# tie-pilot-qxw/NTT

Measured on AMD Instinct MI355X. Metric: field-elements/sec, 2^24 forward NTT over BN254 Fr; achieved HBM GB/s vs peak, higher is better.
Workload: dtype u256 mod p: 9 x 29-bit limbs, u32 x u32 + u64 MAD (v_mad_u64_u32)

## Files before the change

ntt_amd/csrc/eng29_args.hpp:

```cpp
#pragma once
#include <cmath>
#include <stdint.h>

#include "field29.hpp"

namespace ntt {

template <class E29, int L, int NH, class EA>
inline void eng29_fill_consts(EA& A, const uint32_t* p) {
  uint32_t pw[NH];
  for (int i = 0; i < NH; ++i) pw[i] = p[i];
  pack29<L, NH>(A.M.p, pw);
  for (int i = 0; i < L; ++i) A.kp[0][i] = A.M.p[i];
  for (int j = 1; j < 5; ++j) {
    for (int i = 0; i < L; ++i) A.kp[j][i] = A.kp[j - 1][i] << 1;
    norm_u<L>(A.kp[j]);
  }
  for (int i = 0; i < L; ++i) A.M.p2[i] = A.kp[1][i];
  neg29<L>(A.pbar, A.M.p);
  uint32_t inv = 1;
  for (int i = 0; i < 5; ++i) inv *= 2 - p[0] * inv;
  A.M.pinv = (0u - inv) & kMask29;
  const uint32_t ptop = A.M.p[L - 1];
  A.red_ok = ptop >= (1u << 18) ? 1u : 0u;
  A.red_inv = std::nextafter(1.0f / (float)(ptop + 1u), 0.0f);
  auto padded = [&](uint32_t K, uint32_t pad, uint32_t* c) {
    uint32_t kp[L];
    uint64_t carry = 0;
    for (int i = 0; i < L; ++i) {
      const uint64_t v = (uint64_t)A.M.p[i] * K + carry;
      kp[i] = (uint32_t)v & kMask29;
      carry = v >> 29;
    }
    kp[L - 1] += (uint32_t)(carry << 29);
    const uint32_t b = pad >> 29;
    c[0] = kp[0] + pad;
    for (int i = 1; i + 1 < L; ++i) c[i] = kp[i] + pad - b;
    c[L - 1] = kp[L - 1] - b;
  };
  padded(5, 1u << 29, A.pc[E29::PC_5_29]);
  padded(9, 1u << 30, A.pc[E29::PC_9_30]);
  padded(4, 1u << 29, A.pc[E29::PC_4_29]);
  padded(17, 1u << 29, A.pc[E29::PC_17_29]);
  padded(7, 1u << 30, A.pc[E29::PC_7_30]);
}

}
```

ntt_amd/csrc/engines.hpp:

```cpp
#pragma once
#include "field.hpp"
#include "field29.hpp"
#include "field29_asm9.hpp"
#include "field31.hpp"
#include "field64.hpp"

#ifndef NTT_DEBUG_CHECKS
#define NTT_DEBUG_CHECKS 0
#endif
enum : uint32_t {
  NTT_DBG_BOUNDS = 1u << 8,
  NTT_DBG_INPUT = 1u << 9,
  NTT_DBG_LAZY = 1u << 10,
  NTT_DBG_OUTPUT = 1u << 11
};
__device__ __forceinline__ void ntt_dbg_flag(uint32_t* status, uint32_t bit) {
  if (status) __hip_atomic_fetch_or(status, bit, __ATOMIC_RELAXED, __HIP_MEMORY_SCOPE_AGENT);
}
#ifndef NTT_WAVES_256
#define NTT_WAVES_256 4
#endif
#ifndef NTT_EPT_256
#define NTT_EPT_256 4
#endif
#ifndef NTT_256_PASS1_TABLE
#define NTT_256_PASS1_TABLE 1
#endif
#ifndef NTT_P_SCRATCH32
#define NTT_P_SCRATCH32 1
#endif
#ifndef NTT_P_NARROW_FIRST
#define NTT_P_NARROW_FIRST 1
#endif
#ifndef NTT_P_PASS1_TABLE
#define NTT_P_PASS1_TABLE 1
#endif
#ifndef NTT_P_LDS_TW
#define NTT_P_LDS_TW 1
#endif
#ifndef NTT_EPT_P
#define NTT_EPT_P 8
#endif
#ifndef NTT_TILE_LOG_P
#define NTT_TILE_LOG_P 13
#endif
#ifndef NTT_MIN_COLS_LOG_P
#define NTT_MIN_COLS_LOG_P 4
#endif
#ifndef NTT_TILE_LOG_256
#define NTT_TILE_LOG_256 10
#endif
#ifndef NTT_TILE_LOG_G
#define NTT_TILE_LOG_G 12
#endif
#ifndef NTT_EPT_G
#define NTT_EPT_G 8
#endif
#ifndef NTT_G_PASS1_TABLE
#define NTT_G_PASS1_TABLE 0
#endif
#ifndef NTT_TILE_LOG_31
#define NTT_TILE_LOG_31 13
#endif
#ifndef NTT_EPT_31
#define NTT_EPT_31 8
#endif
#ifndef NTT_MIN_COLS_LOG_31
#define NTT_MIN_COLS_LOG_31 4
#endif
#ifndef NTT_PREF_COLS_LOG_31
#define NTT_PREF_COLS_LOG_31 5
#endif
#ifndef NTT_31_PASS1_TABLE
#define NTT_31_PASS1_TABLE 1
#endif

namespace ntt {

__device__ __forceinline__ void store_wt16(uint4* p, uint32_t a, uint32_t b, uint32_t c, uint32_t d) {
  typedef uint32_t v4u __attribute__((ext_vector_type(4)));
  const v4u v = {a, b, c, d};
  asm volatile("global_store_dwordx4 %0, %1, off sc1\n\ts_nop 1" ::"v"(p), "v"(v) : "memory");
}

template <int L, int W32, int SCR_ = 0, int TL_ = 0>
struct Eng29 {
  static constexpr int W = L;
  static constexpr int MEMW = W32;
  static constexpr int SCRW = SCR_ ? SCR_ : ((L <= 9 && W32 > 8) ? 8 : W32);
  static constexpr int TABW = (L <= 9) ? 8 : W32;
  static constexpr int TW = (2 * L + 3) & ~3;
  static constexpr int LDSW = L;
  static constexpr int IN = 4;
  static constexpr int MUL_OUT = 4;
  static constexpr int EPT = (L <= 9) ? NTT_EPT_256 : 8;
  static constexpr int TILE_LOG = TL_ ? TL_ : ((L <= 9) ? (EPT == 8 ? 11 : NTT_TILE_LOG_256) : 10);
  static constexpr int WAVES_PER_EU = (L <= 9) ? (EPT == 4 ? NTT_WAVES_256 : 2) : 2;
  static constexpr int MIN_COLS_LOG = TL_ == 12 ? 0 : 2;
  static constexpr bool PASS1_FULL_TABLE = NTT_256_PASS1_TABLE;
  static constexpr bool NARROW_FIRST = false;
  static constexpr bool SHOUP_OUTER = (L == 9);
  static constexpr bool LDS_TW = false;
  static constexpr bool SGPR_TW = (L == 9);
  static constexpr bool FASTRED = 29 * L - 18 <= 255;
  struct Tw {
    uint32_t w[L];
    uint32_t ws[L];
  };
  struct Args {
    Mod29<L> M;
    uint32_t kp[5][L];
    uint32_t pbar[L];
    Tw w8[3];
    Tw ninv;
    float red_inv;
    uint32_t red_ok;
    uint32_t pc[5][L];
    uint32_t* dbg;
  };
  __device__ static bool dbg_below(const uint32_t (&x)[W], const uint32_t (&q)[L]) {
    uint32_t y[W];
#pragma unroll
    for (int i = 0; i < W; ++i) y[i] = x[i];
    norm_u<L>(y);
    for (int i = L - 1; i >= 0; --i)
      if (y[i] != q[i]) return y[i] < q[i];
    return false;
  }
  __device__ static bool dbg_canonical(const uint32_t (&x)[W], const Args& A) { return dbg_below(x, A.kp[0]); }
  enum : int { PC_5_29 = 0, PC_9_30 = 1, PC_4_29 = 2, PC_17_29 = 3, PC_7_30 = 4 };

  template <int MW = W32>
  __device__ static __forceinline__ void load(uint32_t (&x)[W], const uint32_t* __restrict__ base, size_t idx) {
    constexpr int MR = (L <= 9 && MW > 8 && !NTT_DEBUG_CHECKS) ? 8 : MW;
    uint32_t w[MW];
    const uint4* p = reinterpret_cast<const uint4*>(base + idx * MW);
#pragma unroll
    for (int q = 0; q < MW / 4; ++q) {
      if (4 * q < MR) {
        const uint4 v = p[q];
        w[4 * q] = v.x; w[4 * q + 1] = v.y; w[4 * q + 2] = v.z; w[4 * q + 3] = v.w;
      } else {
        w[4 * q] = w[4 * q + 1] = w[4 * q + 2] = w[4 * q + 3] = 0u;
      }
    }
    pack29<L, MW>(x, w);
  }
  template <int FROM, int TO>
  __device__ static __forceinline__ void reduce_chain(uint32_t (&x)[W], const Args& A) {
    static_assert(FROM <= 32 && TO >= 1, "lazy bound");
    if constexpr (FROM > TO) {
      constexpr int j = __builtin_ctz(FROM / 2);
      cond_sub<L>(x, A.kp[j]);
      reduce_chain<FROM / 2, TO>(x, A);
    }
  }
  template <bool R32 = true>
  __device__ static __forceinline__ void reduce_top(uint32_t (&x)[W], const Args& A) {
    const float qf = __builtin_fmaf((float)x[L - 1], A.red_inv, -0x1p-15f);
    const uint32_t q = qf > 0.f ? (uint32_t)qf : 0u;
    if constexpr (R32) {
    uint32_t c = 0;
#pragma unroll
    for (int i = 0; i < L; ++i) {
      const uint64_t acc = (uint64_t)q * A.pbar[i] + (uint32_t)(x[i] + c);
      x[i] = (uint32_t)acc & kMask29;
      c = (uint32_t)(acc >> 29);
    }
    } else {
    uint64_t acc = 0;
#pragma unroll
    for (int i = 0; i < L; ++i) {
      acc = (acc >> 29) + x[i] + (uint64_t)q * A.pbar[i];
      x[i] = (uint32_t)acc & kMask29;
    }
    }
  }
  __device__ static __forceinline__ void cond_sub_rare(uint32_t (&x)[W], const uint32_t (&q)[L]) {
    if (__any(x[L - 1] >= q[L - 1])) cond_sub<L>(x, q);
  }
  template <int FROM, int TO, bool FAST = false, bool R32 = true>
  __device__ static __forceinline__ void reduce(uint32_t (&x)[W], const Args& A) {
    if constexpr (FAST && FROM > 4 && TO <= 4) {
      reduce_top<R32>(x, A);
      if constexpr (TO == 1) cond_sub_rare(x, A.kp[0]);
    } else if constexpr (FAST && FROM == 4 && TO == 2) {
      cond_sub_rare(x, A.kp[1]);
    } else {
      reduce_chain<FROM, TO>(x, A);
    }
  }
  template <int BOUND, bool FAST = false, int MW = W32, bool WT = false>
  __device__ static __forceinline__ void store_lazy(uint32_t* __restrict__ base, size_t idx, uint32_t (&x)[W],
                                                    const Args& A) {
    reduce<BOUND, 2, FAST>(x, A);
#if NTT_DEBUG_CHECKS
    if (!dbg_below(x, A.kp[1])) ntt_dbg_flag(A.dbg, NTT_DBG_LAZY);
#endif
    put<MW, WT>(base, idx, x);
  }
  template <int BOUND, bool FAST = false, int MW = W32>
  __device__ static __forceinline__ void store(uint32_t* __restrict__ base, size_t idx, uint32_t (&x)[W],
                                               const Args& A) {
    reduce<BOUND, 1, FAST>(x, A);
#if NTT_DEBUG_CHECKS
    if (!dbg_below(x, A.kp[0])) ntt_dbg_flag(A.dbg, NTT_DBG_OUTPUT);
#endif
    put<MW>(base, idx, x);
  }
  template <int MW = W32, bool WT = false>
  __device__ static __forceinline__ void put(uint32_t* __restrict__ base, size_t idx, const uint32_t (&x)[W]) {
    uint32_t w[MW];
    unpack29<L, MW>(w, x);
    uint4* p = reinterpret_cast<uint4*>(base + idx * MW);
#pragma unroll
    for (int q = 0; q < MW / 4; ++q) {
      if constexpr (WT)
        store_wt16(p + q, w[4 * q], w[4 * q + 1], w[4 * q + 2], w[4 * q + 3]);
      else
        p[q] = make_uint4(w[4 * q], w[4 * q + 1], w[4 * q + 2], w[4 * q + 3]);
    }
  }
  __device__ static __forceinline__ void tload(Tw& t, const uint32_t* __restrict__ tab, size_t idx) {
    const uint4* p = reinterpret_cast<const uint4*>(tab + idx * TW);
#pragma unroll
    for (int q = 0; q < TW / 4; ++q) {
      const uint4 v = p[q];
      const uint32_t vv[4] = {v.x, v.y, v.z, v.w};
#pragma unroll
      for (int r = 0; r < 4; ++r) {
        const int i = 4 * q + r;
        if (i < L) t.w[i] = vv[r];
        else if (i < 2 * L) t.ws[i - L] = vv[r];
      }
    }
  }
  __device__ static __forceinline__ void tload_u(Tw& t, const uint32_t* __restrict__ tab, uint32_t idx) {
    typedef uint32_t V4 __attribute__((ext_vector_type(4)));
    typedef const __attribute__((address_space(4))) V4* CP;
    const CP p = (CP)(tab + (size_t)idx * TW);
#pragma unroll
    for (int q = 0; q < TW / 4; ++q) {
      const V4 v = p[q];
      const uint32_t vv[4] = {v.x, v.y, v.z, v.w};
#pragma unroll
      for (int r = 0; r < 4; ++r) {
        const int i = 4 * q + r;
        if (i < L) t.w[i] = vv[r];
        else if (i < 2 * L) t.ws[i - L] = vv[r];
      }
    }
  }
  __device__ static __forceinline__ void mul(uint32_t (&x)[W], const Tw& t, const Args& A) {
    uint32_t r[W];
    if constexpr (L == 9)
      mulc29_a9(r, x, t.w, t.ws, A.pbar);
    else
      mulc29_blk<L>(r, x, t.w, t.ws, A.pbar);
#pragma unroll
    for (int i = 0; i < W; ++i) x[i] = r[i];
  }
  __device__ static __forceinline__ void mul_u(uint32_t (&x)[W], const Tw& t, const Args& A) {
    uint32_t r[W];
    if constexpr (L == 9)
      mulc29_a9u(r, x, t.w, t.ws, A.pbar);
    else
      mulc29_blk<L>(r, x, t.w, t.ws, A.pbar);
#pragma unroll
    for (int i = 0; i < W; ++i) x[i] = r[i];
  }
  __device__ static __forceinline__ void mulv(uint32_t (&x)[W], const uint32_t (&y)[W], const Args& A) {
    uint32_t r[W];
    if constexpr (L == 9)
      mont29_a9(r, x, y, A.M);
    else
      mont29<L>(r, x, y, A.M);
#pragma unroll
    for (int i = 0; i < W; ++i) x[i] = r[i];
  }
  __device__ static __forceinline__ void bfly_lk(uint32_t (&a)[W], uint32_t (&b)[W], const uint32_t (&q)[L]) {
#pragma unroll
    for (int i = 0; i < L; ++i) {
      const uint32_t x = a[i], y = b[i];
      a[i] = x + y;
      b[i] = x - y + q[i];
    }
    norm_u<L>(a);
    norm_s<L>(b);
  }
  template <int K>
  __device__ static __forceinline__ void bfly_l(uint32_t (&a)[W], uint32_t (&b)[W], const Args& A) {
    static_assert(K == 4 || K == 8 || K == 16, "lazy bound");
    bfly_lk(a, b, A.kp[__builtin_ctz(K)]);
  }
  template <int K>
  __device__ static __forceinline__ void bfly_w_l(uint32_t (&a)[W], uint32_t (&b)[W], const Tw& t,
                                                  const Args& A) {
    bfly_l<K>(a, b, A);
    mul_u(b, t, A);
  }
  template <int CI>
  __device__ static __forceinline__ void bfly_raw(uint32_t (&a)[W], uint32_t (&b)[W], const Args& A) {
#pragma unroll
    for (int i = 0; i < L; ++i) {
      const uint32_t x = a[i], y = b[i];
      a[i] = x + y;
      b[i] = x - y + A.pc[CI][i];
    }
  }
  template <int CI>
  __device__ static __forceinline__ void bfly_raw_w(uint32_t (&a)[W], uint32_t (&b)[W], const Tw& t,
                                                    const Args& A) {
    bfly_raw<CI>(a, b, A);
    mul_u(b, t, A);
  }
  __device__ static __forceinline__ void norm(uint32_t (&x)[W]) {
    norm_u<L>(x);
  }
};

template <int N, int MEMW_, int SCR_ = 0>
struct Eng32 {
  static_assert(N == 1, "the 32-bit engine is the 1-limb path (p < 2^30)");
  static constexpr int W = 1;
  static constexpr int MEMW = MEMW_;
  static constexpr int SCRW = SCR_ ? SCR_ : (NTT_P_SCRATCH32 ? 1 : MEMW_);
  static constexpr int TABW = 1;
  static constexpr int TW = 2;
  static constexpr int LDSW = 1;
  static constexpr int IN = 4;
  static constexpr int MUL_OUT = 4;
  static constexpr int EPT = NTT_EPT_P;
  static constexpr int TILE_LOG = NTT_TILE_LOG_P;
  static constexpr int MIN_COLS_LOG = NTT_MIN_COLS_LOG_P;
  static constexpr bool PASS1_FULL_TABLE = NTT_P_PASS1_TABLE;
  static constexpr bool NARROW_FIRST = NTT_P_NARROW_FIRST;
  static constexpr bool SHOUP_OUTER = false;
  static constexpr bool LDS_TW = NTT_P_LDS_TW;
  static constexpr bool SGPR_TW = false;
  static constexpr int WAVES_PER_EU = 4;
  static constexpr bool FASTRED = false;
  struct Tw {
    uint32_t w[1];
    uint32_t ws;
  };
  struct Args {
    uint32_t p, p2;
    uint32_t pinv;
    Tw w8[3];
    Tw ninv;
    uint32_t* dbg;
  };
  __device__ static __forceinline__ uint32_t red(uint32_t x, uint32_t m) {
    return min(x, x - m);
  }
  __device__ static bool dbg_canonical(const uint32_t (&x)[W], const Args& A) { return x[0] < A.p; }
  __device__ static __forceinline__ uint32_t shoup(uint32_t x, uint32_t w, uint32_t ws, uint32_t p) {
    const uint32_t q = __umulhi(x, ws);
    return x * w - q * p;
  }
  template <int MW = MEMW_>
  __device__ static __forceinline__ void load(uint32_t (&x)[W], const uint32_t* __restrict__ base, size_t idx) {
    static_assert(MW == MEMW_ || MW == SCRW || MW == TABW, "HBM width");
    if constexpr (MW == 1)
      x[0] = base[idx];
    else
      x[0] = reinterpret_cast<const uint2*>(base)[idx].x;
  }
  template <int FROM, int TO, bool FAST = false, bool R32 = true>
  __device__ static __forceinline__ void reduce(uint32_t (&)[W], const Args&) {}
  template <int MW = MEMW_>
  __device__ static __forceinline__ void put(uint32_t* __restrict__ base, size_t idx, uint32_t v) {
    static_assert(MW == MEMW_ || MW == SCRW || MW == TABW, "HBM width");
    if constexpr (MW == 1)
      base[idx] = v;
    else
      reinterpret_cast<uint2*>(base)[idx] = make_uint2(v, 0u);
  }
  template <int BOUND, bool FAST = false, int MW = MEMW_, bool WT = false>
  __device__ static __forceinline__ void store_lazy(uint32_t* __restrict__ base, size_t idx, uint32_t (&x)[W],
                                                    [[maybe_unused]] const Args& A) {
    static_assert(!WT, "write-through scratch stores: Eng29 engines only (fused schedule)");
#if NTT_DEBUG_CHECKS
    if (x[0] >= A.p2) ntt_dbg_flag(A.dbg, NTT_DBG_LAZY);
#endif
    put<MW>(base, idx, x[0]);
  }
  template <int BOUND, bool FAST = false, int MW = MEMW_>
  __device__ static __forceinline__ void store(uint32_t* __restrict__ base, size_t idx, uint32_t (&x)[W],
                                               const Args& A) {
    const uint32_t v = red(x[0], A.p);
#if NTT_DEBUG_CHECKS
    if (v >= A.p) ntt_dbg_flag(A.dbg, NTT_DBG_OUTPUT);
#endif
    put<MW>(base, idx, v);
  }
  __device__ static __forceinline__ void tload(Tw& t, const uint32_t* __restrict__ tab, size_t idx) {
    const uint2 v = reinterpret_cast<const uint2*>(tab)[idx];
    t.w[0] = v.x;
    t.ws = v.y;
  }
  __device__ static __forceinline__ void tload_lds(Tw& t, const uint32_t* lds_tw, uint32_t idx) {
    const uint2 v = reinterpret_cast<const uint2*>(lds_tw)[idx];
    t.w[0] = v.x;
    t.ws = v.y;
  }
  __device__ static __forceinline__ void mul(uint32_t (&x)[W], const Tw& t, const Args& A) {
    x[0] = shoup(x[0], t.w[0], t.ws, A.p);
  }
  __device__ static __forceinline__ void mul_u(uint32_t (&x)[W], const Tw& t, const Args& A) { mul(x, t, A); }
  __device__ static __forceinline__ void mulv(uint32_t (&x)[W], const uint32_t (&y)[W], const Args& A) {
    const uint32_t lo = x[0] * y[0], hi = __umulhi(x[0], y[0]);
    const uint32_t m = lo * A.pinv;
    x[0] = hi - __umulhi(m, A.p) + A.p;
  }
  template <int K>
  __device__ static __forceinline__ void bfly_l(uint32_t (&a)[W], uint32_t (&b)[W], const Args& A) {
    const uint32_t s = a[0] + b[0], d = a[0] - b[0] + A.p2;
    a[0] = red(s, A.p2);
    b[0] = red(d, A.p2);
  }
  template <int K>
  __device__ static __forceinline__ void bfly_w_l(uint32_t (&a)[W], uint32_t (&b)[W], const Tw& t, const Args& A) {
    const uint32_t s = a[0] + b[0], d = a[0] - b[0] + A.p2;
    a[0] = red(s, A.p2);
    b[0] = shoup(d, t.w[0], t.ws, A.p);
  }
};

struct Eng64G {
  static constexpr int W = 2;
  static constexpr int MEMW = 2;
  static constexpr int SCRW = 2;
  static constexpr int TABW = 2;
  static constexpr int TW = 2;
  static constexpr int LDSW = 2;
  static constexpr int IN = 1;
  static constexpr int MUL_OUT = 1;
  static constexpr int EPT = NTT_EPT_G;
  static constexpr int TILE_LOG = NTT_TILE_LOG_G;
  static constexpr int MIN_COLS_LOG = 4;
  static constexpr bool PASS1_FULL_TABLE = NTT_G_PASS1_TABLE;
  static constexpr bool NARROW_FIRST = true;
  static constexpr bool SHOUP_OUTER = false;
  static constexpr bool LDS_TW = false;
  static constexpr bool SGPR_TW = false;
  static constexpr int WAVES_PER_EU = 4;
  static constexpr bool FASTRED = false;
  struct Tw {
    uint32_t w[2];
  };
  struct Args {
    Tw w8[3];
    Tw ninv;
    uint32_t* dbg;
  };
  __device__ static __forceinline__ uint64_t u64(const uint32_t (&x)[W]) { return ((uint64_t)x[1] << 32) | x[0]; }
  __device__ static __forceinline__ void set(uint32_t (&x)[W], uint64_t v) {
    x[0] = (uint32_t)v;
    x[1] = (uint32_t)(v >> 32);
  }
  __device__ static bool dbg_canonical(const uint32_t (&x)[W], const Args&) { return gl64::is_canonical(u64(x)); }
  template <int MW = MEMW>
  __device__ static __forceinline__ void load(uint32_t (&x)[W], const uint32_t* __restrict__ base, size_t idx) {
    static_assert(MW == 2, "HBM width");
    const uint2 v = reinterpret_cast<const uint2*>(base)[idx];
    x[0] = v.x;
    x[1] = v.y;
  }
  template <int FROM, int TO, bool FAST = false, bool R32 = true>
  __device__ static __forceinline__ void reduce(uint32_t (&)[W], const Args&) {}
  template <int MW = MEMW, bool WT = false>
  __device__ static __forceinline__ void put(uint32_t* __restrict__ base, size_t idx, const uint32_t (&x)[W]) {
    static_assert(MW == 2 && !WT, "HBM width; write-through stores: Eng29 engines only");
    reinterpret_cast<uint2*>(base)[idx] = make_uint2(x[0], x[1]);
  }
  template <int BOUND, bool FAST = false, int MW = MEMW, bool WT = false>
  __device__ static __forceinline__ void store_lazy(uint32_t* __restrict__ base, size_t idx, uint32_t (&x)[W],
                                                    [[maybe_unused]] const Args& A) {
#if NTT_DEBUG_CHECKS
    if (!gl64::is_canonical(u64(x))) ntt_dbg_flag(A.dbg, NTT_DBG_LAZY);
#endif
    put<MW, WT>(base, idx, x);
  }
  template <int BOUND, bool FAST = false, int MW = MEMW>
  __device__ static __forceinline__ void store(uint32_t* __restrict__ base, size_t idx, uint32_t (&x)[W],
                                               [[maybe_unused]] const Args& A) {
#if NTT_DEBUG_CHECKS
    if (!gl64::is_canonical(u64(x))) ntt_dbg_flag(A.dbg, NTT_DBG_OUTPUT);
#endif
    put<MW>(base, idx, x);
  }
  __device__ static __forceinline__ void tload(Tw& t, const uint32_t* __restrict__ tab, size_t idx) {
    const uint2 v = reinterpret_cast<const uint2*>(tab)[idx];
    t.w[0] = v.x;
    t.w[1] = v.y;
  }
  __device__ static __forceinline__ void tload_lds(Tw& t, const uint32_t* lds_tw, uint32_t idx) {
    const uint2 v = reinterpret_cast<const uint2*>(lds_tw)[idx];
    t.w[0] = v.x;
    t.w[1] = v.y;
  }
  __device__ static __forceinline__ void mul(uint32_t (&x)[W], const Tw& t, const Args&) {
    set(x, gl64::mul(u64(x), u64(t.w)));
  }
  __device__ static __forceinline__ void mul_u(uint32_t (&x)[W], const Tw& t, const Args& A) { mul(x, t, A); }
  __device__ static __forceinline__ void mulv(uint32_t (&x)[W], const uint32_t (&y)[W], const Args&) {
    set(x, gl64::mul(u64(x), u64(y)));
  }
  template <int K>
  __device__ static __forceinline__ void bfly_l(uint32_t (&a)[W], uint32_t (&b)[W], const Args&) {
    const uint64_t x = u64(a), y = u64(b);
    set(a, gl64::add(x, y));
    set(b, gl64::sub(x, y));
  }
  template <int K>
  __device__ static __forceinline__ void bfly_w_l(uint32_t (&a)[W], uint32_t (&b)[W], const Tw& t, const Args&) {
    const uint64_t x = u64(a), y = u64(b);
    set(a, gl64::add(x, y));
    set(b, gl64::mul(gl64::sub(x, y), u64(t.w)));
  }
};

struct Eng31 {
  static constexpr int W = 1;
  static constexpr int MEMW = 1;
  static constexpr int SCRW = 1;
  static constexpr int TABW = 1;
  static constexpr int TW = 2;
  static constexpr int LDSW = 1;
  static constexpr int IN = 1;
  static constexpr int MUL_OUT = 1;
  static constexpr int EPT = NTT_EPT_31;
  static constexpr int TILE_LOG = NTT_TILE_LOG_31;
  static constexpr int MIN_COLS_LOG = NTT_MIN_COLS_LOG_31;
  static constexpr int PREF_COLS_LOG = NTT_PREF_COLS_LOG_31 > NTT_MIN_COLS_LOG_31 ? NTT_PREF_COLS_LOG_31 : NTT_MIN_COLS_LOG_31;
  static constexpr bool PASS1_FULL_TABLE = NTT_31_PASS1_TABLE;
  static constexpr bool NARROW_FIRST = true;
  static constexpr bool SHOUP_OUTER = false;
  static constexpr bool LDS_TW = true;
  static constexpr bool SGPR_TW = false;
  static constexpr int WAVES_PER_EU = 4;
  static constexpr bool FASTRED = false;
  struct Tw {
    uint32_t w[1];
    uint32_t ws;
  };
  struct Args {
    uint32_t p;
    uint32_t pinv;
    Tw w8[3];
    Tw ninv;
    uint32_t* dbg;
  };
  __device__ static bool dbg_canonical(const uint32_t (&x)[W], const Args& A) { return f31::is_canonical(x[0], A.p); }
  template <int MW = MEMW>
  __device__ static __forceinline__ void load(uint32_t (&x)[W], const uint32_t* __restrict__ base, size_t idx) {
    static_assert(MW == 1, "HBM width");
    x[0] = base[idx];
  }
  template <int FROM, int TO, bool FAST = false, bool R32 = true>
  __device__ static __forceinline__ void reduce(uint32_t (&)[W], const Args&) {}
  template <int BOUND, bool FAST = false, int MW = MEMW, bool WT = false>
  __device__ static __forceinline__ void store_lazy(uint32_t* __restrict__ base, size_t idx, uint32_t (&x)[W],
                                                    [[maybe_unused]] const Args& A) {
    static_assert(MW == 1 && !WT, "HBM width; write-through stores: Eng29 engines only");
#if NTT_DEBUG_CHECKS
    if (!f31::is_canonical(x[0], A.p)) ntt_dbg_flag(A.dbg, NTT_DBG_LAZY);
#endif
    base[idx] = x[0];
  }
  template <int BOUND, bool FAST = false, int MW = MEMW>
  __device__ static __forceinline__ void store(uint32_t* __restrict__ base, size_t idx, uint32_t (&x)[W],
                                               [[maybe_unused]] const Args& A) {
    static_assert(MW == 1, "HBM width");
#if NTT_DEBUG_CHECKS
    if (!f31::is_canonical(x[0], A.p)) ntt_dbg_flag(A.dbg, NTT_DBG_OUTPUT);
#endif
    base[idx] = x[0];
  }
  __device__ static __forceinline__ void tload(Tw& t, const uint32_t* __restrict__ tab, size_t idx) {
    const uint2 v = reinterpret_cast<const uint2*>(tab)[idx];
    t.w[0] = v.x;
    t.ws = v.y;
  }
  __device__ static __forceinline__ void tload_lds(Tw& t, const uint32_t* lds_tw, uint32_t idx) {
    const uint2 v = reinterpret_cast<const uint2*>(lds_tw)[idx];
    t.w[0] = v.x;
    t.ws = v.y;
  }
  __device__ static __forceinline__ void mul(uint32_t (&x)[W], const Tw& t, const Args& A) {
    x[0] = f31::mulc(x[0], t.w[0], t.ws, A.p);
  }
  __device__ static __forceinline__ void mul_u(uint32_t (&x)[W], const Tw& t, const Args& A) { mul(x, t, A); }
  __device__ static __forceinline__ void mulv(uint32_t (&x)[W], const uint32_t (&y)[W], const Args& A) {
    x[0] = f31::mulv(x[0], y[0], A.p, A.pinv);
  }
  template <int K>
  __device__ static __forceinline__ void bfly_l(uint32_t (&a)[W], uint32_t (&b)[W], const Args& A) {
    const uint32_t x = a[0], y = b[0];
    a[0] = f31::add(x, y, A.p);
    b[0] = f31::sub(x, y, A.p);
  }
  template <int K>
  __device__ static __forceinline__ void bfly_w_l(uint32_t (&a)[W], uint32_t (&b)[W], const Tw& t, const Args& A) {
    const uint32_t x = a[0], y = b[0];
    a[0] = f31::add(x, y, A.p);
    b[0] = f31::mulc(f31::sub_lazy(x, y, A.p), t.w[0], t.ws, A.p);
  }
};

template <int LDSW, int E>
__device__ __forceinline__ void lds_put(uint32_t* lds, uint32_t idx, const uint32_t (&x)[LDSW]) {
  constexpr int Q = LDSW / 4;
  uint4* l4 = reinterpret_cast<uint4*>(lds);
#pragma unroll
  for (int q = 0; q < Q; ++q) l4[q * E + idx] = make_uint4(x[4 * q], x[4 * q + 1], x[4 * q + 2], x[4 * q + 3]);
  uint32_t* l1 = lds + 4 * Q * E;
#pragma unroll
  for (int r = 4 * Q; r < LDSW; ++r) l1[(r - 4 * Q) * E + idx] = x[r];
}
template <int LDSW, int E>
__device__ __forceinline__ void lds_get(uint32_t (&x)[LDSW], const uint32_t* lds, uint32_t idx) {
  constexpr int Q = LDSW / 4;
  const uint4* l4 = reinterpret_cast<const uint4*>(lds);
#pragma unroll
  for (int q = 0; q < Q; ++q) {
    const uint4 v = l4[q * E + idx];
    x[4 * q] = v.x; x[4 * q + 1] = v.y; x[4 * q + 2] = v.z; x[4 * q + 3] = v.w;
  }
  const uint32_t* l1 = lds + 4 * Q * E;
#pragma unroll
  for (int r = 4 * Q; r < LDSW; ++r) x[r] = l1[(r - 4 * Q) * E + idx];
}

}
```

ntt_amd/csrc/field29.hpp:

```cpp
#pragma once
#include <stdint.h>

#if defined(__HIPCC__) || defined(__HIP__)
#include <hip/hip_runtime.h>
#define F29_HD __host__ __device__ __forceinline__
#else
#define F29_HD static inline
#endif

namespace ntt {

constexpr uint32_t kMask29 = (1u << 29) - 1;

template <int L>
struct Mod29 {
  uint32_t p[L];
  uint32_t p2[L];
  uint32_t pinv;
};

template <int L>
F29_HD void norm_u(uint32_t (&x)[L]) {
#pragma unroll
  for (int i = 0; i + 1 < L; ++i) {
    x[i + 1] += x[i] >> 29;
    x[i] &= kMask29;
  }
}
template <int L>
F29_HD int32_t norm_s(uint32_t (&x)[L]) {
#pragma unroll
  for (int i = 0; i + 1 < L; ++i) {
    x[i + 1] = (uint32_t)((int32_t)x[i + 1] + ((int32_t)x[i] >> 29));
    x[i] &= kMask29;
  }
  return (int32_t)x[L - 1];
}

template <int L>
F29_HD void cond_sub(uint32_t (&x)[L], const uint32_t (&q)[L]) {
  uint32_t t[L];
#pragma unroll
  for (int i = 0; i < L; ++i) t[i] = x[i] - q[i];
  const bool neg = norm_s<L>(t) < 0;
#pragma unroll
  for (int i = 0; i < L; ++i) x[i] = neg ? x[i] : t[i];
}

template <int L>
F29_HD void add29(uint32_t (&u)[L], const uint32_t (&a)[L], const uint32_t (&b)[L], const Mod29<L>& M) {
#pragma unroll
  for (int i = 0; i < L; ++i) u[i] = a[i] + b[i];
  norm_u<L>(u);
  cond_sub<L>(u, M.p2);
}
template <int L>
F29_HD void sub29_raw(uint32_t (&d)[L], const uint32_t (&a)[L], const uint32_t (&b)[L], const Mod29<L>& M) {
#pragma unroll
  for (int i = 0; i < L; ++i) d[i] = a[i] - b[i] + M.p2[i];
  norm_s<L>(d);
}
template <int L>
F29_HD void sub29(uint32_t (&d)[L], const uint32_t (&a)[L], const uint32_t (&b)[L], const Mod29<L>& M) {
  sub29_raw<L>(d, a, b, M);
  cond_sub<L>(d, M.p2);
}

template <int L>
F29_HD void mont29(uint32_t (&r)[L], const uint32_t (&a)[L], const uint32_t (&b)[L], const Mod29<L>& M) {
  uint32_t m[L];
  uint64_t acc = 0;
#pragma unroll
  for (int i = 0; i < L; ++i) {
#pragma unroll
    for (int j = 0; j < i; ++j) {
      acc += (uint64_t)a[j] * b[i - j];
      acc += (uint64_t)m[j] * M.p[i - j];
    }
    acc += (uint64_t)a[i] * b[0];
    m[i] = ((uint32_t)acc * M.pinv) & kMask29;
    acc += (uint64_t)m[i] * M.p[0];
    acc >>= 29;
  }
#pragma unroll
  for (int i = L; i < 2 * L; ++i) {
#pragma unroll
    for (int j = i - L + 1; j < L; ++j) {
      acc += (uint64_t)a[j] * b[i - j];
      acc += (uint64_t)m[j] * M.p[i - j];
    }
    r[i - L] = (uint32_t)acc & kMask29;
    acc >>= 29;
  }
}

#if defined(__HIP_DEVICE_COMPILE__)
__device__ __forceinline__ uint64_t mad29v(uint32_t a, uint32_t b, uint64_t c) {
  uint64_t r, cc;
  asm("v_mad_u64_u32 %0, %1, %2, %3, %4" : "=v"(r), "=s"(cc) : "v"(a), "v"(b), "v"(c));
  return r;
}
__device__ __forceinline__ uint64_t mad29s(uint32_t a, uint32_t b, uint64_t c) {
  uint64_t r, cc;
  asm("v_mad_u64_u32 %0, %1, %2, %3, %4" : "=v"(r), "=s"(cc) : "v"(a), "s"(b), "v"(c));
  return r;
}
#else
static inline uint64_t mad29v(uint32_t a, uint32_t b, uint64_t c) { return c + (uint64_t)a * b; }
static inline uint64_t mad29s(uint32_t a, uint32_t b, uint64_t c) { return c + (uint64_t)a * b; }
#endif

#if defined(__HIP_DEVICE_COMPILE__)
#define NTT_MAD4(C1, C2)                                                                          \
  asm("v_mad_u64_u32 %0, %1, %2, %3, %0\n\t"                                                   \
      "v_mad_u64_u32 %0, %1, %4, %5, %0\n\t"                                                   \
      "v_mad_u64_u32 %0, %1, %6, %7, %0\n\t"                                                   \
      "v_mad_u64_u32 %0, %1, %8, %9, %0"                                                       \
      : "+v"(acc), "=&s"(cc)                                                                    \
      : "v"(a0), C2(b0), "v"(a1), C2(b1), "v"(a2), C2(b2), "v"(a3), C2(b3))
#define NTT_MAD2(C2)                                                                              \
  asm("v_mad_u64_u32 %0, %1, %2, %3, %0\n\t"                                                   \
      "v_mad_u64_u32 %0, %1, %4, %5, %0"                                                       \
      : "+v"(acc), "=&s"(cc)                                                                    \
      : "v"(a0), C2(b0), "v"(a1), C2(b1))
#define NTT_CV(x) "v"(x)
#define NTT_CS(x) "s"(x)
__device__ __forceinline__ uint64_t mad4vv(uint64_t acc, uint32_t a0, uint32_t b0, uint32_t a1, uint32_t b1,
                                           uint32_t a2, uint32_t b2, uint32_t a3, uint32_t b3) {
  uint64_t cc;
  NTT_MAD4(NTT_CV, NTT_CV);
  return acc;
}
__device__ __forceinline__ uint64_t mad4vs(uint64_t acc, uint32_t a0, uint32_t b0, uint32_t a1, uint32_t b1,
                                           uint32_t a2, uint32_t b2, uint32_t a3, uint32_t b3) {
  uint64_t cc;
  NTT_MAD4(NTT_CV, NTT_CS);
  return acc;
}
__device__ __forceinline__ uint64_t mad2vv(uint64_t acc, uint32_t a0, uint32_t b0, uint32_t a1, uint32_t b1) {
  uint64_t cc;
  NTT_MAD2(NTT_CV);
  return acc;
}
__device__ __forceinline__ uint64_t mad2vs(uint64_t acc, uint32_t a0, uint32_t b0, uint32_t a1, uint32_t b1) {
  uint64_t cc;
  NTT_MAD2(NTT_CS);
  return acc;
}
#undef NTT_MAD4
#undef NTT_MAD2
#undef NTT_CV
#undef NTT_CS
#else
static inline uint64_t mad4vv(uint64_t acc, uint32_t a0, uint32_t b0, uint32_t a1, uint32_t b1, uint32_t a2,
                              uint32_t b2, uint32_t a3, uint32_t b3) {
  return acc + (uint64_t)a0 * b0 + (uint64_t)a1 * b1 + (uint64_t)a2 * b2 + (uint64_t)a3 * b3;
}
static inline uint64_t mad4vs(uint64_t acc, uint32_t a0, uint32_t b0, uint32_t a1, uint32_t b1, uint32_t a2,
                              uint32_t b2, uint32_t a3, uint32_t b3) {
  return mad4vv(acc, a0, b0, a1, b1, a2, b2, a3, b3);
}
static inline uint64_t mad2vv(uint64_t acc, uint32_t a0, uint32_t b0, uint32_t a1, uint32_t b1) {
  return acc + (uint64_t)a0 * b0 + (uint64_t)a1 * b1;
}
static inline uint64_t mad2vs(uint64_t acc, uint32_t a0, uint32_t b0, uint32_t a1, uint32_t b1) {
  return mad2vv(acc, a0, b0, a1, b1);
}
#endif

template <int L, bool US, int lo, int hi>
F29_HD uint64_t mad_span(uint64_t acc, const uint32_t (&a)[L], const uint32_t (&b)[L], int k) {
  if constexpr (hi - lo + 1 >= 4) {
    acc = US ? mad4vs(acc, a[lo], b[k - lo], a[lo + 1], b[k - lo - 1], a[lo + 2], b[k - lo - 2], a[lo + 3],
                      b[k - lo - 3])
             : mad4vv(acc, a[lo], b[k - lo], a[lo + 1], b[k - lo - 1], a[lo + 2], b[k - lo - 2], a[lo + 3],
                      b[k - lo - 3]);
    return mad_span<L, US, lo + 4, hi>(acc, a, b, k);
  } else if constexpr (hi - lo + 1 >= 2) {
    acc = US ? mad2vs(acc, a[lo], b[k - lo], a[lo + 1], b[k - lo - 1])
             : mad2vv(acc, a[lo], b[k - lo], a[lo + 1], b[k - lo - 1]);
    return mad_span<L, US, lo + 2, hi>(acc, a, b, k);
  } else if constexpr (hi - lo + 1 == 1) {
    return US ? mad29s(a[lo], b[k - lo], acc) : mad29v(a[lo], b[k - lo], acc);
  } else {
    return acc;
  }
}

template <int L, int K = L - 2>
F29_HD void mulc29_hi(uint32_t (&q)[L], uint64_t& acc, const uint32_t (&x)[L], const uint32_t (&ws)[L]) {
  if constexpr (K < 2 * L - 1) {
    constexpr int lo = (K - (L - 1) > 0) ? K - (L - 1) : 0, hi = (K < L - 1) ? K : L - 1;
    acc = mad_span<L, false, lo, hi>(acc, x, ws, K);
    if constexpr (K >= L) q[K - L] = (uint32_t)acc & kMask29;
    acc >>= 29;
    mulc29_hi<L, K + 1>(q, acc, x, ws);
  }
}
template <int L, int K = 0>
F29_HD void mulc29_lo(uint32_t (&r)[L], uint64_t& acc, const uint32_t (&x)[L], const uint32_t (&w)[L],
                      const uint32_t (&q)[L], const uint32_t (&pbar)[L]) {
  if constexpr (K < L) {
    acc = mad_span<L, false, 0, K>(acc, x, w, K);
    acc = mad_span<L, true, 0, K>(acc, q, pbar, K);
    r[K] = (uint32_t)acc & kMask29;
    acc >>= 29;
    mulc29_lo<L, K + 1>(r, acc, x, w, q, pbar);
  }
}
template <int L>
F29_HD void mulc29_blk(uint32_t (&r)[L], const uint32_t (&x)[L], const uint32_t (&w)[L], const uint32_t (&ws)[L],
                       const uint32_t (&pbar)[L]) {
  uint32_t q[L];
  uint64_t acc = 0;
  mulc29_hi<L>(q, acc, x, ws);
  q[L - 1] = (uint32_t)acc;
  acc = 0;
  mulc29_lo<L>(r, acc, x, w, q, pbar);
}

template <int L>
F29_HD void mont29_chain(uint32_t (&r)[L], const uint32_t (&a)[L], const uint32_t (&b)[L], const Mod29<L>& M) {
  uint32_t m[L];
  uint64_t acc = 0;
#pragma unroll
  for (int i = 0; i < L; ++i) {
#pragma unroll
    for (int j = 0; j <= i; ++j) acc = mad29v(a[j], b[i - j], acc);
#pragma unroll
    for (int j = 0; j < i; ++j) acc = mad29s(m[j], M.p[i - j], acc);
    m[i] = ((uint32_t)acc * M.pinv) & kMask29;
    acc = mad29s(m[i], M.p[0], acc);
    acc >>= 29;
  }
#pragma unroll
  for (int i = L; i < 2 * L; ++i) {
#pragma unroll
    for (int j = i - L + 1; j < L; ++j) acc = mad29v(a[j], b[i - j], acc);
#pragma unroll
    for (int j = i - L + 1; j < L; ++j) acc = mad29s(m[j], M.p[i - j], acc);
    r[i - L] = (uint32_t)acc & kMask29;
    acc >>= 29;
  }
}

template <int L>
F29_HD void mulc29(uint32_t (&r)[L], const uint32_t (&x)[L], const uint32_t (&w)[L], const uint32_t (&ws)[L],
                   const uint32_t (&pbar)[L]) {
  uint32_t q[L];
  uint64_t acc = 0;
#pragma unroll
  for (int k = L - 2; k < 2 * L - 1; ++k) {
#pragma unroll
    for (int i = (k - (L - 1) > 0 ? k - (L - 1) : 0); i <= (k < L - 1 ? k : L - 1); ++i)
      acc = mad29v(x[i], ws[k - i], acc);
    if (k >= L) q[k - L] = (uint32_t)acc & kMask29;
    acc >>= 29;
  }
  q[L - 1] = (uint32_t)acc;
  acc = 0;
#pragma unroll
  for (int k = 0; k < L; ++k) {
#pragma unroll
    for (int i = 0; i <= k; ++i) acc = mad29v(x[i], w[k - i], acc);
#pragma unroll
    for (int i = 0; i <= k; ++i) acc = mad29s(q[i], pbar[k - i], acc);
    r[k] = (uint32_t)acc & kMask29;
    acc >>= 29;
  }
}

template <int L>
F29_HD void mulc29_cc(uint32_t (&r)[L], const uint32_t (&x)[L], const uint32_t (&w)[L], const uint32_t (&ws)[L],
                   const uint32_t (&pbar)[L]) {
  uint32_t q[L];
  uint64_t acc = 0;
#pragma unroll
  for (int k = L - 2; k < 2 * L - 1; ++k) {
#pragma unroll
    for (int i = (k - (L - 1) > 0 ? k - (L - 1) : 0); i <= (k < L - 1 ? k : L - 1); ++i)
      acc += (uint64_t)x[i] * ws[k - i];
    if (k >= L) q[k - L] = (uint32_t)acc & kMask29;
    acc >>= 29;
  }
  q[L - 1] = (uint32_t)acc;
  acc = 0;
#pragma unroll
  for (int k = 0; k < L; ++k) {
#pragma unroll
    for (int i = 0; i <= k; ++i) acc += (uint64_t)x[i] * w[k - i];
#pragma unroll
    for (int i = 0; i <= k; ++i) acc += (uint64_t)q[i] * pbar[k - i];
    r[k] = (uint32_t)acc & kMask29;
    acc >>= 29;
  }
}

template <int L>
F29_HD void mullo29(uint32_t (&r)[L], const uint32_t (&a)[L], const uint32_t (&b)[L]) {
  uint64_t acc = 0;
#pragma unroll
  for (int k = 0; k < L; ++k) {
#pragma unroll
    for (int i = 0; i <= k; ++i) acc = mad29v(a[i], b[k - i], acc);
    r[k] = (uint32_t)acc & kMask29;
    acc >>= 29;
  }
}
template <int L>
F29_HD void neg29(uint32_t (&r)[L], const uint32_t (&a)[L]) {
  uint32_t c = 1;
#pragma unroll
  for (int i = 0; i < L; ++i) {
    const uint32_t v = (kMask29 - a[i]) + c;
    r[i] = v & kMask29;
    c = v >> 29;
  }
}
template <int L>
F29_HD void shoup_ws29(uint32_t (&ws)[L], const uint32_t (&wR)[L], const uint32_t (&pinvB)[L]) {
  uint32_t t[L];
  neg29<L>(t, wR);
  mullo29<L>(ws, t, pinvB);
}
template <int L>
F29_HD void inv_mod_B29(uint32_t (&inv)[L], const uint32_t (&p)[L]) {
  uint32_t i0 = 1;
  for (int k = 0; k < 5; ++k) i0 *= 2 - p[0] * i0;
#pragma unroll
  for (int i = 0; i < L; ++i) inv[i] = 0;
  inv[0] = i0 & kMask29;
  for (int bits = 29; bits < 29 * L; bits *= 2) {
    uint32_t t[L], u[L];
    mullo29<L>(t, p, inv);
    neg29<L>(u, t);
    uint32_t c = 2;
    for (int i = 0; i < L; ++i) {
      const uint32_t v = u[i] + c;
      u[i] = v & kMask29;
      c = v >> 29;
    }
    mullo29<L>(t, inv, u);
    for (int i = 0; i < L; ++i) inv[i] = t[i];
  }
}

template <int L, int W32>
F29_HD void pack29(uint32_t (&x)[L], const uint32_t (&w)[W32]) {
#pragma unroll
  for (int i = 0; i < L; ++i) {
    const int bit = 29 * i, k = bit / 32, s = bit % 32;
    const uint32_t lo = (k < W32) ? w[k] : 0u;
    const uint32_t hi = (k + 1 < W32) ? w[k + 1] : 0u;
#if defined(__HIP_DEVICE_COMPILE__)
    x[i] = __builtin_amdgcn_alignbit(hi, lo, (uint32_t)s) & kMask29;
#else
    const uint64_t v = ((uint64_t)hi << 32) | lo;
    x[i] = (uint32_t)(v >> s) & kMask29;
#endif
  }
}
template <int L, int W32>
F29_HD void unpack29(uint32_t (&w)[W32], const uint32_t (&x)[L]) {
#pragma unroll
  for (int k = 0; k < W32; ++k) {
    const int bit = 32 * k, i = bit / 29, s = bit % 29;
    uint32_t v = (i < L) ? (x[i] >> s) : 0u;
    if (i + 1 < L) v |= x[i + 1] << (29 - s);
    if (i + 2 < L && 58 - s < 32) v |= x[i + 2] << (58 - s);
    w[k] = v;
  }
}

}
```

ntt_amd/csrc/field29_asm9.hpp:

```cpp
#pragma once
#include "field29.hpp"

namespace ntt {
#if defined(__HIP_DEVICE_COMPILE__)
__device__ __forceinline__ void mulc29_a9(uint32_t (&r)[9], const uint32_t (&x)[9], const uint32_t (&w)[9],
                                          const uint32_t (&ws)[9], const uint32_t (&pbar)[9]) {
  uint32_t q[9];
  uint64_t acc = 0, cc;
  asm("v_mad_u64_u32 %0, %1, %2, %3, %0\n\tv_mad_u64_u32 %0, %1, %4, %5, %0\n\tv_mad_u64_u32 %0, %1, %6, %7, %0\n\tv_mad_u64_u32 %0, %1, %8, %9, %0\n\tv_mad_u64_u32 %0, %1, %10, %11, %0\n\tv_mad_u64_u32 %0, %1, %12, %13, %0\n\tv_mad_u64_u32 %0, %1, %14, %15, %0\n\tv_mad_u64_u32 %0, %1, %16, %17, %0"
      : "+v"(acc), "=&s"(cc)
      : "v"(x[0]), "v"(ws[7]), "v"(x[1]), "v"(ws[6]), "v"(x[2]), "v"(ws[5]),
        "v"(x[3]), "v"(ws[4]), "v"(x[4]), "v"(ws[3]), "v"(x[5]), "v"(ws[2]),
        "v"(x[6]), "v"(ws[1]), "v"(x[7]), "v"(ws[0]));
  acc >>= 29;
  asm("v_mad_u64_u32 %0, %1, %2, %3, %0\n\tv_mad_u64_u32 %0, %1, %4, %5, %0\n\tv_mad_u64_u32 %0, %1, %6, %7, %0\n\tv_mad_u64_u32 %0, %1, %8, %9, %0\n\tv_mad_u64_u32 %0, %1, %10, %11, %0\n\tv_mad_u64_u32 %0, %1, %12, %13, %0\n\tv_mad_u64_u32 %0, %1, %14, %15, %0\n\tv_mad_u64_u32 %0, %1, %16, %17, %0\n\tv_mad_u64_u32 %0, %1, %18, %19, %0"
      : "+v"(acc), "=&s"(cc)
      : "v"(x[0]), "v"(ws[8]), "v"(x[1]), "v"(ws[7]), "v"(x[2]), "v"(ws[6]),
        "v"(x[3]), "v"(ws[5]), "v"(x[4]), "v"(ws[4]), "v"(x[5]), "v"(ws[3]),
        "v"(x[6]), "v"(ws[2]), "v"(x[7]), "v"(ws[1]), "v"(x[8]), "v"(ws[0]));
  acc >>= 29;
  asm("v_mad_u64_u32 %0, %1, %2, %3, %0\n\tv_mad_u64_u32 %0, %1, %4, %5, %0\n\tv_mad_u64_u32 %0, %1, %6, %7, %0\n\tv_mad_u64_u32 %0, %1, %8, %9, %0\n\tv_mad_u64_u32 %0, %1, %10, %11, %0\n\tv_mad_u64_u32 %0, %1, %12, %13, %0\n\tv_mad_u64_u32 %0, %1, %14, %15, %0\n\tv_mad_u64_u32 %0, %1, %16, %17, %0"
      : "+v"(acc), "=&s"(cc)
      : "v"(x[1]), "v"(ws[8]), "v"(x[2]), "v"(ws[7]), "v"(x[3]), "v"(ws[6]),
        "v"(x[4]), "v"(ws[5]), "v"(x[5]), "v"(ws[4]), "v"(x[6]), "v"(ws[3]),
        "v"(x[7]), "v"(ws[2]), "v"(x[8]), "v"(ws[1]));
  q[0] = (uint32_t)acc & kMask29;
  acc >>= 29;
  asm("v_mad_u64_u32 %0, %1, %2, %3, %0\n\tv_mad_u64_u32 %0, %1, %4, %5, %0\n\tv_mad_u64_u32 %0, %1, %6, %7, %0\n\tv_mad_u64_u32 %0, %1, %8, %9, %0\n\tv_mad_u64_u32 %0, %1, %10, %11, %0\n\tv_mad_u64_u32 %0, %1, %12, %13, %0\n\tv_mad_u64_u32 %0, %1, %14, %15, %0"
      : "+v"(acc), "=&s"(cc)
      : "v"(x[2]), "v"(ws[8]), "v"(x[3]), "v"(ws[7]), "v"(x[4]), "v"(ws[6]),
        "v"(x[5]), "v"(ws[5]), "v"(x[6]), "v"(ws[4]), "v"(x[7]), "v"(ws[3]),
        "v"(x[8]), "v"(ws[2]));
  q[1] = (uint32_t)acc & kMask29;
  acc >>= 29;
  asm("v_mad_u64_u32 %0, %1, %2, %3, %0\n\tv_mad_u64_u32 %0, %1, %4, %5, %0\n\tv_mad_u64_u32 %0, %1, %6, %7, %0\n\tv_mad_u64_u32 %0, %1, %8, %9, %0\n\tv_mad_u64_u32 %0, %1, %10, %11, %0\n\tv_mad_u64_u32 %0, %1, %12, %13, %0"
      : "+v"(acc), "=&s"(cc)
      : "v"(x[3]), "v"(ws[8]), "v"(x[4]), "v"(ws[7]), "v"(x[5]), "v"(ws[6]),
        "v"(x[6]), "v"(ws[5]), "v"(x[7]), "v"(ws[4]), "v"(x[8]), "v"(ws[3]));
  q[2] = (uint32_t)acc & kMask29;
  acc >>= 29;
  asm("v_mad_u64_u32 %0, %1, %2, %3, %0\n\tv_mad_u64_u32 %0, %1, %4, %5, %0\n\tv_mad_u64_u32 %0, %1, %6, %7, %0\n\tv_mad_u64_u32 %0, %1, %8, %9, %0\n\tv_mad_u64_u32 %0, %1, %10, %11, %0"
      : "+v"(acc), "=&s"(cc)
      : "v"(x[4]), "v"(ws[8]), "v"(x[5]), "v"(ws[7]), "v"(x[6]), "v"(ws[6]),
        "v"(x[7]), "v"(ws[5]), "v"(x[8]), "v"(ws[4]));
  q[3] = (uint32_t)acc & kMask29;
  acc >>= 29;
  asm("v_mad_u64_u32 %0, %1, %2, %3, %0\n\tv_mad_u64_u32 %0, %1, %4, %5, %0\n\tv_mad_u64_u32 %0, %1, %6, %7, %0\n\tv_mad_u64_u32 %0, %1, %8, %9, %0"
      : "+v"(acc), "=&s"(cc)
      : "v"(x[5]), "v"(ws[8]), "v"(x[6]), "v"(ws[7]), "v"(x[7]), "v"(ws[6]),
        "v"(x[8]), "v"(ws[5]));
  q[4] = (uint32_t)acc & kMask29;
  acc >>= 29;
  asm("v_mad_u64_u32 %0, %1, %2, %3, %0\n\tv_mad_u64_u32 %0, %1, %4, %5, %0\n\tv_mad_u64_u32 %0, %1, %6, %7, %0"
      : "+v"(acc), "=&s"(cc)
      : "v"(x[6]), "v"(ws[8]), "v"(x[7]), "v"(ws[7]), "v"(x[8]), "v"(ws[6]));
  q[5] = (uint32_t)acc & kMask29;
  acc >>= 29;
  asm("v_mad_u64_u32 %0, %1, %2, %3, %0\n\tv_mad_u64_u32 %0, %1, %4, %5, %0"
      : "+v"(acc), "=&s"(cc)
      : "v"(x[7]), "v"(ws[8]), "v"(x[8]), "v"(ws[7]));
  q[6] = (uint32_t)acc & kMask29;
  acc >>= 29;
  asm("v_mad_u64_u32 %0, %1, %2, %3, %0"
      : "+v"(acc), "=&s"(cc)
      : "v"(x[8]), "v"(ws[8]));
  q[7] = (uint32_t)acc & kMask29;
  acc >>= 29;
  q[8] = (uint32_t)acc;
  acc = 0;
  asm("v_mad_u64_u32 %0, %1, %2, %3, %0\n\tv_mad_u64_u32 %0, %1, %4, %5, %0"
      : "+v"(acc), "=&s"(cc)
      : "v"(x[0]), "v"(w[0]), "v"(q[0]), "s"(pbar[0]));
  r[0] = (uint32_t)acc & kMask29;
  acc >>= 29;
  asm("v_mad_u64_u32 %0, %1, %2, %3, %0\n\tv_mad_u64_u32 %0, %1, %4, %5, %0\n\tv_mad_u64_u32 %0, %1, %6, %7, %0\n\tv_mad_u64_u32 %0, %1, %8, %9, %0"
      : "+v"(acc), "=&s"(cc)
      : "v"(x[0]), "v"(w[1]), "v"(x[1]), "v"(w[0]), "v"(q[0]), "s"(pbar[1]),
        "v"(q[1]), "s"(pbar[0]));
  r[1] = (uint32_t)acc & kMask29;
  acc >>= 29;
  asm("v_mad_u64_u32 %0, %1, %2, %3, %0\n\tv_mad_u64_u32 %0, %1, %4, %5, %0\n\tv_mad_u64_u32 %0, %1, %6, %7, %0\n\tv_mad_u64_u32 %0, %1, %8, %9, %0\n\tv_mad_u64_u32 %0, %1, %10, %11, %0\n\tv_mad_u64_u32 %0, %1, %12, %13, %0"
      : "+v"(acc), "=&s"(cc)
      : "v"(x[0]), "v"(w[2]), "v"(x[1]), "v"(w[1]), "v"(x[2]), "v"(w[0]),
        "v"(q[0]), "s"(pbar[2]), "v"(q[1]), "s"(pbar[1]), "v"(q[2]), "s"(pbar[0]));
  r[2] = (uint32_t)acc & kMask29;
  acc >>= 29;
  asm("v_mad_u64_u32 %0, %1, %2, %3, %0\n\tv_mad_u64_u32 %0, %1, %4, %5, %0\n\tv_mad_u64_u32 %0, %1, %6, %7, %0\n\tv_mad_u64_u32 %0, %1, %8, %9, %0\n\tv_mad_u64_u32 %0, %1, %10, %11, %0\n\tv_mad_u64_u32 %0, %1, %12, %13, %0\n\tv_mad_u64_u32 %0, %1, %14, %15, %0\n\tv_mad_u64_u32 %0, %1, %16, %17, %0"
      : "+v"(acc), "=&s"(cc)
      : "v"(x[0]), "v"(w[3]), "v"(x[1]), "v"(w[2]), "v"(x[2]), "v"(w[1]),
        "v"(x[3]), "v"(w[0]), "v"(q[0]), "s"(pbar[3]), "v"(q[1]), "s"(pbar[2]),
        "v"(q[2]), "s"(pbar[1]), "v"(q[3]), "s"(pbar[0]));
  r[3] = (uint32_t)acc & kMask29;
  acc >>= 29;
  asm("v_mad_u64_u32 %0, %1, %2, %3, %0\n\tv_mad_u64_u32 %0, %1, %4, %5, %0\n\tv_mad_u64_u32 %0, %1, %6, %7, %0\n\tv_mad_u64_u32 %0, %1, %8, %9, %0\n\tv_mad_u64_u32 %0, %1, %10, %11, %0\n\tv_mad_u64_u32 %0, %1, %12, %13, %0\n\tv_mad_u64_u32 %0, %1, %14, %15, %0\n\tv_mad_u64_u32 %0, %1, %16, %17, %0\n\tv_mad_u64_u32 %0, %1, %18, %19, %0\n\tv_mad_u64_u32 %0, %1, %20, %21, %0"
      : "+v"(acc), "=&s"(cc)
      : "v"(x[0]), "v"(w[4]), "v"(x[1]), "v"(w[3]), "v"(x[2]), "v"(w[2]),
        "v"(x[3]), "v"(w[1]), "v"(x[4]), "v"(w[0]), "v"(q[0]), "s"(pbar[4]),
        "v"(q[1]), "s"(pbar[3]), "v"(q[2]), "s"(pbar[2]), "v"(q[3]), "s"(pbar[1]),
        "v"(q[4]), "s"(pbar[0]));
  r[4] = (uint32_t)acc & kMask29;
  acc >>= 29;
  asm("v_mad_u64_u32 %0, %1, %2, %3, %0\n\tv_mad_u64_u32 %0, %1, %4, %5, %0\n\tv_mad_u64_u32 %0, %1, %6, %7, %0\n\tv_mad_u64_u32 %0, %1, %8, %9, %0\n\tv_mad_u64_u32 %0, %1, %10, %11, %0\n\tv_mad_u64_u32 %0, %1, %12, %13, %0\n\tv_mad_u64_u32 %0, %1, %14, %15, %0\n\tv_mad_u64_u32 %0, %1, %16, %17, %0\n\tv_mad_u64_u32 %0, %1, %18, %19, %0\n\tv_mad_u64_u32 %0, %1, %20, %21, %0\n\tv_mad_u64_u32 %0, %1, %22, %23, %0\n\tv_mad_u64_u32 %0, %1, %24, %25, %0"
      : "+v"(acc), "=&s"(cc)
      : "v"(x[0]), "v"(w[5]), "v"(x[1]), "v"(w[4]), "v"(x[2]), "v"(w[3]),
        "v"(x[3]), "v"(w[2]), "v"(x[4]), "v"(w[1]), "v"(x[5]), "v"(w[0]),
        "v"(q[0]), "s"(pbar[5]), "v"(q[1]), "s"(pbar[4]), "v"(q[2]), "s"(pbar[3]),
        "v"(q[3]), "s"(pbar[2]), "v"(q[4]), "s"(pbar[1]), "v"(q[5]), "s"(pbar[0]));
  r[5] = (uint32_t)acc & kMask29;
  acc >>= 29;
  asm("v_mad_u64_u32 %0, %1, %2, %3, %0\n\tv_mad_u64_u32 %0, %1, %4, %5, %0\n\tv_mad_u64_u32 %0, %1, %6, %7, %0\n\tv_mad_u64_u32 %0, %1, %8, %9, %0\n\tv_mad_u64_u32 %0, %1, %10, %11, %0\n\tv_mad_u64_u32 %0, %1, %12, %13, %0\n\tv_mad_u64_u32 %0, %1, %14, %15, %0\n\tv_mad_u64_u32 %0, %1, %16, %17, %0\n\tv_mad_u64_u32 %0, %1, %18, %19, %0\n\tv_mad_u64_u32 %0, %1, %20, %21, %0\n\tv_mad_u64_u32 %0, %1, %22, %23, %0\n\tv_mad_u64_u32 %0, %1, %24, %25, %0\n\tv_mad_u64_u32 %0, %1, %26, %27, %0\n\tv_mad_u64_u32 %0, %1, %28, %29, %0"
      : "+v"(acc), "=&s"(cc)
      : "v"(x[0]), "v"(w[6]), "v"(x[1]), "v"(w[5]), "v"(x[2]), "v"(w[4]),
        "v"(x[3]), "v"(w[3]), "v"(x[4]), "v"(w[2]), "v"(x[5]), "v"(w[1]),
        "v"(x[6]), "v"(w[0]), "v"(q[0]), "s"(pbar[6]), "v"(q[1]), "s"(pbar[5]),
        "v"(q[2]), "s"(pbar[4]), "v"(q[3]), "s"(pbar[3]), "v"(q[4]), "s"(pbar[2]),
        "v"(q[5]), "s"(pbar[1]), "v"(q[6]), "s"(pbar[0]));
  r[6] = (uint32_t)acc & kMask29;
  acc >>= 29;
  asm("v_mad_u64_u32 %0, %1, %2, %3, %0\n\tv_mad_u64_u32 %0, %1, %4, %5, %0\n\tv_mad_u64_u32 %0, %1, %6, %7, %0\n\tv_mad_u64_u32 %0, %1, %8, %9, %0\n\tv_mad_u64_u32 %0, %1, %10, %11, %0\n\tv_mad_u64_u32 %0, %1, %12, %13, %0\n\tv_mad_u64_u32 %0, %1, %14, %15, %0\n\tv_mad_u64_u32 %0, %1, %16, %17, %0\n\tv_mad_u64_u32 %0, %1, %18, %19, %0\n\tv_mad_u64_u32 %0, %1, %20, %21, %0\n\tv_mad_u64_u32 %0, %1, %22, %23, %0\n\tv_mad_u64_u32 %0, %1, %24, %25, %0\n\tv_mad_u64_u32 %0, %1, %26, %27, %0\n\tv_mad_u64_u32 %0, %1, %28, %29, %0\n\tv_mad_u64_u32 %0, %1, %30, %31, %0\n\tv_mad_u64_u32 %0, %1, %32, %33, %0"
      : "+v"(acc), "=&s"(cc)
      : "v"(x[0]), "v"(w[7]), "v"(x[1]), "v"(w[6]), "v"(x[2]), "v"(w[5]),
        "v"(x[3]), "v"(w[4]), "v"(x[4]), "v"(w[3]), "v"(x[5]), "v"(w[2]),
        "v"(x[6]), "v"(w[1]), "v"(x[7]), "v"(w[0]), "v"(q[0]), "s"(pbar[7]),
        "v"(q[1]), "s"(pbar[6]), "v"(q[2]), "s"(pbar[5]), "v"(q[3]), "s"(pbar[4]),
        "v"(q[4]), "s"(pbar[3]), "v"(q[5]), "s"(pbar[2]), "v"(q[6]), "s"(pbar[1]),
        "v"(q[7]), "s"(pbar[0]));
  r[7] = (uint32_t)acc & kMask29;
  acc >>= 29;
  asm("v_mad_u64_u32 %0, %1, %2, %3, %0\n\tv_mad_u64_u32 %0, %1, %4, %5, %0\n\tv_mad_u64_u32 %0, %1, %6, %7, %0\n\tv_mad_u64_u32 %0, %1, %8, %9, %0\n\tv_mad_u64_u32 %0, %1, %10, %11, %0\n\tv_mad_u64_u32 %0, %1, %12, %13, %0\n\tv_mad_u64_u32 %0, %1, %14, %15, %0\n\tv_mad_u64_u32 %0, %1, %16, %17, %0\n\tv_mad_u64_u32 %0, %1, %18, %19, %0\n\tv_mad_u64_u32 %0, %1, %20, %21, %0\n\tv_mad_u64_u32 %0, %1, %22, %23, %0\n\tv_mad_u64_u32 %0, %1, %24, %25, %0\n\tv_mad_u64_u32 %0, %1, %26, %27, %0\n\tv_mad_u64_u32 %0, %1, %28, %29, %0\n\tv_mad_u64_u32 %0, %1, %30, %31, %0\n\tv_mad_u64_u32 %0, %1, %32, %33, %0\n\tv_mad_u64_u32 %0, %1, %34, %35, %0\n\tv_mad_u64_u32 %0, %1, %36, %37, %0"
      : "+v"(acc), "=&s"(cc)
      : "v"(x[0]), "v"(w[8]), "v"(x[1]), "v"(w[7]), "v"(x[2]), "v"(w[6]),
        "v"(x[3]), "v"(w[5]), "v"(x[4]), "v"(w[4]), "v"(x[5]), "v"(w[3]),
        "v"(x[6]), "v"(w[2]), "v"(x[7]), "v"(w[1]), "v"(x[8]), "v"(w[0]),
        "v"(q[0]), "s"(pbar[8]), "v"(q[1]), "s"(pbar[7]), "v"(q[2]), "s"(pbar[6]),
        "v"(q[3]), "s"(pbar[5]), "v"(q[4]), "s"(pbar[4]), "v"(q[5]), "s"(pbar[3]),
        "v"(q[6]), "s"(pbar[2]), "v"(q[7]), "s"(pbar[1]), "v"(q[8]), "s"(pbar[0]));
  r[8] = (uint32_t)acc & kMask29;
}

__device__ __forceinline__ void mulc29_a9u(uint32_t (&r)[9], const uint32_t (&x)[9], const uint32_t (&w)[9],
                                          const uint32_t (&ws)[9], const uint32_t (&pbar)[9]) {
  uint32_t q[9];
  uint64_t acc = 0, cc;
  asm("v_mad_u64_u32 %0, %1, %2, %3, %0\n\tv_mad_u64_u32 %0, %1, %4, %5, %0\n\tv_mad_u64_u32 %0, %1, %6, %7, %0\n\tv_mad_u64_u32 %0, %1, %8, %9, %0\n\tv_mad_u64_u32 %0, %1, %10, %11, %0\n\tv_mad_u64_u32 %0, %1, %12, %13, %0\n\tv_mad_u64_u32 %0, %1, %14, %15, %0\n\tv_mad_u64_u32 %0, %1, %16, %17, %0"
      : "+v"(acc), "=&s"(cc)
      : "v"(x[0]), "s"(ws[7]), "v"(x[1]), "s"(ws[6]), "v"(x[2]), "s"(ws[5]),
        "v"(x[3]), "s"(ws[4]), "v"(x[4]), "s"(ws[3]), "v"(x[5]), "s"(ws[2]),
        "v"(x[6]), "s"(ws[1]), "v"(x[7]), "s"(ws[0]));
  acc >>= 29;
  asm("v_mad_u64_u32 %0, %1, %2, %3, %0\n\tv_mad_u64_u32 %0, %1, %4, %5, %0\n\tv_mad_u64_u32 %0, %1, %6, %7, %0\n\tv_mad_u64_u32 %0, %1, %8, %9, %0\n\tv_mad_u64_u32 %0, %1, %10, %11, %0\n\tv_mad_u64_u32 %0, %1, %12, %13, %0\n\tv_mad_u64_u32 %0, %1, %14, %15, %0\n\tv_mad_u64_u32 %0, %1, %16, %17, %0\n\tv_mad_u64_u32 %0, %1, %18, %19, %0"
      : "+v"(acc), "=&s"(cc)
      : "v"(x[0]), "s"(ws[8]), "v"(x[1]), "s"(ws[7]), "v"(x[2]), "s"(ws[6]),
        "v"(x[3]), "s"(ws[5]), "v"(x[4]), "s"(ws[4]), "v"(x[5]), "s"(ws[3]),
        "v"(x[6]), "s"(ws[2]), "v"(x[7]), "s"(ws[1]), "v"(x[8]), "s"(ws[0]));
  acc >>= 29;
  asm("v_mad_u64_u32 %0, %1, %2, %3, %0\n\tv_mad_u64_u32 %0, %1, %4, %5, %0\n\tv_mad_u64_u32 %0, %1, %6, %7, %0\n\tv_mad_u64_u32 %0, %1, %8, %9, %0\n\tv_mad_u64_u32 %0, %1, %10, %11, %0\n\tv_mad_u64_u32 %0, %1, %12, %13, %0\n\tv_mad_u64_u32 %0, %1, %14, %15, %0\n\tv_mad_u64_u32 %0, %1, %16, %17, %0"
      : "+v"(acc), "=&s"(cc)
      : "v"(x[1]), "s"(ws[8]), "v"(x[2]), "s"(ws[7]), "v"(x[3]), "s"(ws[6]),
        "v"(x[4]), "s"(ws[5]), "v"(x[5]), "s"(ws[4]), "v"(x[6]), "s"(ws[3]),
        "v"(x[7]), "s"(ws[2]), "v"(x[8]), "s"(ws[1]));
  q[0] = (uint32_t)acc & kMask29;
  acc >>= 29;
  asm("v_mad_u64_u32 %0, %1, %2, %3, %0\n\tv_mad_u64_u32 %0, %1, %4, %5, %0\n\tv_mad_u64_u32 %0, %1, %6, %7, %0\n\tv_mad_u64_u32 %0, %1, %8, %9, %0\n\tv_mad_u64_u32 %0, %1, %10, %11, %0\n\tv_mad_u64_u32 %0, %1, %12, %13, %0\n\tv_mad_u64_u32 %0, %1, %14, %15, %0"
      : "+v"(acc), "=&s"(cc)
      : "v"(x[2]), "s"(ws[8]), "v"(x[3]), "s"(ws[7]), "v"(x[4]), "s"(ws[6]),
        "v"(x[5]), "s"(ws[5]), "v"(x[6]), "s"(ws[4]), "v"(x[7]), "s"(ws[3]),
        "v"(x[8]), "s"(ws[2]));
  q[1] = (uint32_t)acc & kMask29;
  acc >>= 29;
  asm("v_mad_u64_u32 %0, %1, %2, %3, %0\n\tv_mad_u64_u32 %0, %1, %4, %5, %0\n\tv_mad_u64_u32 %0, %1, %6, %7, %0\n\tv_mad_u64_u32 %0, %1, %8, %9, %0\n\tv_mad_u64_u32 %0, %1, %10, %11, %0\n\tv_mad_u64_u32 %0, %1, %12, %13, %0"
      : "+v"(acc), "=&s"(cc)
      : "v"(x[3]), "s"(ws[8]), "v"(x[4]), "s"(ws[7]), "v"(x[5]), "s"(ws[6]),
        "v"(x[6]), "s"(ws[5]), "v"(x[7]), "s"(ws[4]), "v"(x[8]), "s"(ws[3]));
  q[2] = (uint32_t)acc & kMask29;
  acc >>= 29;
  asm("v_mad_u64_u32 %0, %1, %2, %3, %0\n\tv_mad_u64_u32 %0, %1, %4, %5, %0\n\tv_mad_u64_u32 %0, %1, %6, %7, %0\n\tv_mad_u64_u32 %0, %1, %8, %9, %0\n\tv_mad_u64_u32 %0, %1, %10, %11, %0"
      : "+v"(acc), "=&s"(cc)
      : "v"(x[4]), "s"(ws[8]), "v"(x[5]), "s"(ws[7]), "v"(x[6]), "s"(ws[6]),
        "v"(x[7]), "s"(ws[5]), "v"(x[8]), "s"(ws[4]));
  q[3] = (uint32_t)acc & kMask29;
  acc >>= 29;
  asm("v_mad_u64_u32 %0, %1, %2, %3, %0\n\tv_mad_u64_u32 %0, %1, %4, %5, %0\n\tv_mad_u64_u32 %0, %1, %6, %7, %0\n\tv_mad_u64_u32 %0, %1, %8, %9, %0"
      : "+v"(acc), "=&s"(cc)
      : "v"(x[5]), "s"(ws[8]), "v"(x[6]), "s"(ws[7]), "v"(x[7]), "s"(ws[6]),
        "v"(x[8]), "s"(ws[5]));
  q[4] = (uint32_t)acc & kMask29;
  acc >>= 29;
  asm("v_mad_u64_u32 %0, %1, %2, %3, %0\n\tv_mad_u64_u32 %0, %1, %4, %5, %0\n\tv_mad_u64_u32 %0, %1, %6, %7, %0"
      : "+v"(acc), "=&s"(cc)
      : "v"(x[6]), "s"(ws[8]), "v"(x[7]), "s"(ws[7]), "v"(x[8]), "s"(ws[6]));
  q[5] = (uint32_t)acc & kMask29;
  acc >>= 29;
  asm("v_mad_u64_u32 %0, %1, %2, %3, %0\n\tv_mad_u64_u32 %0, %1, %4, %5, %0"
      : "+v"(acc), "=&s"(cc)
      : "v"(x[7]), "s"(ws[8]), "v"(x[8]), "s"(ws[7]));
  q[6] = (uint32_t)acc & kMask29;
  acc >>= 29;
  asm("v_mad_u64_u32 %0, %1, %2, %3, %0"
      : "+v"(acc), "=&s"(cc)
      : "v"(x[8]), "s"(ws[8]));
  q[7] = (uint32_t)acc & kMask29;
  acc >>= 29;
  q[8] = (uint32_t)acc;
  acc = 0;
  asm("v_mad_u64_u32 %0, %1, %2, %3, %0\n\tv_mad_u64_u32 %0, %1, %4, %5, %0"
      : "+v"(acc), "=&s"(cc)
      : "v"(x[0]), "s"(w[0]), "v"(q[0]), "s"(pbar[0]));
  r[0] = (uint32_t)acc & kMask29;
  acc >>= 29;
  asm("v_mad_u64_u32 %0, %1, %2, %3, %0\n\tv_mad_u64_u32 %0, %1, %4, %5, %0\n\tv_mad_u64_u32 %0, %1, %6, %7, %0\n\tv_mad_u64_u32 %0, %1, %8, %9, %0"
      : "+v"(acc), "=&s"(cc)
      : "v"(x[0]), "s"(w[1]), "v"(x[1]), "s"(w[0]), "v"(q[0]), "s"(pbar[1]),
        "v"(q[1]), "s"(pbar[0]));
  r[1] = (uint32_t)acc & kMask29;
  acc >>= 29;
  asm("v_mad_u64_u32 %0, %1, %2, %3, %0\n\tv_mad_u64_u32 %0, %1, %4, %5, %0\n\tv_mad_u64_u32 %0, %1, %6, %7, %0\n\tv_mad_u64_u32 %0, %1, %8, %9, %0\n\tv_mad_u64_u32 %0, %1, %10, %11, %0\n\tv_mad_u64_u32 %0, %1, %12, %13, %0"
      : "+v"(acc), "=&s"(cc)
      : "v"(x[0]), "s"(w[2]), "v"(x[1]), "s"(w[1]), "v"(x[2]), "s"(w[0]),
        "v"(q[0]), "s"(pbar[2]), "v"(q[1]), "s"(pbar[1]), "v"(q[2]), "s"(pbar[0]));
  r[2] = (uint32_t)acc & kMask29;
  acc >>= 29;
  asm("v_mad_u64_u32 %0, %1, %2, %3, %0\n\tv_mad_u64_u32 %0, %1, %4, %5, %0\n\tv_mad_u64_u32 %0, %1, %6, %7, %0\n\tv_mad_u64_u32 %0, %1, %8, %9, %0\n\tv_mad_u64_u32 %0, %1, %10, %11, %0\n\tv_mad_u64_u32 %0, %1, %12, %13, %0\n\tv_mad_u64_u32 %0, %1, %14, %15, %0\n\tv_mad_u64_u32 %0, %1, %16, %17, %0"
      : "+v"(acc), "=&s"(cc)
      : "v"(x[0]), "s"(w[3]), "v"(x[1]), "s"(w[2]), "v"(x[2]), "s"(w[1]),
        "v"(x[3]), "s"(w[0]), "v"(q[0]), "s"(pbar[3]), "v"(q[1]), "s"(pbar[2]),
        "v"(q[2]), "s"(pbar[1]), "v"(q[3]), "s"(pbar[0]));
  r[3] = (uint32_t)acc & kMask29;
  acc >>= 29;
  asm("v_mad_u64_u32 %0, %1, %2, %3, %0\n\tv_mad_u64_u32 %0, %1, %4, %5, %0\n\tv_mad_u64_u32 %0, %1, %6, %7, %0\n\tv_mad_u64_u32 %0, %1, %8, %9, %0\n\tv_mad_u64_u32 %0, %1, %10, %11, %0\n\tv_mad_u64_u32 %0, %1, %12, %13, %0\n\tv_mad_u64_u32 %0, %1, %14, %15, %0\n\tv_mad_u64_u32 %0, %1, %16, %17, %0\n\tv_mad_u64_u32 %0, %1, %18, %19, %0\n\tv_mad_u64_u32 %0, %1, %20, %21, %0"
      : "+v"(acc), "=&s"(cc)
      : "v"(x[0]), "s"(w[4]), "v"(x[1]), "s"(w[3]), "v"(x[2]), "s"(w[2]),
        "v"(x[3]), "s"(w[1]), "v"(x[4]), "s"(w[0]), "v"(q[0]), "s"(pbar[4]),
        "v"(q[1]), "s"(pbar[3]), "v"(q[2]), "s"(pbar[2]), "v"(q[3]), "s"(pbar[1]),
        "v"(q[4]), "s"(pbar[0]));
  r[4] = (uint32_t)acc & kMask29;
  acc >>= 29;
  asm("v_mad_u64_u32 %0, %1, %2, %3, %0\n\tv_mad_u64_u32 %0, %1, %4, %5, %0\n\tv_mad_u64_u32 %0, %1, %6, %7, %0\n\tv_mad_u64_u32 %0, %1, %8, %9, %0\n\tv_mad_u64_u32 %0, %1, %10, %11, %0\n\tv_mad_u64_u32 %0, %1, %12, %13, %0\n\tv_mad_u64_u32 %0, %1, %14, %15, %0\n\tv_mad_u64_u32 %0, %1, %16, %17, %0\n\tv_mad_u64_u32 %0, %1, %18, %19, %0\n\tv_mad_u64_u32 %0, %1, %20, %21, %0\n\tv_mad_u64_u32 %0, %1, %22, %23, %0\n\tv_mad_u64_u32 %0, %1, %24, %25, %0"
      : "+v"(acc), "=&s"(cc)
      : "v"(x[0]), "s"(w[5]), "v"(x[1]), "s"(w[4]), "v"(x[2]), "s"(w[3]),
        "v"(x[3]), "s"(w[2]), "v"(x[4]), "s"(w[1]), "v"(x[5]), "s"(w[0]),
        "v"(q[0]), "s"(pbar[5]), "v"(q[1]), "s"(pbar[4]), "v"(q[2]), "s"(pbar[3]),
        "v"(q[3]), "s"(pbar[2]), "v"(q[4]), "s"(pbar[1]), "v"(q[5]), "s"(pbar[0]));
  r[5] = (uint32_t)acc & kMask29;
  acc >>= 29;
  asm("v_mad_u64_u32 %0, %1, %2, %3, %0\n\tv_mad_u64_u32 %0, %1, %4, %5, %0\n\tv_mad_u64_u32 %0, %1, %6, %7, %0\n\tv_mad_u64_u32 %0, %1, %8, %9, %0\n\tv_mad_u64_u32 %0, %1, %10, %11, %0\n\tv_mad_u64_u32 %0, %1, %12, %13, %0\n\tv_mad_u64_u32 %0, %1, %14, %15, %0\n\tv_mad_u64_u32 %0, %1, %16, %17, %0\n\tv_mad_u64_u32 %0, %1, %18, %19, %0\n\tv_mad_u64_u32 %0, %1, %20, %21, %0\n\tv_mad_u64_u32 %0, %1, %22, %23, %0\n\tv_mad_u64_u32 %0, %1, %24, %25, %0\n\tv_mad_u64_u32 %0, %1, %26, %27, %0\n\tv_mad_u64_u32 %0, %1, %28, %29, %0"
      : "+v"(acc), "=&s"(cc)
      : "v"(x[0]), "s"(w[6]), "v"(x[1]), "s"(w[5]), "v"(x[2]), "s"(w[4]),
        "v"(x[3]), "s"(w[3]), "v"(x[4]), "s"(w[2]), "v"(x[5]), "s"(w[1]),
        "v"(x[6]), "s"(w[0]), "v"(q[0]), "s"(pbar[6]), "v"(q[1]), "s"(pbar[5]),
        "v"(q[2]), "s"(pbar[4]), "v"(q[3]), "s"(pbar[3]), "v"(q[4]), "s"(pbar[2]),
        "v"(q[5]), "s"(pbar[1]), "v"(q[6]), "s"(pbar[0]));
  r[6] = (uint32_t)acc & kMask29;
  acc >>= 29;
  asm("v_mad_u64_u32 %0, %1, %2, %3, %0\n\tv_mad_u64_u32 %0, %1, %4, %5, %0\n\tv_mad_u64_u32 %0, %1, %6, %7, %0\n\tv_mad_u64_u32 %0, %1, %8, %9, %0\n\tv_mad_u64_u32 %0, %1, %10, %11, %0\n\tv_mad_u64_u32 %0, %1, %12, %13, %0\n\tv_mad_u64_u32 %0, %1, %14, %15, %0\n\tv_mad_u64_u32 %0, %1, %16, %17, %0\n\tv_mad_u64_u32 %0, %1, %18, %19, %0\n\tv_mad_u64_u32 %0, %1, %20, %21, %0\n\tv_mad_u64_u32 %0, %1, %22, %23, %0\n\tv_mad_u64_u32 %0, %1, %24, %25, %0\n\tv_mad_u64_u32 %0, %1, %26, %27, %0\n\tv_mad_u64_u32 %0, %1, %28, %29, %0\n\tv_mad_u64_u32 %0, %1, %30, %31, %0\n\tv_mad_u64_u32 %0, %1, %32, %33, %0"
      : "+v"(acc), "=&s"(cc)
      : "v"(x[0]), "s"(w[7]), "v"(x[1]), "s"(w[6]), "v"(x[2]), "s"(w[5]),
        "v"(x[3]), "s"(w[4]), "v"(x[4]), "s"(w[3]), "v"(x[5]), "s"(w[2]),
        "v"(x[6]), "s"(w[1]), "v"(x[7]), "s"(w[0]), "v"(q[0]), "s"(pbar[7]),
        "v"(q[1]), "s"(pbar[6]), "v"(q[2]), "s"(pbar[5]), "v"(q[3]), "s"(pbar[4]),
        "v"(q[4]), "s"(pbar[3]), "v"(q[5]), "s"(pbar[2]), "v"(q[6]), "s"(pbar[1]),
        "v"(q[7]), "s"(pbar[0]));
  r[7] = (uint32_t)acc & kMask29;
  acc >>= 29;
  asm("v_mad_u64_u32 %0, %1, %2, %3, %0\n\tv_mad_u64_u32 %0, %1, %4, %5, %0\n\tv_mad_u64_u32 %0, %1, %6, %7, %0\n\tv_mad_u64_u32 %0, %1, %8, %9, %0\n\tv_mad_u64_u32 %0, %1, %10, %11, %0\n\tv_mad_u64_u32 %0, %1, %12, %13, %0\n\tv_mad_u64_u32 %0, %1, %14, %15, %0\n\tv_mad_u64_u32 %0, %1, %16, %17, %0\n\tv_mad_u64_u32 %0, %1, %18, %19, %0\n\tv_mad_u64_u32 %0, %1, %20, %21, %0\n\tv_mad_u64_u32 %0, %1, %22, %23, %0\n\tv_mad_u64_u32 %0, %1, %24, %25, %0\n\tv_mad_u64_u32 %0, %1, %26, %27, %0\n\tv_mad_u64_u32 %0, %1, %28, %29, %0\n\tv_mad_u64_u32 %0, %1, %30, %31, %0\n\tv_mad_u64_u32 %0, %1, %32, %33, %0\n\tv_mad_u64_u32 %0, %1, %34, %35, %0\n\tv_mad_u64_u32 %0, %1, %36, %37, %0"
      : "+v"(acc), "=&s"(cc)
      : "v"(x[0]), "s"(w[8]), "v"(x[1]), "s"(w[7]), "v"(x[2]), "s"(w[6]),
        "v"(x[3]), "s"(w[5]), "v"(x[4]), "s"(w[4]), "v"(x[5]), "s"(w[3]),
        "v"(x[6]), "s"(w[2]), "v"(x[7]), "s"(w[1]), "v"(x[8]), "s"(w[0]),
        "v"(q[0]), "s"(pbar[8]), "v"(q[1]), "s"(pbar[7]), "v"(q[2]), "s"(pbar[6]),
        "v"(q[3]), "s"(pbar[5]), "v"(q[4]), "s"(pbar[4]), "v"(q[5]), "s"(pbar[3]),
        "v"(q[6]), "s"(pbar[2]), "v"(q[7]), "s"(pbar[1]), "v"(q[8]), "s"(pbar[0]));
  r[8] = (uint32_t)acc & kMask29;
}

__device__ __forceinline__ void mont29_a9(uint32_t (&r)[9], const uint32_t (&a)[9], const uint32_t (&b)[9],
                                          const Mod29<9>& M) {
  uint32_t m[9];
  uint64_t acc = 0, cc;
  asm("v_mad_u64_u32 %0, %1, %2, %3, %0"
      : "+v"(acc), "=&s"(cc)
      : "v"(a[0]), "v"(b[0]));
  m[0] = ((uint32_t)acc * M.pinv) & kMask29;
  asm("v_mad_u64_u32 %0, %1, %2, %3, %0"
      : "+v"(acc), "=&s"(cc)
      : "v"(m[0]), "s"(M.p[0]));
  acc >>= 29;
  asm("v_mad_u64_u32 %0, %1, %2, %3, %0\n\tv_mad_u64_u32 %0, %1, %4, %5, %0\n\tv_mad_u64_u32 %0, %1, %6, %7, %0"
      : "+v"(acc), "=&s"(cc)
      : "v"(a[0]), "v"(b[1]), "v"(a[1]), "v"(b[0]), "v"(m[0]), "s"(M.p[1]));
  m[1] = ((uint32_t)acc * M.pinv) & kMask29;
  asm("v_mad_u64_u32 %0, %1, %2, %3, %0"
      : "+v"(acc), "=&s"(cc)
      : "v"(m[1]), "s"(M.p[0]));
  acc >>= 29;
  asm("v_mad_u64_u32 %0, %1, %2, %3, %0\n\tv_mad_u64_u32 %0, %1, %4, %5, %0\n\tv_mad_u64_u32 %0, %1, %6, %7, %0\n\tv_mad_u64_u32 %0, %1, %8, %9, %0\n\tv_mad_u64_u32 %0, %1, %10, %11, %0"
      : "+v"(acc), "=&s"(cc)
      : "v"(a[0]), "v"(b[2]), "v"(a[1]), "v"(b[1]), "v"(a[2]), "v"(b[0]),
        "v"(m[0]), "s"(M.p[2]), "v"(m[1]), "s"(M.p[1]));
  m[2] = ((uint32_t)acc * M.pinv) & kMask29;
  asm("v_mad_u64_u32 %0, %1, %2, %3, %0"
      : "+v"(acc), "=&s"(cc)
      : "v"(m[2]), "s"(M.p[0]));
  acc >>= 29;
  asm("v_mad_u64_u32 %0, %1, %2, %3, %0\n\tv_mad_u64_u32 %0, %1, %4, %5, %0\n\tv_mad_u64_u32 %0, %1, %6, %7, %0\n\tv_mad_u64_u32 %0, %1, %8, %9, %0\n\tv_mad_u64_u32 %0, %1, %10, %11, %0\n\tv_mad_u64_u32 %0, %1, %12, %13, %0\n\tv_mad_u64_u32 %0, %1, %14, %15, %0"
      : "+v"(acc), "=&s"(cc)
      : "v"(a[0]), "v"(b[3]), "v"(a[1]), "v"(b[2]), "v"(a[2]), "v"(b[1]),
        "v"(a[3]), "v"(b[0]), "v"(m[0]), "s"(M.p[3]), "v"(m[1]), "s"(M.p[2]),
        "v"(m[2]), "s"(M.p[1]));
  m[3] = ((uint32_t)acc * M.pinv) & kMask29;
  asm("v_mad_u64_u32 %0, %1, %2, %3, %0"
      : "+v"(acc), "=&s"(cc)
      : "v"(m[3]), "s"(M.p[0]));
  acc >>= 29;
  asm("v_mad_u64_u32 %0, %1, %2, %3, %0\n\tv_mad_u64_u32 %0, %1, %4, %5, %0\n\tv_mad_u64_u32 %0, %1, %6, %7, %0\n\tv_mad_u64_u32 %0, %1, %8, %9, %0\n\tv_mad_u64_u32 %0, %1, %10, %11, %0\n\tv_mad_u64_u32 %0, %1, %12, %13, %0\n\tv_mad_u64_u32 %0, %1, %14, %15, %0\n\tv_mad_u64_u32 %0, %1, %16, %17, %0\n\tv_mad_u64_u32 %0, %1, %18, %19, %0"
      : "+v"(acc), "=&s"(cc)
      : "v"(a[0]), "v"(b[4]), "v"(a[1]), "v"(b[3]), "v"(a[2]), "v"(b[2]),
        "v"(a[3]), "v"(b[1]), "v"(a[4]), "v"(b[0]), "v"(m[0]), "s"(M.p[4]),
        "v"(m[1]), "s"(M.p[3]), "v"(m[2]), "s"(M.p[2]), "v"(m[3]), "s"(M.p[1]));
  m[4] = ((uint32_t)acc * M.pinv) & kMask29;
  asm("v_mad_u64_u32 %0, %1, %2, %3, %0"
      : "+v"(acc), "=&s"(cc)
      : "v"(m[4]), "s"(M.p[0]));
  acc >>= 29;
  asm("v_mad_u64_u32 %0, %1, %2, %3, %0\n\tv_mad_u64_u32 %0, %1, %4, %5, %0\n\tv_mad_u64_u32 %0, %1, %6, %7, %0\n\tv_mad_u64_u32 %0, %1, %8, %9, %0\n\tv_mad_u64_u32 %0, %1, %10, %11, %0\n\tv_mad_u64_u32 %0, %1, %12, %13, %0\n\tv_mad_u64_u32 %0, %1, %14, %15, %0\n\tv_mad_u64_u32 %0, %1, %16, %17, %0\n\tv_mad_u64_u32 %0, %1, %18, %19, %0\n\tv_mad_u64_u32 %0, %1, %20, %21, %0\n\tv_mad_u64_u32 %0, %1, %22, %23, %0"
      : "+v"(acc), "=&s"(cc)
      : "v"(a[0]), "v"(b[5]), "v"(a[1]), "v"(b[4]), "v"(a[2]), "v"(b[3]),
        "v"(a[3]), "v"(b[2]), "v"(a[4]), "v"(b[1]), "v"(a[5]), "v"(b[0]),
        "v"(m[0]), "s"(M.p[5]), "v"(m[1]), "s"(M.p[4]), "v"(m[2]), "s"(M.p[3]),
        "v"(m[3]), "s"(M.p[2]), "v"(m[4]), "s"(M.p[1]));
  m[5] = ((uint32_t)acc * M.pinv) & kMask29;
  asm("v_mad_u64_u32 %0, %1, %2, %3, %0"
      : "+v"(acc), "=&s"(cc)
      : "v"(m[5]), "s"(M.p[0]));
  acc >>= 29;
  asm("v_mad_u64_u32 %0, %1, %2, %3, %0\n\tv_mad_u64_u32 %0, %1, %4, %5, %0\n\tv_mad_u64_u32 %0, %1, %6, %7, %0\n\tv_mad_u64_u32 %0, %1, %8, %9, %0\n\tv_mad_u64_u32 %0, %1, %10, %11, %0\n\tv_mad_u64_u32 %0, %1, %12, %13, %0\n\tv_mad_u64_u32 %0, %1, %14, %15, %0\n\tv_mad_u64_u32 %0, %1, %16, %17, %0\n\tv_mad_u64_u32 %0, %1, %18, %19, %0\n\tv_mad_u64_u32 %0, %1, %20, %21, %0\n\tv_mad_u64_u32 %0, %1, %22, %23, %0\n\tv_mad_u64_u32 %0, %1, %24, %25, %0\n\tv_mad_u64_u32 %0, %1, %26, %27, %0"
      : "+v"(acc), "=&s"(cc)
      : "v"(a[0]), "v"(b[6]), "v"(a[1]), "v"(b[5]), "v"(a[2]), "v"(b[4]),
        "v"(a[3]), "v"(b[3]), "v"(a[4]), "v"(b[2]), "v"(a[5]), "v"(b[1]),
        "v"(a[6]), "v"(b[0]), "v"(m[0]), "s"(M.p[6]), "v"(m[1]), "s"(M.p[5]),
        "v"(m[2]), "s"(M.p[4]), "v"(m[3]), "s"(M.p[3]), "v"(m[4]), "s"(M.p[2]),
        "v"(m[5]), "s"(M.p[1]));
  m[6] = ((uint32_t)acc * M.pinv) & kMask29;
  asm("v_mad_u64_u32 %0, %1, %2, %3, %0"
      : "+v"(acc), "=&s"(cc)
      : "v"(m[6]), "s"(M.p[0]));
  acc >>= 29;
  asm("v_mad_u64_u32 %0, %1, %2, %3, %0\n\tv_mad_u64_u32 %0, %1, %4, %5, %0\n\tv_mad_u64_u32 %0, %1, %6, %7, %0\n\tv_mad_u64_u32 %0, %1, %8, %9, %0\n\tv_mad_u64_u32 %0, %1, %10, %11, %0\n\tv_mad_u64_u32 %0, %1, %12, %13, %0\n\tv_mad_u64_u32 %0, %1, %14, %15, %0\n\tv_mad_u64_u32 %0, %1, %16, %17, %0\n\tv_mad_u64_u32 %0, %1, %18, %19, %0\n\tv_mad_u64_u32 %0, %1, %20, %21, %0\n\tv_mad_u64_u32 %0, %1, %22, %23, %0\n\tv_mad_u64_u32 %0, %1, %24, %25, %0\n\tv_mad_u64_u32 %0, %1, %26, %27, %0\n\tv_mad_u64_u32 %0, %1, %28, %29, %0\n\tv_mad_u64_u32 %0, %1, %30, %31, %0"
      : "+v"(acc), "=&s"(cc)
      : "v"(a[0]), "v"(b[7]), "v"(a[1]), "v"(b[6]), "v"(a[2]), "v"(b[5]),
        "v"(a[3]), "v"(b[4]), "v"(a[4]), "v"(b[3]), "v"(a[5]), "v"(b[2]),
        "v"(a[6]), "v"(b[1]), "v"(a[7]), "v"(b[0]), "v"(m[0]), "s"(M.p[7]),
        "v"(m[1]), "s"(M.p[6]), "v"(m[2]), "s"(M.p[5]), "v"(m[3]), "s"(M.p[4]),
        "v"(m[4]), "s"(M.p[3]), "v"(m[5]), "s"(M.p[2]), "v"(m[6]), "s"(M.p[1]));
  m[7] = ((uint32_t)acc * M.pinv) & kMask29;
  asm("v_mad_u64_u32 %0, %1, %2, %3, %0"
      : "+v"(acc), "=&s"(cc)
      : "v"(m[7]), "s"(M.p[0]));
  acc >>= 29;
  asm("v_mad_u64_u32 %0, %1, %2, %3, %0\n\tv_mad_u64_u32 %0, %1, %4, %5, %0\n\tv_mad_u64_u32 %0, %1, %6, %7, %0\n\tv_mad_u64_u32 %0, %1, %8, %9, %0\n\tv_mad_u64_u32 %0, %1, %10, %11, %0\n\tv_mad_u64_u32 %0, %1, %12, %13, %0\n\tv_mad_u64_u32 %0, %1, %14, %15, %0\n\tv_mad_u64_u32 %0, %1, %16, %17, %0\n\tv_mad_u64_u32 %0, %1, %18, %19, %0\n\tv_mad_u64_u32 %0, %1, %20, %21, %0\n\tv_mad_u64_u32 %0, %1, %22, %23, %0\n\tv_mad_u64_u32 %0, %1, %24, %25, %0\n\tv_mad_u64_u32 %0, %1, %26, %27, %0\n\tv_mad_u64_u32 %0, %1, %28, %29, %0\n\tv_mad_u64_u32 %0, %1, %30, %31, %0\n\tv_mad_u64_u32 %0, %1, %32, %33, %0\n\tv_mad_u64_u32 %0, %1, %34, %35, %0"
      : "+v"(acc), "=&s"(cc)
      : "v"(a[0]), "v"(b[8]), "v"(a[1]), "v"(b[7]), "v"(a[2]), "v"(b[6]),
        "v"(a[3]), "v"(b[5]), "v"(a[4]), "v"(b[4]), "v"(a[5]), "v"(b[3]),
        "v"(a[6]), "v"(b[2]), "v"(a[7]), "v"(b[1]), "v"(a[8]), "v"(b[0]),
        "v"(m[0]), "s"(M.p[8]), "v"(m[1]), "s"(M.p[7]), "v"(m[2]), "s"(M.p[6]),
        "v"(m[3]), "s"(M.p[5]), "v"(m[4]), "s"(M.p[4]), "v"(m[5]), "s"(M.p[3]),
        "v"(m[6]), "s"(M.p[2]), "v"(m[7]), "s"(M.p[1]));
  m[8] = ((uint32_t)acc * M.pinv) & kMask29;
  asm("v_mad_u64_u32 %0, %1, %2, %3, %0"
      : "+v"(acc), "=&s"(cc)
      : "v"(m[8]), "s"(M.p[0]));
  acc >>= 29;
  asm("v_mad_u64_u32 %0, %1, %2, %3, %0\n\tv_mad_u64_u32 %0, %1, %4, %5, %0\n\tv_mad_u64_u32 %0, %1, %6, %7, %0\n\tv_mad_u64_u32 %0, %1, %8, %9, %0\n\tv_mad_u64_u32 %0, %1, %10, %11, %0\n\tv_mad_u64_u32 %0, %1, %12, %13, %0\n\tv_mad_u64_u32 %0, %1, %14, %15, %0\n\tv_mad_u64_u32 %0, %1, %16, %17, %0\n\tv_mad_u64_u32 %0, %1, %18, %19, %0\n\tv_mad_u64_u32 %0, %1, %20, %21, %0\n\tv_mad_u64_u32 %0, %1, %22, %23, %0\n\tv_mad_u64_u32 %0, %1, %24, %25, %0\n\tv_mad_u64_u32 %0, %1, %26, %27, %0\n\tv_mad_u64_u32 %0, %1, %28, %29, %0\n\tv_mad_u64_u32 %0, %1, %30, %31, %0\n\tv_mad_u64_u32 %0, %1, %32, %33, %0"
      : "+v"(acc), "=&s"(cc)
      : "v"(a[1]), "v"(b[8]), "v"(a[2]), "v"(b[7]), "v"(a[3]), "v"(b[6]),
        "v"(a[4]), "v"(b[5]), "v"(a[5]), "v"(b[4]), "v"(a[6]), "v"(b[3]),
        "v"(a[7]), "v"(b[2]), "v"(a[8]), "v"(b[1]), "v"(m[1]), "s"(M.p[8]),
        "v"(m[2]), "s"(M.p[7]), "v"(m[3]), "s"(M.p[6]), "v"(m[4]), "s"(M.p[5]),
        "v"(m[5]), "s"(M.p[4]), "v"(m[6]), "s"(M.p[3]), "v"(m[7]), "s"(M.p[2]),
        "v"(m[8]), "s"(M.p[1]));
  r[0] = (uint32_t)acc & kMask29;
  acc >>= 29;
  asm("v_mad_u64_u32 %0, %1, %2, %3, %0\n\tv_mad_u64_u32 %0, %1, %4, %5, %0\n\tv_mad_u64_u32 %0, %1, %6, %7, %0\n\tv_mad_u64_u32 %0, %1, %8, %9, %0\n\tv_mad_u64_u32 %0, %1, %10, %11, %0\n\tv_mad_u64_u32 %0, %1, %12, %13, %0\n\tv_mad_u64_u32 %0, %1, %14, %15, %0\n\tv_mad_u64_u32 %0, %1, %16, %17, %0\n\tv_mad_u64_u32 %0, %1, %18, %19, %0\n\tv_mad_u64_u32 %0, %1, %20, %21, %0\n\tv_mad_u64_u32 %0, %1, %22, %23, %0\n\tv_mad_u64_u32 %0, %1, %24, %25, %0\n\tv_mad_u64_u32 %0, %1, %26, %27, %0\n\tv_mad_u64_u32 %0, %1, %28, %29, %0"
      : "+v"(acc), "=&s"(cc)
      : "v"(a[2]), "v"(b[8]), "v"(a[3]), "v"(b[7]), "v"(a[4]), "v"(b[6]),
        "v"(a[5]), "v"(b[5]), "v"(a[6]), "v"(b[4]), "v"(a[7]), "v"(b[3]),
        "v"(a[8]), "v"(b[2]), "v"(m[2]), "s"(M.p[8]), "v"(m[3]), "s"(M.p[7]),
        "v"(m[4]), "s"(M.p[6]), "v"(m[5]), "s"(M.p[5]), "v"(m[6]), "s"(M.p[4]),
        "v"(m[7]), "s"(M.p[3]), "v"(m[8]), "s"(M.p[2]));
  r[1] = (uint32_t)acc & kMask29;
  acc >>= 29;
  asm("v_mad_u64_u32 %0, %1, %2, %3, %0\n\tv_mad_u64_u32 %0, %1, %4, %5, %0\n\tv_mad_u64_u32 %0, %1, %6, %7, %0\n\tv_mad_u64_u32 %0, %1, %8, %9, %0\n\tv_mad_u64_u32 %0, %1, %10, %11, %0\n\tv_mad_u64_u32 %0, %1, %12, %13, %0\n\tv_mad_u64_u32 %0, %1, %14, %15, %0\n\tv_mad_u64_u32 %0, %1, %16, %17, %0\n\tv_mad_u64_u32 %0, %1, %18, %19, %0\n\tv_mad_u64_u32 %0, %1, %20, %21, %0\n\tv_mad_u64_u32 %0, %1, %22, %23, %0\n\tv_mad_u64_u32 %0, %1, %24, %25, %0"
      : "+v"(acc), "=&s"(cc)
      : "v"(a[3]), "v"(b[8]), "v"(a[4]), "v"(b[7]), "v"(a[5]), "v"(b[6]),
        "v"(a[6]), "v"(b[5]), "v"(a[7]), "v"(b[4]), "v"(a[8]), "v"(b[3]),
        "v"(m[3]), "s"(M.p[8]), "v"(m[4]), "s"(M.p[7]), "v"(m[5]), "s"(M.p[6]),
        "v"(m[6]), "s"(M.p[5]), "v"(m[7]), "s"(M.p[4]), "v"(m[8]), "s"(M.p[3]));
  r[2] = (uint32_t)acc & kMask29;
  acc >>= 29;
  asm("v_mad_u64_u32 %0, %1, %2, %3, %0\n\tv_mad_u64_u32 %0, %1, %4, %5, %0\n\tv_mad_u64_u32 %0, %1, %6, %7, %0\n\tv_mad_u64_u32 %0, %1, %8, %9, %0\n\tv_mad_u64_u32 %0, %1, %10, %11, %0\n\tv_mad_u64_u32 %0, %1, %12, %13, %0\n\tv_mad_u64_u32 %0, %1, %14, %15, %0\n\tv_mad_u64_u32 %0, %1, %16, %17, %0\n\tv_mad_u64_u32 %0, %1, %18, %19, %0\n\tv_mad_u64_u32 %0, %1, %20, %21, %0"
      : "+v"(acc), "=&s"(cc)
      : "v"(a[4]), "v"(b[8]), "v"(a[5]), "v"(b[7]), "v"(a[6]), "v"(b[6]),
        "v"(a[7]), "v"(b[5]), "v"(a[8]), "v"(b[4]), "v"(m[4]), "s"(M.p[8]),
        "v"(m[5]), "s"(M.p[7]), "v"(m[6]), "s"(M.p[6]), "v"(m[7]), "s"(M.p[5]),
        "v"(m[8]), "s"(M.p[4]));
  r[3] = (uint32_t)acc & kMask29;
  acc >>= 29;
  asm("v_mad_u64_u32 %0, %1, %2, %3, %0\n\tv_mad_u64_u32 %0, %1, %4, %5, %0\n\tv_mad_u64_u32 %0, %1, %6, %7, %0\n\tv_mad_u64_u32 %0, %1, %8, %9, %0\n\tv_mad_u64_u32 %0, %1, %10, %11, %0\n\tv_mad_u64_u32 %0, %1, %12, %13, %0\n\tv_mad_u64_u32 %0, %1, %14, %15, %0\n\tv_mad_u64_u32 %0, %1, %16, %17, %0"
      : "+v"(acc), "=&s"(cc)
      : "v"(a[5]), "v"(b[8]), "v"(a[6]), "v"(b[7]), "v"(a[7]), "v"(b[6]),
        "v"(a[8]), "v"(b[5]), "v"(m[5]), "s"(M.p[8]), "v"(m[6]), "s"(M.p[7]),
        "v"(m[7]), "s"(M.p[6]), "v"(m[8]), "s"(M.p[5]));
  r[4] = (uint32_t)acc & kMask29;
  acc >>= 29;
  asm("v_mad_u64_u32 %0, %1, %2, %3, %0\n\tv_mad_u64_u32 %0, %1, %4, %5, %0\n\tv_mad_u64_u32 %0, %1, %6, %7, %0\n\tv_mad_u64_u32 %0, %1, %8, %9, %0\n\tv_mad_u64_u32 %0, %1, %10, %11, %0\n\tv_mad_u64_u32 %0, %1, %12, %13, %0"
      : "+v"(acc), "=&s"(cc)
      : "v"(a[6]), "v"(b[8]), "v"(a[7]), "v"(b[7]), "v"(a[8]), "v"(b[6]),
        "v"(m[6]), "s"(M.p[8]), "v"(m[7]), "s"(M.p[7]), "v"(m[8]), "s"(M.p[6]));
  r[5] = (uint32_t)acc & kMask29;
  acc >>= 29;
  asm("v_mad_u64_u32 %0, %1, %2, %3, %0\n\tv_mad_u64_u32 %0, %1, %4, %5, %0\n\tv_mad_u64_u32 %0, %1, %6, %7, %0\n\tv_mad_u64_u32 %0, %1, %8, %9, %0"
      : "+v"(acc), "=&s"(cc)
      : "v"(a[7]), "v"(b[8]), "v"(a[8]), "v"(b[7]), "v"(m[7]), "s"(M.p[8]),
        "v"(m[8]), "s"(M.p[7]));
  r[6] = (uint32_t)acc & kMask29;
  acc >>= 29;
  asm("v_mad_u64_u32 %0, %1, %2, %3, %0\n\tv_mad_u64_u32 %0, %1, %4, %5, %0"
      : "+v"(acc), "=&s"(cc)
      : "v"(a[8]), "v"(b[8]), "v"(m[8]), "s"(M.p[8]));
  r[7] = (uint32_t)acc & kMask29;
  acc >>= 29;
  r[8] = (uint32_t)acc & kMask29;
}
#else
F29_HD void mulc29_a9(uint32_t (&r)[9], const uint32_t (&x)[9], const uint32_t (&w)[9], const uint32_t (&ws)[9],
                       const uint32_t (&pbar)[9]) {
  mulc29<9>(r, x, w, ws, pbar);
}
F29_HD void mulc29_a9u(uint32_t (&r)[9], const uint32_t (&x)[9], const uint32_t (&w)[9], const uint32_t (&ws)[9],
                        const uint32_t (&pbar)[9]) {
  mulc29<9>(r, x, w, ws, pbar);
}
F29_HD void mont29_a9(uint32_t (&r)[9], const uint32_t (&a)[9], const uint32_t (&b)[9], const Mod29<9>& M) {
  mont29<9>(r, a, b, M);
}
#endif
}
```

ntt_amd/csrc/ntt_kernels_impl.hpp:

```cpp
#pragma once
#include <cstdlib>
#include <utility>

#include "ntt_kernels.hpp"

namespace ntt {


template <class F, int... I>
__device__ __forceinline__ void static_for_impl(F&& f, std::integer_sequence<int, I...>) {
  (f(std::integral_constant<int, I>{}), ...);
}
template <int N, class F>
__device__ __forceinline__ void static_for(F&& f) {
  static_for_impl(f, std::make_integer_sequence<int, N>{});
}

template <int LO, class F, int... I>
hipError_t with_radix_impl(int logr, F&& f, std::integer_sequence<int, I...>) {
  hipError_t e = hipErrorInvalidValue;
  (void)((logr == LO + I ? (e = f(std::integral_constant<int, LO + I>{}), true) : false) || ...);
  return e;
}
template <int LO, int HI, class F>
hipError_t with_radix(int logr, F&& f) {
  return with_radix_impl<LO>(logr, f, std::make_integer_sequence<int, HI - LO + 1>{});
}

__host__ __device__ constexpr int brev_bits(int v, int bits) {
  int r = 0;
  for (int i = 0; i < bits; ++i) r |= ((v >> i) & 1) << (bits - 1 - i);
  return r;
}

template <int LOGR, int QB>
struct Sched {
  static constexpr int nsub = (LOGR + QB - 1) / QB;
  static constexpr int qb(int s) { return (LOGR - QB * s) >= QB ? QB : (LOGR - QB * s); }
  static constexpr int logN(int s) { return LOGR - QB * s; }
  static constexpr int logsig(int s) { return logN(s) - qb(s); }
};
template <class E>
constexpr int ept_log() { return E::EPT >= 8 ? 3 : (E::EPT == 4 ? 2 : 1); }

template <int LOGR, int QB>
__device__ __forceinline__ uint32_t natural_index(uint32_t pi) {
  using S = Sched<LOGR, QB>;
  uint32_t k = 0;
#pragma unroll
  for (int s = 0; s < S::nsub; ++s) {
    const uint32_t ks = (pi >> S::logsig(s)) & ((1u << S::qb(s)) - 1);
    k |= ks << (QB * s);
  }
  return k;
}

template <class E, int Q, int base, int N>
__device__ __forceinline__ void dft_q(uint32_t (&x)[N][E::W], const typename E::Args& F) {
  constexpr int K1 = E::IN, K2 = 2 * E::IN, K3 = 4 * E::IN;
  if constexpr (Q == 2) {
    E::template bfly_l<K1>(x[base], x[base + 1], F);
  } else if constexpr (Q == 4) {
    E::template bfly_l<K1>(x[base], x[base + 2], F);
    E::template bfly_w_l<K1>(x[base + 1], x[base + 3], F.w8[1], F);
    E::template bfly_l<K2>(x[base], x[base + 1], F);
    E::template bfly_l<K2>(x[base + 2], x[base + 3], F);
  } else {
    static_assert(Q == 8, "radix");
    E::template bfly_l<K1>(x[base], x[base + 4], F);
    E::template bfly_w_l<K1>(x[base + 1], x[base + 5], F.w8[0], F);
    E::template bfly_w_l<K1>(x[base + 2], x[base + 6], F.w8[1], F);
    E::template bfly_w_l<K1>(x[base + 3], x[base + 7], F.w8[2], F);
    E::template bfly_l<K2>(x[base], x[base + 2], F);
    E::template bfly_w_l<K2>(x[base + 1], x[base + 3], F.w8[1], F);
    E::template bfly_l<K2>(x[base + 4], x[base + 6], F);
    E::template bfly_w_l<K2>(x[base + 5], x[base + 7], F.w8[1], F);
    E::template bfly_l<K3>(x[base], x[base + 1], F);
    E::template bfly_l<K3>(x[base + 2], x[base + 3], F);
    E::template bfly_l<K3>(x[base + 4], x[base + 5], F);
    E::template bfly_l<K3>(x[base + 6], x[base + 7], F);
  }
}

template <class E, int Q, int base, int N>
__device__ __forceinline__ void dft_q_fast(uint32_t (&x)[N][E::W], const typename E::Args& F) {
  if constexpr (Q == 2) {
    E::template bfly_raw<E::PC_5_29>(x[base], x[base + 1], F);
  } else if constexpr (Q == 4) {
    E::template bfly_raw<E::PC_5_29>(x[base], x[base + 2], F);
    E::template bfly_raw_w<E::PC_5_29>(x[base + 1], x[base + 3], F.w8[1], F);
    E::template bfly_raw<E::PC_9_30>(x[base], x[base + 1], F);
    E::template bfly_raw<E::PC_4_29>(x[base + 2], x[base + 3], F);
  } else {
    static_assert(Q == 8, "radix");
    E::template bfly_raw<E::PC_5_29>(x[base], x[base + 4], F);
    E::template bfly_raw_w<E::PC_5_29>(x[base + 1], x[base + 5], F.w8[0], F);
    E::template bfly_raw_w<E::PC_5_29>(x[base + 2], x[base + 6], F.w8[1], F);
    E::template bfly_raw_w<E::PC_5_29>(x[base + 3], x[base + 7], F.w8[2], F);
    E::template bfly_raw<E::PC_9_30>(x[base], x[base + 2], F);
    E::template bfly_raw_w<E::PC_9_30>(x[base + 1], x[base + 3], F.w8[1], F);
    E::template bfly_raw<E::PC_4_29>(x[base + 4], x[base + 6], F);
    E::template bfly_raw_w<E::PC_4_29>(x[base + 5], x[base + 7], F.w8[1], F);
    E::norm(x[base]);
    E::norm(x[base + 1]);
    E::norm(x[base + 2]);
    E::norm(x[base + 4]);
    E::norm(x[base + 6]);
    E::template bfly_raw<E::PC_17_29>(x[base], x[base + 1], F);
    E::template bfly_raw<E::PC_4_29>(x[base + 2], x[base + 3], F);
    E::template bfly_raw<E::PC_7_30>(x[base + 4], x[base + 5], F);
    E::template bfly_raw<E::PC_4_29>(x[base + 6], x[base + 7], F);
  }
}
template <class E, int Q, int base, bool FAST, int N>
__device__ __forceinline__ void dft(uint32_t (&x)[N][E::W], const typename E::Args& F) {
  if constexpr (FAST)
    dft_q_fast<E, Q, base>(x, F);
  else
    dft_q<E, Q, base>(x, F);
}

template <class E>
__device__ __forceinline__ void twiddle_mul(uint32_t (&x)[E::W], const uint32_t* tab, uint32_t e,
                                            const typename E::Args& F) {
  typename E::Tw w;
  E::tload(w, tab, e);
  E::mul(x, w, F);
}
template <class E>
__device__ __forceinline__ void twiddle_mul_lds(uint32_t (&x)[E::W], const uint32_t* lds_tw, uint32_t e,
                                                const typename E::Args& F) {
  typename E::Tw w;
  E::tload_lds(w, lds_tw, e);
  E::mul(x, w, F);
}

template <int T>
__device__ __forceinline__ uint32_t lds_slot(uint32_t c, uint32_t pi) {
  if constexpr (T == 1)
    return pi ^ (((pi >> 4) ^ (pi >> 8)) & 15u);
  else
    return (c ^ (pi & (T - 1))) + T * pi;
}

#ifndef NTT_UNIFORM_CP
#define NTT_UNIFORM_CP 1
#endif
template <int LOGR, int QB, int NT, int s>
struct Uniform {
  using S = Sched<LOGR, QB>;
  static constexpr int sb = S::logsig(s);
  static constexpr bool on = NTT_UNIFORM_CP && s > 0 && s + 1 < S::nsub && sb >= 1 && (1 << sb) <= NT / 64;
};
template <int LOGR, int QB, int T, int NT, int EPT, int s>
__device__ __forceinline__ void sub_map(uint32_t t, int j, uint32_t rot, uint32_t& c, uint32_t& g) {
  using U = Uniform<LOGR, QB, NT, s>;
  if constexpr (U::on) {
    constexpr int sb = U::sb, G = EPT >> Sched<LOGR, QB>::qb(s);
    const uint32_t wave = t >> 6, lane = t & 63;
    const uint32_t cp = (wave + rot) & ((1u << sb) - 1);
    const uint32_t u = ((((wave >> sb) << 6) | lane)) + (uint32_t)(NT >> sb) * (uint32_t)j;
    (void)G;
    c = u % T;
    g = ((u / T) << sb) | cp;
  } else {
    const uint32_t lam = t + NT * j;
    c = lam % T;
    g = lam / T;
  }
}

template <class E, int LOGR, int T, int TE, int NT, int s, bool FAST, bool R32, bool LTW>
__device__ __forceinline__ void substage(uint32_t (&x)[E::EPT][E::W], uint32_t (&cl)[E::EPT / 2],
                                         uint32_t (&pil)[E::EPT / 2], uint32_t* lds, const PassArgs<E>& A, int t,
                                         const uint32_t* lds_tw, uint32_t rot) {
  using S = Sched<LOGR, ept_log<E>()>;
  constexpr int EPT = E::EPT;
  constexpr int pqb = S::qb(s - 1), PQ = 1 << pqb, PG = EPT / PQ, psb = S::logsig(s - 1), plN = S::logN(s - 1);
  constexpr int qb = S::qb(s), Q = 1 << qb, G = EPT / Q, sb = S::logsig(s), lN = S::logN(s);
  static_for<1>([&](auto) {
    if constexpr (s > 1) __syncthreads();
    static_for<PG>([&](auto J) {
      constexpr int j = J;
      const uint32_t g = pil[j];
      const uint32_t rho = g >> psb, cp = g & ((1u << psb) - 1);
      static_for<PQ>([&](auto K) {
        constexpr int k = K;
        const uint32_t pi = (rho << plN) + cp + (k << psb);
        lds_put<E::LDSW, TE>(lds, lds_slot<T>(cl[j], pi), x[j * PQ + brev_bits(k, pqb)]);
      });
    });
    __syncthreads();
    static_for<G>([&](auto J) {
      constexpr int j = J;
      uint32_t c, g;
      sub_map<LOGR, ept_log<E>(), T, NT, EPT, s>(t, j, rot, c, g);
      const uint32_t rho = g >> sb, cp = g & ((1u << sb) - 1);
      static_for<Q>([&](auto D) {
        constexpr int d = D;
        const uint32_t pi = (rho << lN) + cp + (d << sb);
        lds_get<E::LDSW, TE>(x[j * Q + d], lds, lds_slot<T>(c, pi));
      });
    });
  });
  static_for<G>([&](auto J) {
    constexpr int j = J;
    uint32_t c, g;
    sub_map<LOGR, ept_log<E>(), T, NT, EPT, s>(t, j, rot, c, g);
    cl[j] = c;
    pil[j] = g;
  });
  static_for<G>([&](auto J) {
    constexpr int j = J;
    dft<E, Q, j * Q, FAST>(x, A.F);
    if constexpr (s + 1 < S::nsub) {
      E::template reduce<E::IN * Q, E::IN, FAST, R32>(x[j * Q], A.F);
      const uint32_t cp = pil[j] & ((1u << sb) - 1);
      auto twiddles = [&]() {
        static_for<Q - 1>([&](auto K1) {
          constexpr int k = K1 + 1;
          if constexpr (LTW)
            twiddle_mul_lds<E>(x[j * Q + brev_bits(k, qb)], lds_tw, (cp * k) << (LOGR - lN), A.F);
          else
            twiddle_mul<E>(x[j * Q + brev_bits(k, qb)], A.tw_int, (cp * k) << (LOGR - lN), A.F);
        });
      };
      if constexpr (Uniform<LOGR, ept_log<E>(), NT, s>::on) {
        const uint32_t cps = __builtin_amdgcn_readfirstlane(cp);
        if (cps == 0) {
          static_for<Q - 1>([&](auto K1) {
            E::template reduce<E::IN * Q, E::IN, FAST, R32>(x[j * Q + brev_bits(K1 + 1, qb)], A.F);
          });
        } else if constexpr (E::SGPR_TW && !LTW) {
          static_for<Q - 1>([&](auto K1) {
            constexpr int k = K1 + 1;
            typename E::Tw w;
            E::tload_u(w, A.tw_int, (cps * k) << (LOGR - lN));
            E::mul_u(x[j * Q + brev_bits(k, qb)], w, A.F);
          });
        } else {
          twiddles();
        }
      } else {
        twiddles();
      }
    }
  });
}

enum : int { PRO_NONE = 0, PRO_PW = 1, PRO_COSET = 2, PRO_LDE = 3 };
#ifndef NTT_COL_R32_BELOW
#define NTT_COL_R32_BELOW 9
#endif
template <class E>
__device__ __forceinline__ void ipn_signal_read(const PassArgs<E>& A, uint32_t mid) {
  asm volatile("s_waitcnt vmcnt(0)" ::: "memory");
  __syncthreads();
  uint32_t* line = A.ipn_sync + 32 * (1 + mid);
  if (threadIdx.x == 0 && __hip_atomic_fetch_add(line, 1u, __ATOMIC_RELAXED, __HIP_MEMORY_SCOPE_AGENT) == A.ipn_strips - 1)
    __hip_atomic_store(line + 1, 1u, __ATOMIC_RELAXED, __HIP_MEMORY_SCOPE_AGENT);
}
__device__ __forceinline__ void watchdog_trip(const Watchdog& wd) {
  if (wd.abort) __hip_atomic_store(wd.abort, 1u, __ATOMIC_RELAXED, __HIP_MEMORY_SCOPE_AGENT);
  if (wd.report) __hip_atomic_store(wd.report, 1u, __ATOMIC_RELAXED, __HIP_MEMORY_SCOPE_SYSTEM);
}
template <int S0, uint32_t N0, int S1, uint32_t N1, int S2>
__device__ __forceinline__ bool poll_bounded(uint32_t* word, const Watchdog& wd) {
  typedef __attribute__((address_space(1))) uint32_t gu32;
  gu32* const g = (gu32*)word;
  gu32* const ab = (gu32*)wd.abort;
  for (uint32_t spins = 0;; ++spins) {
    if (__hip_atomic_load(g, __ATOMIC_RELAXED, __HIP_MEMORY_SCOPE_AGENT)) return true;
    if (spins >= wd.spins) {
      watchdog_trip(wd);
      return false;
    }
    if ((spins & 255u) == 255u && ab && __hip_atomic_load(ab, __ATOMIC_RELAXED, __HIP_MEMORY_SCOPE_AGENT)) return false;
    if (spins < N0) __builtin_amdgcn_s_sleep(S0);
    else if (spins < N1) __builtin_amdgcn_s_sleep(S1);
    else __builtin_amdgcn_s_sleep(S2);
  }
}
template <class E>
__device__ __forceinline__ bool ipn_wait_mirror(const PassArgs<E>& A, uint32_t midrev) {
  __shared__ uint32_t s_ok;
  if (threadIdx.x == 0)
    s_ok = poll_bounded<4, 8, 32, 8, 32>(A.ipn_sync + 32 * (1 + midrev) + 1, A.wd) ? 1u : 0u;
  __syncthreads();
  return __builtin_amdgcn_readfirstlane(s_ok) != 0u;
}

__device__ __forceinline__ bool grid_barrier_words(uint32_t* top, uint32_t* shards, uint32_t* go, uint32_t k,
                                                   const Watchdog& wd) {
  asm volatile("s_waitcnt vmcnt(0)" ::: "memory");
  __syncthreads();
  __shared__ uint32_t s_ok;
  if (threadIdx.x == 0) {
    const uint32_t G = gridDim.x, sh = blockIdx.x & 7u;
    const uint32_t ns = (G + 7u - sh) >> 3, nsh = G < 8u ? G : 8u;
    if (__hip_atomic_fetch_add(shards + 32 * sh, 1u, __ATOMIC_RELAXED, __HIP_MEMORY_SCOPE_AGENT) == k * ns - 1 &&
        __hip_atomic_fetch_add(top, 1u, __ATOMIC_RELAXED, __HIP_MEMORY_SCOPE_AGENT) == k * nsh - 1)
      __hip_atomic_store(go, 1u, __ATOMIC_RELAXED, __HIP_MEMORY_SCOPE_AGENT);
    s_ok = poll_bounded<4, 16, 32, 16, 32>(go, wd) ? 1u : 0u;
    __builtin_amdgcn_fence(__ATOMIC_ACQUIRE, "agent");
    asm volatile("s_waitcnt vmcnt(0)" ::: "memory");
  }
  __syncthreads();
  return __builtin_amdgcn_readfirstlane(s_ok) != 0u;
}
template <uint32_t K, class E>
__device__ __forceinline__ bool ipn_grid_barrier(const PassArgs<E>& A) {
  return grid_barrier_words(A.ipn_sync, A.ipn_shards, A.ipn_go, K, A.wd);
}

__device__ __forceinline__ void residency_arrive(uint32_t* top, uint32_t* shards, uint32_t* go) {
  if (threadIdx.x == 0) {
    const uint32_t G = gridDim.x, sh = blockIdx.x & 7u;
    const uint32_t ns = (G + 7u - sh) >> 3, nsh = G < 8u ? G : 8u;
    if (__hip_atomic_fetch_add(shards + 32 * sh, 1u, __ATOMIC_RELAXED, __HIP_MEMORY_SCOPE_AGENT) == ns - 1 &&
        __hip_atomic_fetch_add(top, 1u, __ATOMIC_RELAXED, __HIP_MEMORY_SCOPE_AGENT) == nsh - 1) {
      uint32_t zero = 0u;
      __hip_atomic_compare_exchange_strong(go, &zero, 1u, __ATOMIC_RELAXED, __ATOMIC_RELAXED, __HIP_MEMORY_SCOPE_AGENT);
    }
  }
}
__device__ __forceinline__ bool residency_wait(uint32_t* go, const Watchdog& wd) {
  __shared__ uint32_t s_go;
  if (threadIdx.x == 0) {
    typedef __attribute__((address_space(1))) uint32_t gu32;
    uint32_t v = 0;
    for (uint32_t spins = 0;; ++spins) {
      v = __hip_atomic_load((gu32*)go, __ATOMIC_RELAXED, __HIP_MEMORY_SCOPE_AGENT);
      if (v) break;
      if (spins >= wd.spins) {
        uint32_t cur = 0u;
        if (__hip_atomic_compare_exchange_strong(go, &cur, 2u, __ATOMIC_RELAXED, __ATOMIC_RELAXED,
                                                 __HIP_MEMORY_SCOPE_AGENT)) {
          watchdog_trip(wd);
          v = 2u;
        } else {
          v = cur;
        }
        break;
      }
      if (spins < 16) __builtin_amdgcn_s_sleep(4);
      else __builtin_amdgcn_s_sleep(32);
    }
    s_go = v;
  }
  __syncthreads();
  return __builtin_amdgcn_readfirstlane(s_go) == 1u;
}
__device__ __forceinline__ bool residency_went(uint32_t* go) {
  __shared__ uint32_t s_go;
  if (threadIdx.x == 0) s_go = __hip_atomic_load(go, __ATOMIC_RELAXED, __HIP_MEMORY_SCOPE_AGENT);
  __syncthreads();
  return __builtin_amdgcn_readfirstlane(s_go) == 1u;
}

template <class E, int LOGR, int KIND>
__host__ __device__ constexpr int pass_tile_te() {
  return (KIND == KIND_SINGLE) ? (1 << LOGR) : (1 << tile_log_of<E>());
}
template <class E, int LOGR, int KIND>
__host__ __device__ constexpr int pass_lds_words() {
  return pass_tile_te<E, LOGR, KIND>() * E::LDSW;
}
template <class E, int KIND, bool FULLTW>
__host__ __device__ constexpr bool pass_ltw() {
  return E::LDS_TW && !(KIND == KIND_COLUMN && !FULLTW);
}

enum : int { IPN_NONE = 0, IPN_SLAB = 1, IPN_FUSED3 = 2, IPN_FUSED2 = 3, IPN_RESIDENCY = 4 };
constexpr bool TW_FULL = true, TW_TWO_LEVEL = false;
constexpr bool RED_FAST = true, RED_GENERIC = false;
constexpr bool SRC_CALLER = true, SRC_SCRATCH = false;
enum : int { FSM_NONE = 0, FSM_MAPS = 1, FSM_EPILOGUE = 2 };
constexpr bool OUTER_SHOUP = true, OUTER_MONT = false;
constexpr bool STORE_WT = true, STORE_PLAIN = false;
constexpr bool TILE_LOOPED = true, TILE_ONCE = false;
constexpr bool STRIP_FORM = true;
template <class E, int LOGR, int KIND, bool FULLTW, bool FAST, int PRO = PRO_NONE, bool SRC_USER = true,
          int FSM = 0, bool SHTW = false, bool WT = false, bool LOOPED = false, int IPN = 0, bool MAT = false>
__device__ __forceinline__ void pass_tile(const uint32_t* __restrict__ src, uint32_t* __restrict__ dst,
                                          const PassArgs<E>& A, const uint32_t w, const uint32_t bq,
                                          uint32_t* __restrict__ lds, uint32_t* __restrict__ lds_tw) {
  static_assert(!SHTW || (FULLTW && KIND == KIND_COLUMN), "Shoup pairs: a column pass's full table");
  static_assert(!WT || KIND == KIND_COLUMN, "write-through stores: scratch");
  static_assert(IPN == IPN_NONE || (IPN == IPN_RESIDENCY ? KIND == KIND_COLUMN && WT : KIND == KIND_FINAL), "IPN forms");
  constexpr int QB = ept_log<E>(), EPT = E::EPT;
  using S = Sched<LOGR, QB>;
  constexpr bool COLLIKE = KIND == KIND_COLUMN || KIND == KIND_STOCKHAM || KIND == KIND_DIT;
  constexpr bool ROWS = KIND == KIND_ROWS;
  constexpr int TE = pass_tile_te<E, LOGR, KIND>();
  constexpr int T = TE >> LOGR;
  constexpr bool R32 = KIND != KIND_COLUMN || LOGR < NTT_COL_R32_BELOW;
  constexpr int NT = TE / EPT;
  static_assert(LOGR >= QB && T >= 1, "radix");
  constexpr bool LTW = pass_ltw<E, KIND, FULLTW>();

  constexpr int SW = (KIND == KIND_COLUMN) ? (SRC_USER ? E::MEMW : E::SCRW) : (KIND == KIND_FINAL ? E::SCRW : E::MEMW);
  constexpr int DW = (KIND == KIND_COLUMN) ? E::SCRW : E::MEMW;

  int t = threadIdx.x;
  if constexpr (LOOPED) asm volatile("" : "+v"(t));
  if (t >= NT) return;
  constexpr bool IN_USER = (KIND == KIND_COLUMN && SRC_USER) || KIND == KIND_SINGLE || ROWS;
  constexpr bool EPI = FSM == 2 && KIND != KIND_COLUMN;
  static_assert(!MAT || ((KIND == KIND_COLUMN || KIND == KIND_FINAL) && FSM == 1 && !FULLTW && IPN == 0), "strip form");
  const bool fs_il = MAT || (FSM > 0 && (A.fs & FS_IL) != 0);
  const bool map_in = !MAT && FSM > 0 && IN_USER && (A.fs & FS_MAP_IN);
  const bool map_out = !MAT && FSM > 0 && KIND != KIND_COLUMN && (A.fs & FS_MAP_OUT);
  const bool single_il = (KIND == KIND_SINGLE || ROWS) && fs_il;
  const size_t tstride = A.batch_stride / E::MEMW;
  const size_t bidx = MAT ? 0 : (size_t)bq * tstride;
  if constexpr (MAT) {}
  else if constexpr (PRO == PRO_LDE) src += (size_t)bq * A.src_stride;
  else if (!map_in && !single_il) src += bidx * SW;
  if (!map_out && !single_il) dst += bidx * DW;
  const size_t boff = bidx * E::MEMW;
  auto in_pos = [&](size_t pos, size_t b) -> size_t {
    if (single_il) pos = (pos << A.il) + b;
    else if (ROWS && !map_in) pos += b * tstride;
    if (!map_in) return pos;
    return A.min(pos, fs_il ? 0 : b);
  };
  auto out_pos = [&](size_t pos, size_t b) -> size_t {
    if (single_il) pos = (pos << A.il) + b;
    else if (ROWS && !map_out) pos += b * tstride;
    if (!map_out) return pos;
    return A.mout(pos, fs_il ? 0 : b);
  };
  auto epi_idx = [&](size_t pos, size_t b) -> size_t {
    if (!fs_il) return (b << A.log_n) + pos;
    if (single_il) pos = (pos << A.il) + b;
    return (A.fs & FS_MAP_EPI) ? A.mepi(pos, 0) : pos;
  };
  auto mat_at = [&](size_t P, size_t& at, bool rev = false) -> bool {
    const uint32_t col = (bq << A.il) + (uint32_t)(P & ((1u << A.il) - 1));
    uint32_t row = (uint32_t)(P >> A.il);
    if (rev) row = __builtin_bitreverse32(row) >> (32 - A.log_n);
    at = (size_t)row * A.mat_w + col;
    return col < A.mat_w;
  };
  auto mat_mul_out = [&]([[maybe_unused]] uint32_t (&v)[E::W], [[maybe_unused]] uint32_t row) {
    if constexpr (MAT) {
      typename E::Tw tl, th;
      E::tload(tl, A.tw_in, row & ((1u << A.lo_bits) - 1));
      E::tload(th, A.tw_in_hi, row >> A.lo_bits);
      E::mul(tl.w, th, A.F);
      E::mulv(v, tl.w, A.F);
    }
  };
  auto ck = [&](size_t i, [[maybe_unused]] size_t lim) -> size_t {
#if NTT_DEBUG_CHECKS
    if (i >= lim) {
      ntt_dbg_flag(A.F.dbg, NTT_DBG_BOUNDS);
      return 0;
    }
#endif
    return i;
  };

  size_t colbase = 0;
  uint32_t col0 = 0;
  uint32_t mid = 0, k10 = 0, midrev = 0;
  uint32_t b0 = 0, tb_log = 0;
  if constexpr (COLLIKE) {
    const uint32_t log_s = A.log_blk - LOGR;
    const uint32_t groups_log = log_s - __builtin_ctz(T);
    const size_t blk = w >> groups_log;
    col0 = (w & ((1u << groups_log) - 1)) * T;
    colbase = (blk << A.log_blk) + col0;
  } else if constexpr (KIND == KIND_FINAL) {
    const uint32_t w1_log = A.log_n - A.r1 - LOGR;
    mid = w & ((1u << w1_log) - 1);
    if (fs_il) {
      constexpr uint32_t tl = __builtin_ctz(T);
      tb_log = tl < A.il ? tl : A.il;
      const uint32_t tk_log = tl - tb_log;
      const uint32_t rest = w >> w1_log;
      k10 = (rest & ((1u << (A.r1 - tk_log)) - 1)) << tk_log;
      b0 = (rest >> (A.r1 - tk_log)) << tb_log;
    } else {
      k10 = (w >> w1_log) * T;
    }
    uint32_t m = mid;
    for (uint32_t i = 0; i < A.nmid; ++i) {
      const uint32_t d = m & ((1u << A.mid_bits[i]) - 1);
      m >>= A.mid_bits[i];
      midrev |= d << A.mid_off[i];
    }
  }
  const uint32_t log_s = COLLIKE ? (A.log_blk - LOGR) : 0u;

  uint32_t x[EPT][E::W];
  uint32_t cl[EPT / 2];
  uint32_t pil[EPT / 2];

  constexpr int TWWORDS = LTW ? (1 << LOGR) * E::TW : 1;
  uint32_t stw[LTW ? (TWWORDS + NT - 1) / NT : 1];
  if constexpr (LTW && S::nsub > 1) {
    static_for<(TWWORDS + NT - 1) / NT>([&](auto I) {
      constexpr int i = I;
      stw[i] = (t + NT * i < TWWORDS) ? A.tw_int[t + NT * i] : 0u;
    });
  }
  {
    constexpr int qb = S::qb(0), Q = 1 << qb, G = EPT / Q, sb = S::logsig(0);
    static_for<G>([&](auto J) {
      constexpr int j = J;
      const uint32_t lam = t + NT * j;
      uint32_t c, g;
      if constexpr (COLLIKE) {
        c = lam % T;
        g = lam / T;
      } else {
        g = lam & ((1u << sb) - 1);
        c = lam >> sb;
      }
      cl[j] = c;
      pil[j] = g;
      static_for<Q>([&](auto D) {
        constexpr int d = D;
        const uint32_t pi = g + (d << sb);
        size_t pos;
        if constexpr (COLLIKE) {
          pos = colbase + c + ((size_t)pi << log_s);
        } else if constexpr (KIND == KIND_FINAL) {
          if (fs_il) {
            const uint32_t k1 = k10 + (c >> tb_log), b = b0 + (c & ((1u << tb_log) - 1));
            const size_t beta = ((size_t)k1 << (A.log_n - A.r1 - LOGR)) + mid;
            pos = (((beta << LOGR) + pi) << A.il) + b;
          } else {
            const size_t beta = ((size_t)(k10 + c) << (A.log_n - A.r1 - LOGR)) + mid;
            pos = (beta << LOGR) + pi;
          }
        } else {
          pos = pi;
        }
        const size_t b = ROWS ? (size_t)w * T + c : (size_t)bq;
        if constexpr (PRO == PRO_LDE) {
          static_assert((FSM == 0 || MAT) && SRC_USER && (KIND == KIND_SINGLE || KIND == KIND_COLUMN), "PRO_LDE passes");
          size_t at = pos;
          bool have = true;
          if constexpr (MAT) {
            have = mat_at(pos, at);
            pos >>= A.il;
          }
          if (have && pos < A.src_stride / E::MEMW) {
            E::template load<SW>(x[j * Q + d], src, ck(at, A.dbg_src_n));
#if NTT_DEBUG_CHECKS
            if (!E::dbg_canonical(x[j * Q + d], A.F)) ntt_dbg_flag(A.F.dbg, NTT_DBG_INPUT);
#endif
            if constexpr (KIND == KIND_COLUMN && FULLTW) {
              if (A.tw_in) {
                typename E::Tw u;
                E::tload(u, A.tw_in, pi);
                E::mul(x[j * Q + d], u, A.F);
              }
            } else if constexpr (lde_mul_at_load<E, KIND>()) {
              if (A.tw_in) {
                typename E::Tw tl, th;
                E::tload(tl, A.tw_in, (uint32_t)(pos & ((1u << A.lo_bits) - 1)));
                E::tload(th, A.tw_in_hi, (uint32_t)(pos >> A.lo_bits));
                E::mul(tl.w, th, A.F);
                E::mulv(x[j * Q + d], tl.w, A.F);
              }
            }
          } else {
#pragma unroll
            for (int l = 0; l < E::W; ++l) x[j * Q + d][l] = 0u;
          }
        } else if constexpr (MAT) {
          size_t at;
          if (mat_at(pos, at, KIND == KIND_COLUMN && (A.mat_ops & MAT_REV_IN))) {
            E::template load<SW>(x[j * Q + d], src, ck(at, A.dbg_src_n));
#if NTT_DEBUG_CHECKS
            if (KIND == KIND_COLUMN && A.src_user) {
              if (!E::dbg_canonical(x[j * Q + d], A.F)) ntt_dbg_flag(A.F.dbg, NTT_DBG_INPUT);
            }
#endif
          } else {
#pragma unroll
            for (int l = 0; l < E::W; ++l) x[j * Q + d][l] = 0u;
          }
        } else {
          E::template load<SW>(x[j * Q + d], src, ck(IN_USER ? in_pos(pos, b) : pos, A.dbg_src_n));
#if NTT_DEBUG_CHECKS
          if (KIND == KIND_SINGLE || ROWS || (KIND == KIND_COLUMN && A.src_user)) {
            if (!E::dbg_canonical(x[j * Q + d], A.F)) ntt_dbg_flag(A.F.dbg, NTT_DBG_INPUT);
          }
#endif
        }
        if constexpr ((KIND == KIND_STOCKHAM || KIND == KIND_DIT) && FULLTW) {
          uint32_t tw[E::W];
          const uint32_t k0 = col0 & ((1u << A.lgp) - 1);
          E::template load<E::TABW>(tw, A.tw_full, ((size_t)k0 << LOGR) + pi * T + c);
          E::mulv(x[j * Q + d], tw, A.F);
        }
        if constexpr (PRO == PRO_PW) {
          uint32_t y[E::W];
          E::load(y, A.src2 + boff, in_pos(pos, b));
          E::mulv(x[j * Q + d], y, A.F);
        } else if constexpr (PRO == PRO_COSET) {
          typename E::Tw u;
          E::tload(u, A.tw_in, pi);
          E::mul(x[j * Q + d], u, A.F);
        }
      });
    });
    static_for<G>([&](auto J) {
      constexpr int j = J;
      dft<E, Q, j * Q, FAST>(x, A.F);
      if constexpr (S::nsub > 1) {
        E::template reduce<E::IN * Q, E::IN, FAST, R32>(x[j * Q], A.F);
        static_for<Q - 1>([&](auto K1) {
          constexpr int k = K1 + 1;
          twiddle_mul<E>(x[j * Q + brev_bits(k, qb)], A.tw_int, pil[j] * k, A.F);
        });
      }
    });
    if constexpr (LTW && S::nsub > 1) {
      static_for<(TWWORDS + NT - 1) / NT>([&](auto I) {
        constexpr int i = I;
        if (t + NT * i < TWWORDS) lds_tw[t + NT * i] = stw[i];
      });
    }
  }

  if constexpr (IPN == IPN_SLAB) ipn_signal_read(A, mid);

  if constexpr (S::nsub > 1) substage<E, LOGR, T, TE, NT, 1, FAST, R32, LTW>(x, cl, pil, lds, A, t, lds_tw, w);
  if constexpr (S::nsub > 2) substage<E, LOGR, T, TE, NT, 2, FAST, R32, LTW>(x, cl, pil, lds, A, t, lds_tw, w);
  if constexpr (S::nsub > 3) substage<E, LOGR, T, TE, NT, 3, FAST, R32, LTW>(x, cl, pil, lds, A, t, lds_tw, w);
  if constexpr (S::nsub > 4) substage<E, LOGR, T, TE, NT, 4, FAST, R32, LTW>(x, cl, pil, lds, A, t, lds_tw, w);
  if constexpr (S::nsub > 5) substage<E, LOGR, T, TE, NT, 5, FAST, R32, LTW>(x, cl, pil, lds, A, t, lds_tw, w);
  static_assert(S::nsub <= 6, "sub-stages");

  if constexpr (IPN == IPN_SLAB) {
    if (!ipn_wait_mirror(A, midrev)) return;
  } else if constexpr (IPN == IPN_FUSED3 || IPN == IPN_FUSED2) {
    if (!ipn_grid_barrier<IPN == IPN_FUSED3 ? FUSED3BI_BARRIERS : FUSED2BI_BARRIERS>(A)) return;
  } else if constexpr (IPN == IPN_RESIDENCY) {
    if (!residency_wait(A.ipn_go, A.wd)) return;
  }
  {
    constexpr int ls = S::nsub - 1;
    constexpr int qb = S::qb(ls), Q = 1 << qb, G = EPT / Q, sb = S::logsig(ls), lN = S::logN(ls);
    static_for<G>([&](auto J) {
      constexpr int j = J;
      const uint32_t g = pil[j];
      const uint32_t rho = g >> sb, cp = g & ((1u << sb) - 1);
      const uint32_t c = cl[j];
      static_for<Q>([&](auto K) {
        constexpr int k = K;
        uint32_t(&v)[E::W] = x[j * Q + brev_bits(k, qb)];
        const uint32_t pi = (rho << lN) + cp + (k << sb);
        const uint32_t kn = natural_index<LOGR, QB>(pi);
        size_t pos;
        if constexpr (KIND == KIND_DIT) {
          pos = colbase + c + ((size_t)kn << log_s);
          E::template store<E::IN * Q, FAST, DW>(dst, ck(pos, A.dbg_dst_n), v, A.F);
        } else if constexpr (KIND == KIND_STOCKHAM) {
          const uint32_t idx = col0 + c, kk = idx & ((1u << A.lgp) - 1);
          pos = ((size_t)(idx - kk) << LOGR) + kk + ((size_t)kn << A.lgp);
          E::template store<E::IN * Q, FAST, DW>(dst, ck(pos, A.dbg_dst_n), v, A.F);
        } else if constexpr (KIND == KIND_COLUMN) {
          if constexpr (FULLTW) {
            uint32_t tw[E::W];
            size_t ti = ((size_t)col0 << LOGR) + (kn * T + c);
            if (fs_il) {
              const uint32_t tc = (col0 + c) >> A.il;
              ti = ((size_t)(tc & ~(uint32_t)(T - 1)) << LOGR) + kn * T + (tc & (T - 1));
            }
            if constexpr (SHTW) {
              typename E::Tw tws;
              E::tload(tws, A.tw_full, ti);
              E::mul(v, tws, A.F);
            } else {
              E::template load<E::TABW>(tw, A.tw_full, ti);
              E::mulv(v, tw, A.F);
            }
          } else {
            const size_t e = ((size_t)((col0 + c) >> A.il) * kn) << A.log_m;
            typename E::Tw tl, th;
            E::tload(tl, A.tw_lo, (uint32_t)(e & ((1u << A.lo_bits) - 1)));
            E::tload(th, A.tw_hi, (uint32_t)(e >> A.lo_bits));
            E::mul(tl.w, th, A.F);
            E::mulv(v, tl.w, A.F);
          }
          pos = colbase + c + ((size_t)kn << log_s);
          if constexpr (MAT) {
            size_t at;
            if (mat_at(pos, at, (A.mat_ops & MAT_REV_OUT) != 0)) {
              if constexpr (PRO == PRO_NONE) {
                if (A.mat_ops & MAT_MUL_OUT) mat_mul_out(v, (uint32_t)(pos >> A.il));
              }
              E::template store_lazy<E::MUL_OUT, FAST, DW, WT>(dst, ck(at, A.dbg_dst_n), v, A.F);
            }
          } else {
            E::template store_lazy<E::MUL_OUT, FAST, DW, WT>(dst, ck(pos, A.dbg_dst_n), v, A.F);
          }
        } else if constexpr (KIND == KIND_FINAL) {
          if (fs_il) {
            const uint32_t k1 = k10 + (c >> tb_log), b = b0 + (c & ((1u << tb_log) - 1));
            pos = (((size_t)k1 + ((size_t)midrev << A.r1) + ((size_t)kn << (A.log_n - LOGR))) << A.il) + b;
          } else if (!IPN && (A.flags & 2u)) {
            pos = ((size_t)(k10 + c) << (A.log_n - A.r1)) + ((size_t)mid << LOGR) + kn;
          } else {
            pos = (size_t)(k10 + c) + ((size_t)midrev << A.r1) + ((size_t)kn << (A.log_n - LOGR));
          }
          if constexpr (EPI) {
            uint32_t tw[E::W];
            E::template load<E::TABW>(tw, A.tw_epi, epi_idx(pos, bq));
            E::mulv(v, tw, A.F);
            E::template store<E::MUL_OUT, FAST, DW>(dst, ck(out_pos(pos, bq), A.dbg_dst_n), v, A.F);
          } else if constexpr (MAT) {
            size_t at;
            if (mat_at(pos, at, (A.mat_ops & MAT_REV_OUT) != 0)) {
              if (A.mat_ops & MAT_MUL_OUT) {
                mat_mul_out(v, (uint32_t)(pos >> A.il));
                E::template store<E::MUL_OUT, FAST, DW>(dst, ck(at, A.dbg_dst_n), v, A.F);
              } else {
                E::template store<E::IN * Q, FAST, DW>(dst, ck(at, A.dbg_dst_n), v, A.F);
              }
            }
          } else {
            E::template store<E::IN * Q, FAST, DW>(dst, ck(out_pos(pos, bq), A.dbg_dst_n), v, A.F);
          }
        } else {
          pos = kn;
          const size_t b = ROWS ? (size_t)w * T + c : (size_t)bq;
          if constexpr (EPI) {
            if (A.flags & 1u) E::mul(v, A.F.ninv, A.F);
            uint32_t tw[E::W];
            E::template load<E::TABW>(tw, A.tw_epi, epi_idx(pos, b));
            E::mulv(v, tw, A.F);
            E::template store<E::MUL_OUT, FAST>(dst, ck(out_pos(pos, b), A.dbg_dst_n), v, A.F);
          } else if (A.flags & 1u) {
            E::mul(v, A.F.ninv, A.F);
            E::template store<E::MUL_OUT, FAST>(dst, ck(out_pos(pos, b), A.dbg_dst_n), v, A.F);
          } else {
            E::template store<E::IN * Q, FAST>(dst, ck(out_pos(pos, b), A.dbg_dst_n), v, A.F);
          }
        }
      });
    });
  }
}

template <class E, int LOGR, int KIND, bool FULLTW, bool FAST, int PRO = PRO_NONE, bool SRC_USER = true,
          int FSM = 0, bool SHTW = false>
__global__ __launch_bounds__((1 << E::TILE_LOG) / E::EPT) __attribute__((amdgpu_waves_per_eu(E::WAVES_PER_EU)))
void k_pass(const uint32_t* __restrict__ src, uint32_t* __restrict__ dst, const PassArgs<E> A) {
  __shared__ __attribute__((aligned(16))) uint32_t lds[pass_lds_words<E, LOGR, KIND>()];
  __shared__ __attribute__((aligned(16))) uint32_t lds_tw[pass_ltw<E, KIND, FULLTW>() ? (1 << LOGR) * E::TW : 1];
  uint32_t w = blockIdx.x;
  if (A.flags & 4u) {
    const uint32_t G = gridDim.x;
    if ((G & 7u) == 0) w = (w & 7u) * (G >> 3) + (w >> 3);
  }
  pass_tile<E, LOGR, KIND, FULLTW, FAST, PRO, SRC_USER, FSM, SHTW>(src, dst, A, w, blockIdx.y, lds, lds_tw);
}

template <class E, int LOGR, int KIND, bool FULLTW, bool FAST, int FSM>
static hipError_t launch_plain(const uint32_t* src, uint32_t* dst, const PassArgs<E>& A, dim3 g, dim3 b,
                               hipStream_t st) {
  if constexpr (KIND == KIND_COLUMN && FULLTW && FAST && E::SHOUP_OUTER) {
    if (A.tw_sh) {
      constexpr bool SU = E::SCRW == E::MEMW;
      if (A.src_user && !SU) return hipErrorInvalidValue;
      hipLaunchKernelGGL((k_pass<E, LOGR, KIND, true, true, PRO_NONE, SU, FSM, true>), g, b, 0, st, src, dst, A);
      return hipGetLastError();
    }
  }
  if (A.tw_sh) return hipErrorInvalidValue;
  if constexpr (KIND == KIND_COLUMN && E::SCRW != E::MEMW) {
    if (!A.src_user) {
      hipLaunchKernelGGL((k_pass<E, LOGR, KIND, FULLTW, FAST, PRO_NONE, false, FSM>), g, b, 0, st, src, dst, A);
      return hipGetLastError();
    }
  }
  hipLaunchKernelGGL((k_pass<E, LOGR, KIND, FULLTW, FAST, PRO_NONE, true, FSM>), g, b, 0, st, src, dst, A);
  return hipGetLastError();
}

template <class E, int KIND, int LOGR, bool FULLTW, bool FAST>
static hipError_t launch_fsm(const uint32_t* src, uint32_t* dst, const PassArgs<E>& A, dim3 g, dim3 b,
                             hipStream_t st) {
  if constexpr (KIND == KIND_STOCKHAM || KIND == KIND_DIT) {
    if (A.fs || A.tw_epi) return hipErrorInvalidValue;
    return launch_plain<E, LOGR, KIND, FULLTW, FAST, 0>(src, dst, A, g, b, st);
  }
  if (A.fs == 0 && !A.tw_epi) return launch_plain<E, LOGR, KIND, FULLTW, FAST, 0>(src, dst, A, g, b, st);
  if constexpr (KIND != KIND_COLUMN) {
    if (A.tw_epi) return launch_plain<E, LOGR, KIND, FULLTW, FAST, 2>(src, dst, A, g, b, st);
  }
  return launch_plain<E, LOGR, KIND, FULLTW, FAST, 1>(src, dst, A, g, b, st);
}

template <class E, int KIND, int LOGR>
static hipError_t launch_pass_r(const uint32_t* src, uint32_t* dst, const PassArgs<E>& A, uint32_t grid,
                                uint32_t batch, hipStream_t st) {
  constexpr int TL = tile_log_of<E>();
  constexpr int MAXR = (KIND == KIND_SINGLE || KIND == KIND_ROWS) ? TL : TL - E::MIN_COLS_LOG;
  constexpr bool ROWS_OFF = KIND == KIND_ROWS && (!HasRows<E>::value || LOGR < kRowsMinLog ||
                                                  LOGR > rows_max_log<E>() || LOGR >= TL);
  if constexpr (LOGR > MAXR || ROWS_OFF || ((KIND == KIND_STOCKHAM || KIND == KIND_DIT) && !HasStockham<E>::value)) {
    return hipErrorInvalidValue;
  } else {
    constexpr int TE = (KIND == KIND_SINGLE) ? (1 << LOGR) : (1 << TL);
    constexpr int NT = TE / E::EPT;
    const dim3 g(grid, batch), b(NT < 64 ? 64 : NT);
    if constexpr (E::FASTRED) {
      if (A.F.red_ok) {
        if constexpr (KIND == KIND_STOCKHAM || KIND == KIND_DIT) {
          return A.tw_full ? launch_fsm<E, KIND, LOGR, true, true>(src, dst, A, g, b, st)
                           : launch_fsm<E, KIND, LOGR, false, true>(src, dst, A, g, b, st);
        }
        if constexpr (KIND == KIND_COLUMN) {
          if (A.tw_full && A.src2) {
            if (A.fs)
              hipLaunchKernelGGL((k_pass<E, LOGR, KIND, true, true, PRO_PW, true, 1>), g, b, 0, st, src, dst, A);
            else
              hipLaunchKernelGGL((k_pass<E, LOGR, KIND, true, true, PRO_PW>), g, b, 0, st, src, dst, A);
            return hipGetLastError();
          }
          if (A.tw_full && A.tw_in) {
            if (A.fs) return hipErrorInvalidValue;
            hipLaunchKernelGGL((k_pass<E, LOGR, KIND, true, true, PRO_COSET>), g, b, 0, st, src, dst, A);
            return hipGetLastError();
          }
          if (A.tw_full) return launch_fsm<E, KIND, LOGR, true, true>(src, dst, A, g, b, st);
        }
        if (A.src2 || A.tw_in) return hipErrorInvalidValue;
        return launch_fsm<E, KIND, LOGR, false, true>(src, dst, A, g, b, st);
      }
    }
    if (A.src2 || A.tw_in) return hipErrorInvalidValue;
    if constexpr (KIND == KIND_ROWS && E::FASTRED) {
      return hipErrorInvalidValue;
    } else {
      if constexpr (KIND == KIND_COLUMN || KIND == KIND_STOCKHAM || KIND == KIND_DIT) {
        if (A.tw_full) return launch_fsm<E, KIND, LOGR, true, false>(src, dst, A, g, b, st);
      }
      return launch_fsm<E, KIND, LOGR, false, false>(src, dst, A, g, b, st);
    }
  }
}

template <class E, int KIND>
hipError_t launch_pass_kind(int logr, const uint32_t* src, uint32_t* dst, const PassArgs<E>& A, uint32_t grid,
                                uint32_t batch, hipStream_t st) {
  return with_radix<3, 13>(logr, [&](auto R) { return launch_pass_r<E, KIND, R>(src, dst, A, grid, batch, st); });
}

template <class E>
hipError_t launch_pass(int kind, int logr, const uint32_t* src, uint32_t* dst, const PassArgs<E>& A, uint32_t grid,
                       uint32_t batch, hipStream_t st) {
  if (kind == KIND_COLUMN) return launch_pass_kind<E, KIND_COLUMN>(logr, src, dst, A, grid, batch, st);
  if (kind == KIND_FINAL) return launch_pass_kind<E, KIND_FINAL>(logr, src, dst, A, grid, batch, st);
  if (kind == KIND_STOCKHAM || kind == KIND_DIT) {
    if constexpr (HasStockham<E>::value) {
      if (kind == KIND_DIT) return launch_pass_kind<E, KIND_DIT>(logr, src, dst, A, grid, batch, st);
      return launch_pass_kind<E, KIND_STOCKHAM>(logr, src, dst, A, grid, batch, st);
    }
    return hipErrorInvalidValue;
  }
  if (kind == KIND_ROWS) {
    if constexpr (HasRows<E>::value) return launch_pass_kind<E, KIND_ROWS>(logr, src, dst, A, grid, batch, st);
    return hipErrorInvalidValue;
  }
  return launch_pass_kind<E, KIND_SINGLE>(logr, src, dst, A, grid, batch, st);
}

#define NTT_INSTANTIATE_KIND(E, KIND)                                                                          \
  template hipError_t launch_pass_kind<E, KIND>(int, const uint32_t*, uint32_t*, const PassArgs<E>&, uint32_t, \
                                                uint32_t, hipStream_t);

#define NTT_EXTERN_KIND(E, KIND)                                                                                     \
  extern template hipError_t launch_pass_kind<E, KIND>(int, const uint32_t*, uint32_t*, const PassArgs<E>&, uint32_t, \
                                                       uint32_t, hipStream_t);

#define NTT_INSTANTIATE(E)                                                                                         \
  NTT_EXTERN_KIND(E, KIND_COLUMN)                                                                                  \
  NTT_EXTERN_KIND(E, KIND_FINAL)                                                                                   \
  NTT_EXTERN_KIND(E, KIND_SINGLE)                                                                                  \
  NTT_EXTERN_KIND(E, KIND_STOCKHAM)                                                                                \
  NTT_EXTERN_KIND(E, KIND_DIT)                                                                                     \
  template hipError_t launch_pass<E>(int, int, const uint32_t*, uint32_t*, const PassArgs<E>&, uint32_t, uint32_t, \
                                     hipStream_t);

}
```

Measured before the change: 11.05 billion.

## Use signed lazy butterflies with signed Shoup twiddle products for 256-bit radix-4

Adds a signed-limb lazy representation for the 9-limb BN254 engine. Radix-2/4 butterflies drop the padded-modulus correction on the difference and let limbs go negative. A new signed Shoup multiply built on v_mad_i64_i32 consumes these signed values directly, and non-multiplied slots are re-biased with a padded constant before reduce or store. The aim is to cut per-limb add instructions in the FFT core at the cost of a new multiply routine with different bound assumptions, plus a risk of correctness edge cases in the signed bounds.

```diff
diff --git a/ntt_amd/csrc/eng29_args.hpp b/ntt_amd/csrc/eng29_args.hpp
--- a/ntt_amd/csrc/eng29_args.hpp
+++ b/ntt_amd/csrc/eng29_args.hpp
@@ -18,6 +18,7 @@
   }
   for (int i = 0; i < L; ++i) A.M.p2[i] = A.kp[1][i];
   neg29<L>(A.pbar, A.M.p);
+  for (int i = 0; i < L; ++i) A.np[i] = 0u - A.M.p[i];
   uint32_t inv = 1;
   for (int i = 0; i < 5; ++i) inv *= 2 - p[0] * inv;
   A.M.pinv = (0u - inv) & kMask29;
diff --git a/ntt_amd/csrc/engines.hpp b/ntt_amd/csrc/engines.hpp
--- a/ntt_amd/csrc/engines.hpp
+++ b/ntt_amd/csrc/engines.hpp
@@ -25,6 +25,9 @@
 #endif
 #ifndef NTT_256_PASS1_TABLE
 #define NTT_256_PASS1_TABLE 1
+#endif
+#ifndef NTT_SIGNED_LAZY
+#define NTT_SIGNED_LAZY 1
 #endif
 #ifndef NTT_P_SCRATCH32
 #define NTT_P_SCRATCH32 1
@@ -103,6 +106,7 @@
   static constexpr bool LDS_TW = false;
   static constexpr bool SGPR_TW = (L == 9);
   static constexpr bool FASTRED = 29 * L - 18 <= 255;
+  static constexpr bool SIGNED_LAZY = NTT_SIGNED_LAZY && L == 9 && EPT == 4;
   struct Tw {
     uint32_t w[L];
     uint32_t ws[L];
@@ -116,6 +120,7 @@
     float red_inv;
     uint32_t red_ok;
     uint32_t pc[5][L];
+    uint32_t np[L];
     uint32_t* dbg;
   };
   __device__ static bool dbg_below(const uint32_t (&x)[W], const uint32_t (&q)[L]) {
@@ -260,6 +265,25 @@
 #pragma unroll
     for (int i = 0; i < W; ++i) x[i] = r[i];
   }
+  __device__ static __forceinline__ void mul_s(uint32_t (&x)[W], const Tw& t, const Args& A) {
+    static_assert(L == 9, "signed product: 256-bit class");
+    uint32_t r[W];
+    mulc29_s9(r, x, t.w, t.ws, A.np);
+#pragma unroll
+    for (int i = 0; i < W; ++i) x[i] = r[i];
+  }
+  __device__ static __forceinline__ void mul_us(uint32_t (&x)[W], const Tw& t, const Args& A) {
+    static_assert(L == 9, "signed product: 256-bit class");
+    uint32_t r[W];
+    mulc29_s9u(r, x, t.w, t.ws, A.np);
+#pragma unroll
+    for (int i = 0; i < W; ++i) x[i] = r[i];
+  }
+  static constexpr int UNSIGNED_BOUND = 32;
+  __device__ static __forceinline__ void unsign(uint32_t (&x)[W], const Args& A) {
+#pragma unroll
+    for (int i = 0; i < L; ++i) x[i] += A.pc[PC_9_30][i];
+  }
   __device__ static __forceinline__ void mul_u(uint32_t (&x)[W], const Tw& t, const Args& A) {
     uint32_t r[W];
     if constexpr (L == 9)
@@ -313,6 +337,19 @@
                                                     const Args& A) {
     bfly_raw<CI>(a, b, A);
     mul_u(b, t, A);
+  }
+  __device__ static __forceinline__ void bfly_sgn(uint32_t (&a)[W], uint32_t (&b)[W]) {
+#pragma unroll
+    for (int i = 0; i < L; ++i) {
+      const uint32_t x = a[i], y = b[i];
+      a[i] = x + y;
+      b[i] = x - y;
+    }
+  }
+  __device__ static __forceinline__ void bfly_sgn_w(uint32_t (&a)[W], uint32_t (&b)[W], const Tw& t,
+                                                    const Args& A) {
+    bfly_sgn(a, b);
+    mul_us(b, t, A);
   }
   __device__ static __forceinline__ void norm(uint32_t (&x)[W]) {
     norm_u<L>(x);
diff --git a/ntt_amd/csrc/field29.hpp b/ntt_amd/csrc/field29.hpp
--- a/ntt_amd/csrc/field29.hpp
+++ b/ntt_amd/csrc/field29.hpp
@@ -270,6 +270,33 @@
   }
 }
 
+constexpr int64_t kShoupBiasS = ((int64_t)1 << 55) + ((int64_t)1 << 33);
+template <int L>
+F29_HD void mulc29_s(uint32_t (&r)[L], const uint32_t (&x)[L], const uint32_t (&w)[L], const uint32_t (&ws)[L],
+                     const uint32_t (&np)[L]) {
+  uint32_t q[L];
+  int64_t acc = -kShoupBiasS;
+#pragma unroll
+  for (int k = L - 2; k < 2 * L - 1; ++k) {
+#pragma unroll
+    for (int i = (k - (L - 1) > 0 ? k - (L - 1) : 0); i <= (k < L - 1 ? k : L - 1); ++i)
+      acc += (int64_t)(int32_t)x[i] * (int32_t)ws[k - i];
+    if (k >= L) q[k - L] = (uint32_t)acc & kMask29;
+    acc >>= 29;
+  }
+  q[L - 1] = (uint32_t)acc;
+  acc = 0;
+#pragma unroll
+  for (int k = 0; k < L; ++k) {
+#pragma unroll
+    for (int i = 0; i <= k; ++i) acc += (int64_t)(int32_t)x[i] * (int32_t)w[k - i];
+#pragma unroll
+    for (int i = 0; i <= k; ++i) acc += (int64_t)(int32_t)q[i] * (int32_t)np[k - i];
+    r[k] = (uint32_t)acc & kMask29;
+    acc >>= 29;
+  }
+}
+
 template <int L>
 F29_HD void mulc29_cc(uint32_t (&r)[L], const uint32_t (&x)[L], const uint32_t (&w)[L], const uint32_t (&ws)[L],
                    const uint32_t (&pbar)[L]) {
diff --git a/ntt_amd/csrc/field29_asm9.hpp b/ntt_amd/csrc/field29_asm9.hpp
--- a/ntt_amd/csrc/field29_asm9.hpp
+++ b/ntt_amd/csrc/field29_asm9.hpp
@@ -431,6 +431,278 @@
   acc >>= 29;
   r[8] = (uint32_t)acc & kMask29;
 }
+
+__device__ __forceinline__ void mulc29_s9(uint32_t (&r)[9], const uint32_t (&x)[9], const uint32_t (&w)[9],
+                                          const uint32_t (&ws)[9], const uint32_t (&np)[9]) {
+  uint32_t q[9];
+  int64_t acc = -kShoupBiasS;
+  uint64_t cc;
+  asm("v_mad_i64_i32 %0, %1, %2, %3, %0\n\tv_mad_i64_i32 %0, %1, %4, %5, %0\n\tv_mad_i64_i32 %0, %1, %6, %7, %0\n\tv_mad_i64_i32 %0, %1, %8, %9, %0\n\tv_mad_i64_i32 %0, %1, %10, %11, %0\n\tv_mad_i64_i32 %0, %1, %12, %13, %0\n\tv_mad_i64_i32 %0, %1, %14, %15, %0\n\tv_mad_i64_i32 %0, %1, %16, %17, %0"
+      : "+v"(acc), "=&s"(cc)
+      : "v"(x[0]), "v"(ws[7]), "v"(x[1]), "v"(ws[6]), "v"(x[2]), "v"(ws[5]),
+        "v"(x[3]), "v"(ws[4]), "v"(x[4]), "v"(ws[3]), "v"(x[5]), "v"(ws[2]),
+        "v"(x[6]), "v"(ws[1]), "v"(x[7]), "v"(ws[0]));
+  acc >>= 29;
+  asm("v_mad_i64_i32 %0, %1, %2, %3, %0\n\tv_mad_i64_i32 %0, %1, %4, %5, %0\n\tv_mad_i64_i32 %0, %1, %6, %7, %0\n\tv_mad_i64_i32 %0, %1, %8, %9, %0\n\tv_mad_i64_i32 %0, %1, %10, %11, %0\n\tv_mad_i64_i32 %0, %1, %12, %13, %0\n\tv_mad_i64_i32 %0, %1, %14, %15, %0\n\tv_mad_i64_i32 %0, %1, %16, %17, %0\n\tv_mad_i64_i32 %0, %1, %18, %19, %0"
+      : "+v"(acc), "=&s"(cc)
+      : "v"(x[0]), "v"(ws[8]), "v"(x[1]), "v"(ws[7]), "v"(x[2]), "v"(ws[6]),
+        "v"(x[3]), "v"(ws[5]), "v"(x[4]), "v"(ws[4]), "v"(x[5]), "v"(ws[3]),
+        "v"(x[6]), "v"(ws[2]), "v"(x[7]), "v"(ws[1]), "v"(x[8]), "v"(ws[0]));
+  acc >>= 29;
+  asm("v_mad_i64_i32 %0, %1, %2, %3, %0\n\tv_mad_i64_i32 %0, %1, %4, %5, %0\n\tv_mad_i64_i32 %0, %1, %6, %7, %0\n\tv_mad_i64_i32 %0, %1, %8, %9, %0\n\tv_mad_i64_i32 %0, %1, %10, %11, %0\n\tv_mad_i64_i32 %0, %1, %12, %13, %0\n\tv_mad_i64_i32 %0, %1, %14, %15, %0\n\tv_mad_i64_i32 %0, %1, %16, %17, %0"
+      : "+v"(acc), "=&s"(cc)
+      : "v"(x[1]), "v"(ws[8]), "v"(x[2]), "v"(ws[7]), "v"(x[3]), "v"(ws[6]),
+        "v"(x[4]), "v"(ws[5]), "v"(x[5]), "v"(ws[4]), "v"(x[6]), "v"(ws[3]),
+        "v"(x[7]), "v"(ws[2]), "v"(x[8]), "v"(ws[1]));
+  q[0] = (uint32_t)acc & kMask29;
+  acc >>= 29;
+  asm("v_mad_i64_i32 %0, %1, %2, %3, %0\n\tv_mad_i64_i32 %0, %1, %4, %5, %0\n\tv_mad_i64_i32 %0, %1, %6, %7, %0\n\tv_mad_i64_i32 %0, %1, %8, %9, %0\n\tv_mad_i64_i32 %0, %1, %10, %11, %0\n\tv_mad_i64_i32 %0, %1, %12, %13, %0\n\tv_mad_i64_i32 %0, %1, %14, %15, %0"
+      : "+v"(acc), "=&s"(cc)
+      : "v"(x[2]), "v"(ws[8]), "v"(x[3]), "v"(ws[7]), "v"(x[4]), "v"(ws[6]),
+        "v"(x[5]), "v"(ws[5]), "v"(x[6]), "v"(ws[4]), "v"(x[7]), "v"(ws[3]),
+        "v"(x[8]), "v"(ws[2]));
+  q[1] = (uint32_t)acc & kMask29;
+  acc >>= 29;
+  asm("v_mad_i64_i32 %0, %1, %2, %3, %0\n\tv_mad_i64_i32 %0, %1, %4, %5, %0\n\tv_mad_i64_i32 %0, %1, %6, %7, %0\n\tv_mad_i64_i32 %0, %1, %8, %9, %0\n\tv_mad_i64_i32 %0, %1, %10, %11, %0\n\tv_mad_i64_i32 %0, %1, %12, %13, %0"
+      : "+v"(acc), "=&s"(cc)
+      : "v"(x[3]), "v"(ws[8]), "v"(x[4]), "v"(ws[7]), "v"(x[5]), "v"(ws[6]),
+        "v"(x[6]), "v"(ws[5]), "v"(x[7]), "v"(ws[4]), "v"(x[8]), "v"(ws[3]));
+  q[2] = (uint32_t)acc & kMask29;
+  acc >>= 29;
+  asm("v_mad_i64_i32 %0, %1, %2, %3, %0\n\tv_mad_i64_i32 %0, %1, %4, %5, %0\n\tv_mad_i64_i32 %0, %1, %6, %7, %0\n\tv_mad_i64_i32 %0, %1, %8, %9, %0\n\tv_mad_i64_i32 %0, %1, %10, %11, %0"
+      : "+v"(acc), "=&s"(cc)
+      : "v"(x[4]), "v"(ws[8]), "v"(x[5]), "v"(ws[7]), "v"(x[6]), "v"(ws[6]),
+        "v"(x[7]), "v"(ws[5]), "v"(x[8]), "v"(ws[4]));
+  q[3] = (uint32_t)acc & kMask29;
+  acc >>= 29;
+  asm("v_mad_i64_i32 %0, %1, %2, %3, %0\n\tv_mad_i64_i32 %0, %1, %4, %5, %0\n\tv_mad_i64_i32 %0, %1, %6, %7, %0\n\tv_mad_i64_i32 %0, %1, %8, %9, %0"
+      : "+v"(acc), "=&s"(cc)
+      : "v"(x[5]), "v"(ws[8]), "v"(x[6]), "v"(ws[7]), "v"(x[7]), "v"(ws[6]),
+        "v"(x[8]), "v"(ws[5]));
+  q[4] = (uint32_t)acc & kMask29;
+  acc >>= 29;
+  asm("v_mad_i64_i32 %0, %1, %2, %3, %0\n\tv_mad_i64_i32 %0, %1, %4, %5, %0\n\tv_mad_i64_i32 %0, %1, %6, %7, %0"
+      : "+v"(acc), "=&s"(cc)
+      : "v"(x[6]), "v"(ws[8]), "v"(x[7]), "v"(ws[7]), "v"(x[8]), "v"(ws[6]));
+  q[5] = (uint32_t)acc & kMask29;
+  acc >>= 29;
+  asm("v_mad_i64_i32 %0, %1, %2, %3, %0\n\tv_mad_i64_i32 %0, %1, %4, %5, %0"
+      : "+v"(acc), "=&s"(cc)
+      : "v"(x[7]), "v"(ws[8]), "v"(x[8]), "v"(ws[7]));
+  q[6] = (uint32_t)acc & kMask29;
+  acc >>= 29;
+  asm("v_mad_i64_i32 %0, %1, %2, %3, %0"
+      : "+v"(acc), "=&s"(cc)
+      : "v"(x[8]), "v"(ws[8]));
+  q[7] = (uint32_t)acc & kMask29;
+  acc >>= 29;
+  q[8] = (uint32_t)acc;
+  acc = 0;
+  asm("v_mad_i64_i32 %0, %1, %2, %3, %0\n\tv_mad_i64_i32 %0, %1, %4, %5, %0"
+      : "+v"(acc), "=&s"(cc)
+      : "v"(x[0]), "v"(w[0]), "v"(q[0]), "s"(np[0]));
+  r[0] = (uint32_t)acc & kMask29;
+  acc >>= 29;
+  asm("v_mad_i64_i32 %0, %1, %2, %3, %0\n\tv_mad_i64_i32 %0, %1, %4, %5, %0\n\tv_mad_i64_i32 %0, %1, %6, %7, %0\n\tv_mad_i64_i32 %0, %1, %8, %9, %0"
+      : "+v"(acc), "=&s"(cc)
+      : "v"(x[0]), "v"(w[1]), "v"(x[1]), "v"(w[0]), "v"(q[0]), "s"(np[1]),
+        "v"(q[1]), "s"(np[0]));
+  r[1] = (uint32_t)acc & kMask29;
+  acc >>= 29;
+  asm("v_mad_i64_i32 %0, %1, %2, %3, %0\n\tv_mad_i64_i32 %0, %1, %4, %5, %0\n\tv_mad_i64_i32 %0, %1, %6, %7, %0\n\tv_mad_i64_i32 %0, %1, %8, %9, %0\n\tv_mad_i64_i32 %0, %1, %10, %11, %0\n\tv_mad_i64_i32 %0, %1, %12, %13, %0"
+      : "+v"(acc), "=&s"(cc)
+      : "v"(x[0]), "v"(w[2]), "v"(x[1]), "v"(w[1]), "v"(x[2]), "v"(w[0]),
+        "v"(q[0]), "s"(np[2]), "v"(q[1]), "s"(np[1]), "v"(q[2]), "s"(np[0]));
+  r[2] = (uint32_t)acc & kMask29;
+  acc >>= 29;
+  asm("v_mad_i64_i32 %0, %1, %2, %3, %0\n\tv_mad_i64_i32 %0, %1, %4, %5, %0\n\tv_mad_i64_i32 %0, %1, %6, %7, %0\n\tv_mad_i64_i32 %0, %1, %8, %9, %0\n\tv_mad_i64_i32 %0, %1, %10, %11, %0\n\tv_mad_i64_i32 %0, %1, %12, %13, %0\n\tv_mad_i64_i32 %0, %1, %14, %15, %0\n\tv_mad_i64_i32 %0, %1, %16, %17, %0"
+      : "+v"(acc), "=&s"(cc)
+      : "v"(x[0]), "v"(w[3]), "v"(x[1]), "v"(w[2]), "v"(x[2]), "v"(w[1]),
+        "v"(x[3]), "v"(w[0]), "v"(q[0]), "s"(np[3]), "v"(q[1]), "s"(np[2]),
+        "v"(q[2]), "s"(np[1]), "v"(q[3]), "s"(np[0]));
+  r[3] = (uint32_t)acc & kMask29;
+  acc >>= 29;
+  asm("v_mad_i64_i32 %0, %1, %2, %3, %0\n\tv_mad_i64_i32 %0, %1, %4, %5, %0\n\tv_mad_i64_i32 %0, %1, %6, %7, %0\n\tv_mad_i64_i32 %0, %1, %8, %9, %0\n\tv_mad_i64_i32 %0, %1, %10, %11, %0\n\tv_mad_i64_i32 %0, %1, %12, %13, %0\n\tv_mad_i64_i32 %0, %1, %14, %15, %0\n\tv_mad_i64_i32 %0, %1, %16, %17, %0\n\tv_mad_i64_i32 %0, %1, %18, %19, %0\n\tv_mad_i64_i32 %0, %1, %20, %21, %0"
+      : "+v"(acc), "=&s"(cc)
+      : "v"(x[0]), "v"(w[4]), "v"(x[1]), "v"(w[3]), "v"(x[2]), "v"(w[2]),
+        "v"(x[3]), "v"(w[1]), "v"(x[4]), "v"(w[0]), "v"(q[0]), "s"(np[4]),
+        "v"(q[1]), "s"(np[3]), "v"(q[2]), "s"(np[2]), "v"(q[3]), "s"(np[1]),
+        "v"(q[4]), "s"(np[0]));
+  r[4] = (uint32_t)acc & kMask29;
+  acc >>= 29;
+  asm("v_mad_i64_i32 %0, %1, %2, %3, %0\n\tv_mad_i64_i32 %0, %1, %4, %5, %0\n\tv_mad_i64_i32 %0, %1, %6, %7, %0\n\tv_mad_i64_i32 %0, %1, %8, %9, %0\n\tv_mad_i64_i32 %0, %1, %10, %11, %0\n\tv_mad_i64_i32 %0, %1, %12, %13, %0\n\tv_mad_i64_i32 %0, %1, %14, %15, %0\n\tv_mad_i64_i32 %0, %1, %16, %17, %0\n\tv_mad_i64_i32 %0, %1, %18, %19, %0\n\tv_mad_i64_i32 %0, %1, %20, %21, %0\n\tv_mad_i64_i32 %0, %1, %22, %23, %0\n\tv_mad_i64_i32 %0, %1, %24, %25, %0"
+      : "+v"(acc), "=&s"(cc)
+      : "v"(x[0]), "v"(w[5]), "v"(x[1]), "v"(w[4]), "v"(x[2]), "v"(w[3]),
+        "v"(x[3]), "v"(w[2]), "v"(x[4]), "v"(w[1]), "v"(x[5]), "v"(w[0]),
+        "v"(q[0]), "s"(np[5]), "v"(q[1]), "s"(np[4]), "v"(q[2]), "s"(np[3]),
+        "v"(q[3]), "s"(np[2]), "v"(q[4]), "s"(np[1]), "v"(q[5]), "s"(np[0]));
+  r[5] = (uint32_t)acc & kMask29;
+  acc >>= 29;
+  asm("v_mad_i64_i32 %0, %1, %2, %3, %0\n\tv_mad_i64_i32 %0, %1, %4, %5, %0\n\tv_mad_i64_i32 %0, %1, %6, %7, %0\n\tv_mad_i64_i32 %0, %1, %8, %9, %0\n\tv_mad_i64_i32 %0, %1, %10, %11, %0\n\tv_mad_i64_i32 %0, %1, %12, %13, %0\n\tv_mad_i64_i32 %0, %1, %14, %15, %0\n\tv_mad_i64_i32 %0, %1, %16, %17, %0\n\tv_mad_i64_i32 %0, %1, %18, %19, %0\n\tv_mad_i64_i32 %0, %1, %20, %21, %0\n\tv_mad_i64_i32 %0, %1, %22, %23, %0\n\tv_mad_i64_i32 %0, %1, %24, %25, %0\n\tv_mad_i64_i32 %0, %1, %26, %27, %0\n\tv_mad_i64_i32 %0, %1, %28, %29, %0"
+      : "+v"(acc), "=&s"(cc)
+      : "v"(x[0]), "v"(w[6]), "v"(x[1]), "v"(w[5]), "v"(x[2]), "v"(w[4]),
+        "v"(x[3]), "v"(w[3]), "v"(x[4]), "v"(w[2]), "v"(x[5]), "v"(w[1]),
+        "v"(x[6]), "v"(w[0]), "v"(q[0]), "s"(np[6]), "v"(q[1]), "s"(np[5]),
+        "v"(q[2]), "s"(np[4]), "v"(q[3]), "s"(np[3]), "v"(q[4]), "s"(np[2]),
+        "v"(q[5]), "s"(np[1]), "v"(q[6]), "s"(np[0]));
+  r[6] = (uint32_t)acc & kMask29;
+  acc >>= 29;
+  asm("v_mad_i64_i32 %0, %1, %2, %3, %0\n\tv_mad_i64_i32 %0, %1, %4, %5, %0\n\tv_mad_i64_i32 %0, %1, %6, %7, %0\n\tv_mad_i64_i32 %0, %1, %8, %9, %0\n\tv_mad_i64_i32 %0, %1, %10, %11, %0\n\tv_mad_i64_i32 %0, %1, %12, %13, %0\n\tv_mad_i64_i32 %0, %1, %14, %15, %0\n\tv_mad_i64_i32 %0, %1, %16, %17, %0\n\tv_mad_i64_i32 %0, %1, %18, %19, %0\n\tv_mad_i64_i32 %0, %1, %20, %21, %0\n\tv_mad_i64_i32 %0, %1, %22, %23, %0\n\tv_mad_i64_i32 %0, %1, %24, %25, %0\n\tv_mad_i64_i32 %0, %1, %26, %27, %0\n\tv_mad_i64_i32 %0, %1, %28, %29, %0\n\tv_mad_i64_i32 %0, %1, %30, %31, %0\n\tv_mad_i64_i32 %0, %1, %32, %33, %0"
+      : "+v"(acc), "=&s"(cc)
+      : "v"(x[0]), "v"(w[7]), "v"(x[1]), "v"(w[6]), "v"(x[2]), "v"(w[5]),
+        "v"(x[3]), "v"(w[4]), "v"(x[4]), "v"(w[3]), "v"(x[5]), "v"(w[2]),
+        "v"(x[6]), "v"(w[1]), "v"(x[7]), "v"(w[0]), "v"(q[0]), "s"(np[7]),
+        "v"(q[1]), "s"(np[6]), "v"(q[2]), "s"(np[5]), "v"(q[3]), "s"(np[4]),
+        "v"(q[4]), "s"(np[3]), "v"(q[5]), "s"(np[2]), "v"(q[6]), "s"(np[1]),
+        "v"(q[7]), "s"(np[0]));
+  r[7] = (uint32_t)acc & kMask29;
+  acc >>= 29;
+  asm("v_mad_i64_i32 %0, %1, %2, %3, %0\n\tv_mad_i64_i32 %0, %1, %4, %5, %0\n\tv_mad_i64_i32 %0, %1, %6, %7, %0\n\tv_mad_i64_i32 %0, %1, %8, %9, %0\n\tv_mad_i64_i32 %0, %1, %10, %11, %0\n\tv_mad_i64_i32 %0, %1, %12, %13, %0\n\tv_mad_i64_i32 %0, %1, %14, %15, %0\n\tv_mad_i64_i32 %0, %1, %16, %17, %0\n\tv_mad_i64_i32 %0, %1, %18, %19, %0\n\tv_mad_i64_i32 %0, %1, %20, %21, %0\n\tv_mad_i64_i32 %0, %1, %22, %23, %0\n\tv_mad_i64_i32 %0, %1, %24, %25, %0\n\tv_mad_i64_i32 %0, %1, %26, %27, %0\n\tv_mad_i64_i32 %0, %1, %28, %29, %0\n\tv_mad_i64_i32 %0, %1, %30, %31, %0\n\tv_mad_i64_i32 %0, %1, %32, %33, %0\n\tv_mad_i64_i32 %0, %1, %34, %35, %0\n\tv_mad_i64_i32 %0, %1, %36, %37, %0"
+      : "+v"(acc), "=&s"(cc)
+      : "v"(x[0]), "v"(w[8]), "v"(x[1]), "v"(w[7]), "v"(x[2]), "v"(w[6]),
+        "v"(x[3]), "v"(w[5]), "v"(x[4]), "v"(w[4]), "v"(x[5]), "v"(w[3]),
+        "v"(x[6]), "v"(w[2]), "v"(x[7]), "v"(w[1]), "v"(x[8]), "v"(w[0]),
+        "v"(q[0]), "s"(np[8]), "v"(q[1]), "s"(np[7]), "v"(q[2]), "s"(np[6]),
+        "v"(q[3]), "s"(np[5]), "v"(q[4]), "s"(np[4]), "v"(q[5]), "s"(np[3]),
+        "v"(q[6]), "s"(np[2]), "v"(q[7]), "s"(np[1]), "v"(q[8]), "s"(np[0]));
+  r[8] = (uint32_t)acc & kMask29;
+}
+
+__device__ __forceinline__ void mulc29_s9u(uint32_t (&r)[9], const uint32_t (&x)[9], const uint32_t (&w)[9],
+                                          const uint32_t (&ws)[9], const uint32_t (&np)[9]) {
+  uint32_t q[9];
+  int64_t acc = -kShoupBiasS;
+  uint64_t cc;
+  asm("v_mad_i64_i32 %0, %1, %2, %3, %0\n\tv_mad_i64_i32 %0, %1, %4, %5, %0\n\tv_mad_i64_i32 %0, %1, %6, %7, %0\n\tv_mad_i64_i32 %0, %1, %8, %9, %0\n\tv_mad_i64_i32 %0, %1, %10, %11, %0\n\tv_mad_i64_i32 %0, %1, %12, %13, %0\n\tv_mad_i64_i32 %0, %1, %14, %15, %0\n\tv_mad_i64_i32 %0, %1, %16, %17, %0"
+      : "+v"(acc), "=&s"(cc)
+      : "v"(x[0]), "s"(ws[7]), "v"(x[1]), "s"(ws[6]), "v"(x[2]), "s"(ws[5]),
+        "v"(x[3]), "s"(ws[4]), "v"(x[4]), "s"(ws[3]), "v"(x[5]), "s"(ws[2]),
+        "v"(x[6]), "s"(ws[1]), "v"(x[7]), "s"(ws[0]));
+  acc >>= 29;
+  asm("v_mad_i64_i32 %0, %1, %2, %3, %0\n\tv_mad_i64_i32 %0, %1, %4, %5, %0\n\tv_mad_i64_i32 %0, %1, %6, %7, %0\n\tv_mad_i64_i32 %0, %1, %8, %9, %0\n\tv_mad_i64_i32 %0, %1, %10, %11, %0\n\tv_mad_i64_i32 %0, %1, %12, %13, %0\n\tv_mad_i64_i32 %0, %1, %14, %15, %0\n\tv_mad_i64_i32 %0, %1, %16, %17, %0\n\tv_mad_i64_i32 %0, %1, %18, %19, %0"
+      : "+v"(acc), "=&s"(cc)
+      : "v"(x[0]), "s"(ws[8]), "v"(x[1]), "s"(ws[7]), "v"(x[2]), "s"(ws[6]),
+        "v"(x[3]), "s"(ws[5]), "v"(x[4]), "s"(ws[4]), "v"(x[5]), "s"(ws[3]),
+        "v"(x[6]), "s"(ws[2]), "v"(x[7]), "s"(ws[1]), "v"(x[8]), "s"(ws[0]));
+  acc >>= 29;
+  asm("v_mad_i64_i32 %0, %1, %2, %3, %0\n\tv_mad_i64_i32 %0, %1, %4, %5, %0\n\tv_mad_i64_i32 %0, %1, %6, %7, %0\n\tv_mad_i64_i32 %0, %1, %8, %9, %0\n\tv_mad_i64_i32 %0, %1, %10, %11, %0\n\tv_mad_i64_i32 %0, %1, %12, %13, %0\n\tv_mad_i64_i32 %0, %1, %14, %15, %0\n\tv_mad_i64_i32 %0, %1, %16, %17, %0"
+      : "+v"(acc), "=&s"(cc)
+      : "v"(x[1]), "s"(ws[8]), "v"(x[2]), "s"(ws[7]), "v"(x[3]), "s"(ws[6]),
+        "v"(x[4]), "s"(ws[5]), "v"(x[5]), "s"(ws[4]), "v"(x[6]), "s"(ws[3]),
+        "v"(x[7]), "s"(ws[2]), "v"(x[8]), "s"(ws[1]));
+  q[0] = (uint32_t)acc & kMask29;
+  acc >>= 29;
+  asm("v_mad_i64_i32 %0, %1, %2, %3, %0\n\tv_mad_i64_i32 %0, %1, %4, %5, %0\n\tv_mad_i64_i32 %0, %1, %6, %7, %0\n\tv_mad_i64_i32 %0, %1, %8, %9, %0\n\tv_mad_i64_i32 %0, %1, %10, %11, %0\n\tv_mad_i64_i32 %0, %1, %12, %13, %0\n\tv_mad_i64_i32 %0, %1, %14, %15, %0"
+      : "+v"(acc), "=&s"(cc)
+      : "v"(x[2]), "s"(ws[8]), "v"(x[3]), "s"(ws[7]), "v"(x[4]), "s"(ws[6]),
+        "v"(x[5]), "s"(ws[5]), "v"(x[6]), "s"(ws[4]), "v"(x[7]), "s"(ws[3]),
+        "v"(x[8]), "s"(ws[2]));
+  q[1] = (uint32_t)acc & kMask29;
+  acc >>= 29;
+  asm("v_mad_i64_i32 %0, %1, %2, %3, %0\n\tv_mad_i64_i32 %0, %1, %4, %5, %0\n\tv_mad_i64_i32 %0, %1, %6, %7, %0\n\tv_mad_i64_i32 %0, %1, %8, %9, %0\n\tv_mad_i64_i32 %0, %1, %10, %11, %0\n\tv_mad_i64_i32 %0, %1, %12, %13, %0"
+      : "+v"(acc), "=&s"(cc)
+      : "v"(x[3]), "s"(ws[8]), "v"(x[4]), "s"(ws[7]), "v"(x[5]), "s"(ws[6]),
+        "v"(x[6]), "s"(ws[5]), "v"(x[7]), "s"(ws[4]), "v"(x[8]), "s"(ws[3]));
+  q[2] = (uint32_t)acc & kMask29;
+  acc >>= 29;
+  asm("v_mad_i64_i32 %0, %1, %2, %3, %0\n\tv_mad_i64_i32 %0, %1, %4, %5, %0\n\tv_mad_i64_i32 %0, %1, %6, %7, %0\n\tv_mad_i64_i32 %0, %1, %8, %9, %0\n\tv_mad_i64_i32 %0, %1, %10, %11, %0"
+      : "+v"(acc), "=&s"(cc)
+      : "v"(x[4]), "s"(ws[8]), "v"(x[5]), "s"(ws[7]), "v"(x[6]), "s"(ws[6]),
+        "v"(x[7]), "s"(ws[5]), "v"(x[8]), "s"(ws[4]));
+  q[3] = (uint32_t)acc & kMask29;
+  acc >>= 29;
+  asm("v_mad_i64_i32 %0, %1, %2, %3, %0\n\tv_mad_i64_i32 %0, %1, %4, %5, %0\n\tv_mad_i64_i32 %0, %1, %6, %7, %0\n\tv_mad_i64_i32 %0, %1, %8, %9, %0"
+      : "+v"(acc), "=&s"(cc)
+      : "v"(x[5]), "s"(ws[8]), "v"(x[6]), "s"(ws[7]), "v"(x[7]), "s"(ws[6]),
+        "v"(x[8]), "s"(ws[5]));
+  q[4] = (uint32_t)acc & kMask29;
+  acc >>= 29;
+  asm("v_mad_i64_i32 %0, %1, %2, %3, %0\n\tv_mad_i64_i32 %0, %1, %4, %5, %0\n\tv_mad_i64_i32 %0, %1, %6, %7, %0"
+      : "+v"(acc), "=&s"(cc)
+      : "v"(x[6]), "s"(ws[8]), "v"(x[7]), "s"(ws[7]), "v"(x[8]), "s"(ws[6]));
+  q[5] = (uint32_t)acc & kMask29;
+  acc >>= 29;
+  asm("v_mad_i64_i32 %0, %1, %2, %3, %0\n\tv_mad_i64_i32 %0, %1, %4, %5, %0"
+      : "+v"(acc), "=&s"(cc)
+      : "v"(x[7]), "s"(ws[8]), "v"(x[8]), "s"(ws[7]));
+  q[6] = (uint32_t)acc & kMask29;
+  acc >>= 29;
+  asm("v_mad_i64_i32 %0, %1, %2, %3, %0"
+      : "+v"(acc), "=&s"(cc)
+      : "v"(x[8]), "s"(ws[8]));
+  q[7] = (uint32_t)acc & kMask29;
+  acc >>= 29;
+  q[8] = (uint32_t)acc;
+  acc = 0;
+  asm("v_mad_i64_i32 %0, %1, %2, %3, %0\n\tv_mad_i64_i32 %0, %1, %4, %5, %0"
+      : "+v"(acc), "=&s"(cc)
+      : "v"(x[0]), "s"(w[0]), "v"(q[0]), "s"(np[0]));
+  r[0] = (uint32_t)acc & kMask29;
+  acc >>= 29;
+  asm("v_mad_i64_i32 %0, %1, %2, %3, %0\n\tv_mad_i64_i32 %0, %1, %4, %5, %0\n\tv_mad_i64_i32 %0, %1, %6, %7, %0\n\tv_mad_i64_i32 %0, %1, %8, %9, %0"
+      : "+v"(acc), "=&s"(cc)
+      : "v"(x[0]), "s"(w[1]), "v"(x[1]), "s"(w[0]), "v"(q[0]), "s"(np[1]),
+        "v"(q[1]), "s"(np[0]));
+  r[1] = (uint32_t)acc & kMask29;
+  acc >>= 29;
+  asm("v_mad_i64_i32 %0, %1, %2, %3, %0\n\tv_mad_i64_i32 %0, %1, %4, %5, %0\n\tv_mad_i64_i32 %0, %1, %6, %7, %0\n\tv_mad_i64_i32 %0, %1, %8, %9, %0\n\tv_mad_i64_i32 %0, %1, %10, %11, %0\n\tv_mad_i64_i32 %0, %1, %12, %13, %0"
+      : "+v"(acc), "=&s"(cc)
+      : "v"(x[0]), "s"(w[2]), "v"(x[1]), "s"(w[1]), "v"(x[2]), "s"(w[0]),
+        "v"(q[0]), "s"(np[2]), "v"(q[1]), "s"(np[1]), "v"(q[2]), "s"(np[0]));
+  r[2] = (uint32_t)acc & kMask29;
+  acc >>= 29;
+  asm("v_mad_i64_i32 %0, %1, %2, %3, %0\n\tv_mad_i64_i32 %0, %1, %4, %5, %0\n\tv_mad_i64_i32 %0, %1, %6, %7, %0\n\tv_mad_i64_i32 %0, %1, %8, %9, %0\n\tv_mad_i64_i32 %0, %1, %10, %11, %0\n\tv_mad_i64_i32 %0, %1, %12, %13, %0\n\tv_mad_i64_i32 %0, %1, %14, %15, %0\n\tv_mad_i64_i32 %0, %1, %16, %17, %0"
+      : "+v"(acc), "=&s"(cc)
+      : "v"(x[0]), "s"(w[3]), "v"(x[1]), "s"(w[2]), "v"(x[2]), "s"(w[1]),
+        "v"(x[3]), "s"(w[0]), "v"(q[0]), "s"(np[3]), "v"(q[1]), "s"(np[2]),
+        "v"(q[2]), "s"(np[1]), "v"(q[3]), "s"(np[0]));
+  r[3] = (uint32_t)acc & kMask29;
+  acc >>= 29;
+  asm("v_mad_i64_i32 %0, %1, %2, %3, %0\n\tv_mad_i64_i32 %0, %1, %4, %5, %0\n\tv_mad_i64_i32 %0, %1, %6, %7, %0\n\tv_mad_i64_i32 %0, %1, %8, %9, %0\n\tv_mad_i64_i32 %0, %1, %10, %11, %0\n\tv_mad_i64_i32 %0, %1, %12, %13, %0\n\tv_mad_i64_i32 %0, %1, %14, %15, %0\n\tv_mad_i64_i32 %0, %1, %16, %17, %0\n\tv_mad_i64_i32 %0, %1, %18, %19, %0\n\tv_mad_i64_i32 %0, %1, %20, %21, %0"
+      : "+v"(acc), "=&s"(cc)
+      : "v"(x[0]), "s"(w[4]), "v"(x[1]), "s"(w[3]), "v"(x[2]), "s"(w[2]),
+        "v"(x[3]), "s"(w[1]), "v"(x[4]), "s"(w[0]), "v"(q[0]), "s"(np[4]),
+        "v"(q[1]), "s"(np[3]), "v"(q[2]), "s"(np[2]), "v"(q[3]), "s"(np[1]),
+        "v"(q[4]), "s"(np[0]));
+  r[4] = (uint32_t)acc & kMask29;
+  acc >>= 29;
+  asm("v_mad_i64_i32 %0, %1, %2, %3, %0\n\tv_mad_i64_i32 %0, %1, %4, %5, %0\n\tv_mad_i64_i32 %0, %1, %6, %7, %0\n\tv_mad_i64_i32 %0, %1, %8, %9, %0\n\tv_mad_i64_i32 %0, %1, %10, %11, %0\n\tv_mad_i64_i32 %0, %1, %12, %13, %0\n\tv_mad_i64_i32 %0, %1, %14, %15, %0\n\tv_mad_i64_i32 %0, %1, %16, %17, %0\n\tv_mad_i64_i32 %0, %1, %18, %19, %0\n\tv_mad_i64_i32 %0, %1, %20, %21, %0\n\tv_mad_i64_i32 %0, %1, %22, %23, %0\n\tv_mad_i64_i32 %0, %1, %24, %25, %0"
+      : "+v"(acc), "=&s"(cc)
+      : "v"(x[0]), "s"(w[5]), "v"(x[1]), "s"(w[4]), "v"(x[2]), "s"(w[3]),
+        "v"(x[3]), "s"(w[2]), "v"(x[4]), "s"(w[1]), "v"(x[5]), "s"(w[0]),
+        "v"(q[0]), "s"(np[5]), "v"(q[1]), "s"(np[4]), "v"(q[2]), "s"(np[3]),
+        "v"(q[3]), "s"(np[2]), "v"(q[4]), "s"(np[1]), "v"(q[5]), "s"(np[0]));
+  r[5] = (uint32_t)acc & kMask29;
+  acc >>= 29;
+  asm("v_mad_i64_i32 %0, %1, %2, %3, %0\n\tv_mad_i64_i32 %0, %1, %4, %5, %0\n\tv_mad_i64_i32 %0, %1, %6, %7, %0\n\tv_mad_i64_i32 %0, %1, %8, %9, %0\n\tv_mad_i64_i32 %0, %1, %10, %11, %0\n\tv_mad_i64_i32 %0, %1, %12, %13, %0\n\tv_mad_i64_i32 %0, %1, %14, %15, %0\n\tv_mad_i64_i32 %0, %1, %16, %17, %0\n\tv_mad_i64_i32 %0, %1, %18, %19, %0\n\tv_mad_i64_i32 %0, %1, %20, %21, %0\n\tv_mad_i64_i32 %0, %1, %22, %23, %0\n\tv_mad_i64_i32 %0, %1, %24, %25, %0\n\tv_mad_i64_i32 %0, %1, %26, %27, %0\n\tv_mad_i64_i32 %0, %1, %28, %29, %0"
+      : "+v"(acc), "=&s"(cc)
+      : "v"(x[0]), "s"(w[6]), "v"(x[1]), "s"(w[5]), "v"(x[2]), "s"(w[4]),
+        "v"(x[3]), "s"(w[3]), "v"(x[4]), "s"(w[2]), "v"(x[5]), "s"(w[1]),
+        "v"(x[6]), "s"(w[0]), "v"(q[0]), "s"(np[6]), "v"(q[1]), "s"(np[5]),
+        "v"(q[2]), "s"(np[4]), "v"(q[3]), "s"(np[3]), "v"(q[4]), "s"(np[2]),
+        "v"(q[5]), "s"(np[1]), "v"(q[6]), "s"(np[0]));
+  r[6] = (uint32_t)acc & kMask29;
+  acc >>= 29;
+  asm("v_mad_i64_i32 %0, %1, %2, %3, %0\n\tv_mad_i64_i32 %0, %1, %4, %5, %0\n\tv_mad_i64_i32 %0, %1, %6, %7, %0\n\tv_mad_i64_i32 %0, %1, %8, %9, %0\n\tv_mad_i64_i32 %0, %1, %10, %11, %0\n\tv_mad_i64_i32 %0, %1, %12, %13, %0\n\tv_mad_i64_i32 %0, %1, %14, %15, %0\n\tv_mad_i64_i32 %0, %1, %16, %17, %0\n\tv_mad_i64_i32 %0, %1, %18, %19, %0\n\tv_mad_i64_i32 %0, %1, %20, %21, %0\n\tv_mad_i64_i32 %0, %1, %22, %23, %0\n\tv_mad_i64_i32 %0, %1, %24, %25, %0\n\tv_mad_i64_i32 %0, %1, %26, %27, %0\n\tv_mad_i64_i32 %0, %1, %28, %29, %0\n\tv_mad_i64_i32 %0, %1, %30, %31, %0\n\tv_mad_i64_i32 %0, %1, %32, %33, %0"
+      : "+v"(acc), "=&s"(cc)
+      : "v"(x[0]), "s"(w[7]), "v"(x[1]), "s"(w[6]), "v"(x[2]), "s"(w[5]),
+        "v"(x[3]), "s"(w[4]), "v"(x[4]), "s"(w[3]), "v"(x[5]), "s"(w[2]),
+        "v"(x[6]), "s"(w[1]), "v"(x[7]), "s"(w[0]), "v"(q[0]), "s"(np[7]),
+        "v"(q[1]), "s"(np[6]), "v"(q[2]), "s"(np[5]), "v"(q[3]), "s"(np[4]),
+        "v"(q[4]), "s"(np[3]), "v"(q[5]), "s"(np[2]), "v"(q[6]), "s"(np[1]),
+        "v"(q[7]), "s"(np[0]));
+  r[7] = (uint32_t)acc & kMask29;
+  acc >>= 29;
+  asm("v_mad_i64_i32 %0, %1, %2, %3, %0\n\tv_mad_i64_i32 %0, %1, %4, %5, %0\n\tv_mad_i64_i32 %0, %1, %6, %7, %0\n\tv_mad_i64_i32 %0, %1, %8, %9, %0\n\tv_mad_i64_i32 %0, %1, %10, %11, %0\n\tv_mad_i64_i32 %0, %1, %12, %13, %0\n\tv_mad_i64_i32 %0, %1, %14, %15, %0\n\tv_mad_i64_i32 %0, %1, %16, %17, %0\n\tv_mad_i64_i32 %0, %1, %18, %19, %0\n\tv_mad_i64_i32 %0, %1, %20, %21, %0\n\tv_mad_i64_i32 %0, %1, %22, %23, %0\n\tv_mad_i64_i32 %0, %1, %24, %25, %0\n\tv_mad_i64_i32 %0, %1, %26, %27, %0\n\tv_mad_i64_i32 %0, %1, %28, %29, %0\n\tv_mad_i64_i32 %0, %1, %30, %31, %0\n\tv_mad_i64_i32 %0, %1, %32, %33, %0\n\tv_mad_i64_i32 %0, %1, %34, %35, %0\n\tv_mad_i64_i32 %0, %1, %36, %37, %0"
+      : "+v"(acc), "=&s"(cc)
+      : "v"(x[0]), "s"(w[8]), "v"(x[1]), "s"(w[7]), "v"(x[2]), "s"(w[6]),
+        "v"(x[3]), "s"(w[5]), "v"(x[4]), "s"(w[4]), "v"(x[5]), "s"(w[3]),
+        "v"(x[6]), "s"(w[2]), "v"(x[7]), "s"(w[1]), "v"(x[8]), "s"(w[0]),
+        "v"(q[0]), "s"(np[8]), "v"(q[1]), "s"(np[7]), "v"(q[2]), "s"(np[6]),
+        "v"(q[3]), "s"(np[5]), "v"(q[4]), "s"(np[4]), "v"(q[5]), "s"(np[3]),
+        "v"(q[6]), "s"(np[2]), "v"(q[7]), "s"(np[1]), "v"(q[8]), "s"(np[0]));
+  r[8] = (uint32_t)acc & kMask29;
+}
 #else
 F29_HD void mulc29_a9(uint32_t (&r)[9], const uint32_t (&x)[9], const uint32_t (&w)[9], const uint32_t (&ws)[9],
                        const uint32_t (&pbar)[9]) {
@@ -440,6 +712,14 @@
                         const uint32_t (&pbar)[9]) {
   mulc29<9>(r, x, w, ws, pbar);
 }
+F29_HD void mulc29_s9(uint32_t (&r)[9], const uint32_t (&x)[9], const uint32_t (&w)[9], const uint32_t (&ws)[9],
+                       const uint32_t (&np)[9]) {
+  mulc29_s<9>(r, x, w, ws, np);
+}
+F29_HD void mulc29_s9u(uint32_t (&r)[9], const uint32_t (&x)[9], const uint32_t (&w)[9], const uint32_t (&ws)[9],
+                        const uint32_t (&np)[9]) {
+  mulc29_s<9>(r, x, w, ws, np);
+}
 F29_HD void mont29_a9(uint32_t (&r)[9], const uint32_t (&a)[9], const uint32_t (&b)[9], const Mod29<9>& M) {
   mont29<9>(r, a, b, M);
 }
diff --git a/ntt_amd/csrc/ntt_kernels_impl.hpp b/ntt_amd/csrc/ntt_kernels_impl.hpp
--- a/ntt_amd/csrc/ntt_kernels_impl.hpp
+++ b/ntt_amd/csrc/ntt_kernels_impl.hpp
@@ -79,6 +79,53 @@
     E::template bfly_l<K3>(x[base + 2], x[base + 3], F);
     E::template bfly_l<K3>(x[base + 4], x[base + 5], F);
     E::template bfly_l<K3>(x[base + 6], x[base + 7], F);
+  }
+}
+
+template <class E, class = void>
+struct signed_lazy_t { static constexpr bool value = false; };
+template <class E>
+struct signed_lazy_t<E, decltype((void)E::SIGNED_LAZY)> { static constexpr bool value = E::SIGNED_LAZY; };
+template <class E, int Q, bool FAST>
+constexpr bool signed_slot(int k) { return FAST && signed_lazy_t<E>::value && Q <= 4 && k != 0; }
+
+template <class E, int Q, bool SG>
+constexpr int out_bound() {
+  if constexpr (SG)
+    return E::UNSIGNED_BOUND;
+  else
+    return E::IN * Q;
+}
+
+template <class E, bool SG>
+__device__ __forceinline__ void unsign_if(uint32_t (&x)[E::W], const typename E::Args& F) {
+  if constexpr (SG) E::unsign(x, F);
+}
+template <class E, bool SG>
+__device__ __forceinline__ void mul_sg(uint32_t (&x)[E::W], const typename E::Tw& t, const typename E::Args& F) {
+  if constexpr (SG)
+    E::mul_s(x, t, F);
+  else
+    E::mul(x, t, F);
+}
+template <class E, bool SG>
+__device__ __forceinline__ void mul_u_sg(uint32_t (&x)[E::W], const typename E::Tw& t, const typename E::Args& F) {
+  if constexpr (SG)
+    E::mul_us(x, t, F);
+  else
+    E::mul_u(x, t, F);
+}
+
+template <class E, int Q, int base, int N>
+__device__ __forceinline__ void dft_q_sgn(uint32_t (&x)[N][E::W], const typename E::Args& F) {
+  static_assert(Q == 2 || Q == 4, "signed DFTs: radix 2 and 4");
+  if constexpr (Q == 2) {
+    E::bfly_sgn(x[base], x[base + 1]);
+  } else {
+    E::bfly_sgn(x[base], x[base + 2]);
+    E::bfly_sgn_w(x[base + 1], x[base + 3], F.w8[1], F);
+    E::bfly_sgn(x[base], x[base + 1]);
+    E::bfly_sgn(x[base + 2], x[base + 3]);
   }
 }
 
@@ -114,18 +161,20 @@
 }
 template <class E, int Q, int base, bool FAST, int N>
 __device__ __forceinline__ void dft(uint32_t (&x)[N][E::W], const typename E::Args& F) {
-  if constexpr (FAST)
+  if constexpr (FAST && signed_lazy_t<E>::value && Q <= 4)
+    dft_q_sgn<E, Q, base>(x, F);
+  else if constexpr (FAST)
     dft_q_fast<E, Q, base>(x, F);
   else
     dft_q<E, Q, base>(x, F);
 }
 
-template <class E>
+template <class E, bool SGN = false>
 __device__ __forceinline__ void twiddle_mul(uint32_t (&x)[E::W], const uint32_t* tab, uint32_t e,
                                             const typename E::Args& F) {
   typename E::Tw w;
   E::tload(w, tab, e);
-  E::mul(x, w, F);
+  mul_sg<E, SGN>(x, w, F);
 }
 template <class E>
 __device__ __forceinline__ void twiddle_mul_lds(uint32_t (&x)[E::W], const uint32_t* lds_tw, uint32_t e,
@@ -178,6 +227,7 @@
   constexpr int EPT = E::EPT;
   constexpr int pqb = S::qb(s - 1), PQ = 1 << pqb, PG = EPT / PQ, psb = S::logsig(s - 1), plN = S::logN(s - 1);
   constexpr int qb = S::qb(s), Q = 1 << qb, G = EPT / Q, sb = S::logsig(s), lN = S::logN(s);
+  static_assert(!(LTW && FAST && signed_lazy_t<E>::value), "no signed product from LDS-staged twiddles");
   static_for<1>([&](auto) {
     if constexpr (s > 1) __syncthreads();
     static_for<PG>([&](auto J) {
@@ -222,21 +272,24 @@
           if constexpr (LTW)
             twiddle_mul_lds<E>(x[j * Q + brev_bits(k, qb)], lds_tw, (cp * k) << (LOGR - lN), A.F);
           else
-            twiddle_mul<E>(x[j * Q + brev_bits(k, qb)], A.tw_int, (cp * k) << (LOGR - lN), A.F);
+            twiddle_mul<E, signed_slot<E, Q, FAST>(k)>(x[j * Q + brev_bits(k, qb)], A.tw_int,
+                                                       (cp * k) << (LOGR - lN), A.F);
         });
       };
       if constexpr (Uniform<LOGR, ept_log<E>(), NT, s>::on) {
         const uint32_t cps = __builtin_amdgcn_readfirstlane(cp);
         if (cps == 0) {
           static_for<Q - 1>([&](auto K1) {
-            E::template reduce<E::IN * Q, E::IN, FAST, R32>(x[j * Q + brev_bits(K1 + 1, qb)], A.F);
+            constexpr bool SG = signed_slot<E, Q, FAST>(K1 + 1);
+            unsign_if<E, SG>(x[j * Q + brev_bits(K1 + 1, qb)], A.F);
+            E::template reduce<out_bound<E, Q, SG>(), E::IN, FAST, R32>(x[j * Q + brev_bits(K1 + 1, qb)], A.F);
           });
         } else if constexpr (E::SGPR_TW && !LTW) {
           static_for<Q - 1>([&](auto K1) {
             constexpr int k = K1 + 1;
             typename E::Tw w;
             E::tload_u(w, A.tw_int, (cps * k) << (LOGR - lN));
-            E::mul_u(x[j * Q + brev_bits(k, qb)], w, A.F);
+            mul_u_sg<E, signed_slot<E, Q, FAST>(k)>(x[j * Q + brev_bits(k, qb)], w, A.F);
           });
         } else {
           twiddles();
@@ -617,7 +670,7 @@
         E::template reduce<E::IN * Q, E::IN, FAST, R32>(x[j * Q], A.F);
         static_for<Q - 1>([&](auto K1) {
           constexpr int k = K1 + 1;
-          twiddle_mul<E>(x[j * Q + brev_bits(k, qb)], A.tw_int, pil[j] * k, A.F);
+          twiddle_mul<E, signed_slot<E, Q, FAST>(k)>(x[j * Q + brev_bits(k, qb)], A.tw_int, pil[j] * k, A.F);
         });
       }
     });
@@ -656,16 +709,20 @@
       static_for<Q>([&](auto K) {
         constexpr int k = K;
         uint32_t(&v)[E::W] = x[j * Q + brev_bits(k, qb)];
+        constexpr bool SG = signed_slot<E, Q, FAST>(k);
+        constexpr bool SG_MUL = SG && KIND == KIND_COLUMN && FULLTW && SHTW;
+        constexpr int OUTB = out_bound<E, Q, SG>();
+        unsign_if<E, SG && !SG_MUL>(v, A.F);
         const uint32_t pi = (rho << lN) + cp + (k << sb);
         const uint32_t kn = natural_index<LOGR, QB>(pi);
         size_t pos;
         if constexpr (KIND == KIND_DIT) {
           pos = colbase + c + ((size_t)kn << log_s);
-          E::template store<E::IN * Q, FAST, DW>(dst, ck(pos, A.dbg_dst_n), v, A.F);
+          E::template store<OUTB, FAST, DW>(dst, ck(pos, A.dbg_dst_n), v, A.F);
         } else if constexpr (KIND == KIND_STOCKHAM) {
           const uint32_t idx = col0 + c, kk = idx & ((1u << A.lgp) - 1);
           pos = ((size_t)(idx - kk) << LOGR) + kk + ((size_t)kn << A.lgp);
-          E::template store<E::IN * Q, FAST, DW>(dst, ck(pos, A.dbg_dst_n), v, A.F);
+          E::template store<OUTB, FAST, DW>(dst, ck(pos, A.dbg_dst_n), v, A.F);
         } else if constexpr (KIND == KIND_COLUMN) {
           if constexpr (FULLTW) {
             uint32_t tw[E::W];
@@ -677,7 +734,7 @@
             if constexpr (SHTW) {
               typename E::Tw tws;
               E::tload(tws, A.tw_full, ti);
-              E::mul(v, tws, A.F);
+              mul_sg<E, SG_MUL>(v, tws, A.F);
             } else {
               E::template load<E::TABW>(tw, A.tw_full, ti);
               E::mulv(v, tw, A.F);
@@ -723,11 +780,11 @@
                 mat_mul_out(v, (uint32_t)(pos >> A.il));
                 E::template store<E::MUL_OUT, FAST, DW>(dst, ck(at, A.dbg_dst_n), v, A.F);
               } else {
-                E::template store<E::IN * Q, FAST, DW>(dst, ck(at, A.dbg_dst_n), v, A.F);
+                E::template store<OUTB, FAST, DW>(dst, ck(at, A.dbg_dst_n), v, A.F);
               }
             }
           } else {
-            E::template store<E::IN * Q, FAST, DW>(dst, ck(out_pos(pos, bq), A.dbg_dst_n), v, A.F);
+            E::template store<OUTB, FAST, DW>(dst, ck(out_pos(pos, bq), A.dbg_dst_n), v, A.F);
           }
         } else {
           pos = kn;
@@ -742,7 +799,7 @@
             E::mul(v, A.F.ninv, A.F);
             E::template store<E::MUL_OUT, FAST>(dst, ck(out_pos(pos, b), A.dbg_dst_n), v, A.F);
           } else {
-            E::template store<E::IN * Q, FAST>(dst, ck(out_pos(pos, b), A.dbg_dst_n), v, A.F);
+            E::template store<OUTB, FAST>(dst, ck(out_pos(pos, b), A.dbg_dst_n), v, A.F);
           }
         }
       });
```

New measurement: 11.11 billion (median of 6 runs). About the same (+0.5%).
